# marsermd/DeepestScatter

Measured on AMD Instinct MI355X. Metric: Msamples/s (rays x spp) at 512^3 vol, 1024^2 frame; HBM GB/s vs roofline, higher is better.
Workload: dtype f32

## Files before the change

deepestscatter_amd/csrc/ct_api.cpp:

```cpp
#include <algorithm>
#include <array>
#include <atomic>
#include <chrono>
#include <climits>
#include <cmath>
#include <cstdarg>
#include <cstdio>
#include <cstdlib>
#include <cstring>
#include <new>
#include <string>
#include <utility>
#include <map>
#include <vector>

#include "../../include/cloudtrace.h"
#include "ct_handle.hpp"

static thread_local std::string g_create_error;

int ct::fail(CtHandle h, int code, const char *fmt, ...)
{
    char buf[512];
    va_list ap;
// ... 10 lines not shown

struct TracePhase {
    const char *name;
    std::chrono::steady_clock::time_point t0;
    bool on;
    TracePhase(CtHandle h, const char *n);
    ~TracePhase()
    {
        if (on) {
            fprintf(stderr, "[cloudtrace] %s %.2f ms\n", name,
                    std::chrono::duration<double, std::milli>(std::chrono::steady_clock::now() - t0).count());
        }
    }
};

inline TracePhase::TracePhase(CtHandle h, const char *n) : name(n), t0(std::chrono::steady_clock::now()), on(h && h->tune.TRACE) {}

static int check_invariants(CtHandle h);

static void v3_normalize_twice(const float in[3], float out[3])
{
    float v[3] = { in[0], in[1], in[2] };
    for (int pass = 0; pass < 2; pass++) {
        const float inv = 1.0f / sqrtf(v[0] * v[0] + v[1] * v[1] + v[2] * v[2]);
        v[0] *= inv;
        v[1] *= inv;
        v[2] *= inv;
    }
    out[0] = v[0];
    out[1] = v[1];
    out[2] = v[2];
}

static void mie_phase_texture(const float *raw, uint32_t n, std::vector<float> &out)
{
    out.resize(n);
    float average = 0;
    for (uint32_t i = 0; i < n; i++) {
        average += raw[i];
    }
    average /= (float)n;
    for (uint32_t i = 0; i < n; i++) {
        out[i] = raw[i] / average;
    }
}

static void mie_integral_texture(const float *raw, uint32_t n, std::vector<float> &out)
{
    out.resize(n);
    float sum = 0;
    for (uint32_t i = 0; i < n; i++) {
        sum += raw[i];
    }
    float integral = 0;
    for (uint32_t i = 0; i < n; i++) {
        integral += raw[i] / sum;
        out[i] = integral;
    }
}

static void build_guide(const std::vector<float> &cdf, std::vector<uint16_t> &guide)
{
    guide.assign(kGuideN + 2, 0);
    uint32_t t = 0;
    for (uint32_t b = 0; b <= (uint32_t)kGuideN; b++) {
        const float edge = (float)b / (float)kGuideN;
        while (t < cdf.size() && cdf[t] < edge) {
            t++;
        }
        guide[b] = (uint16_t)t;
    }
    guide[kGuideN + 1] = guide[kGuideN];
}

constexpr int kNeeSkipMaxR = 8;

static float nee_skip_reach(const DevScene &d)
{
    return d.sample_step * (1.0f - 1.0f / 256.0f);
}

static int nee_skip_radius(const DevScene &d, bool mie_finite)
{
    if (!mie_finite || !std::isfinite(d.lr) || !std::isfinite(d.lg) || !std::isfinite(d.lb) || !std::isfinite(d.sun_ratio) ||
        !(d.sample_step > 0.0f) || !std::isfinite(d.sample_step)) {
        return 0;
    }
    const double reach = (double)nee_skip_reach(d);
    int r = 0;
    for (const float s : { d.sx, d.sy, d.sz }) {
        const double D = reach * s * (1.0 + std::ldexp(1.0, -20)) + std::ldexp(1.0, -22) * (s + 1.0);
        if (!(D < kNeeSkipMaxR)) {
            return 0;
        }
        r = std::max(r, (int)std::ceil(D));
    }
    return std::max(r, 1);
}

static uint32_t morton2(uint32_t x, uint32_t y)
{
    auto spread = [](uint32_t v) {
        v &= 0xffffu;
        v = (v | (v << 8)) & 0x00ff00ffu;
        v = (v | (v << 4)) & 0x0f0f0f0fu;
        v = (v | (v << 2)) & 0x33333333u;
        v = (v | (v << 1)) & 0x55555555u;
        return v;
    };
    return spread(x) | (spread(y) << 1);
}

static uint32_t hilbert2(uint32_t x, uint32_t y)
{
    const uint32_t n = 1u << 15;
    uint32_t d = 0;
    for (uint32_t s = n / 2; s > 0; s /= 2) {
        const uint32_t rx = (x & s) ? 1u : 0u, ry = (y & s) ? 1u : 0u;
        d += s * s * ((3u * rx) ^ ry);
        if (ry == 0) {
            if (rx == 1) {
                x = n - 1u - x;
                y = n - 1u - y;
            }
            const uint32_t t = x;
            x = y;
            y = t;
        }
    }
    return d;
}

static void release(CtHandle h)
{
    if (!h) {
        return;
    }
    hipSetDevice(h->device);
    if (h->stream) {
        hipStreamSynchronize(h->stream);
    }
#ifdef CT_EXPERIMENTS
    if (h->vmm.va) {
        hipMemUnmap(h->vmm.va, h->vmm.size);
        for (auto &hd : h->vmm.handles) {
            hipMemRelease(hd);
        }
        hipMemAddressFree(h->vmm.va, h->vmm.size);
        h->vmm.va = nullptr;
        h->d_mbricks = nullptr;
    }
#endif
    void *ptrs[] = { h->d_density, h->d_inscatter, h->d_dbricks, h->d_ibricks, h->d_mbricks, h->d_tbricks, h->d_touched[0], h->d_touched[1], h->d_mrows, h->d_mcoarse, h->d_pyramid, h->d_mie, h->d_chopped, h->d_cdf,
                     h->d_guide, h->d_dist, h->d_dist_tmp, h->d_majorant, h->d_maj_cells, h->d_maj_codes, h->d_frame, h->d_mean, h->d_m2, h->d_screen, h->d_frames_all, h->cont[0], h->cont[1], h->left[0], h->left[1], h->d_cont_count, h->d_cont_total, h->d_primary, h->d_advance, h->d_pixels, h->d_cost, h->d_group_rank, h->d_group_order, h->d_job_group, h->d_job_sub, h->d_queue,
                     h->d_counters, h->d_colsum, h->d_avg, h->d_freeze, h->d_hit, h->d_cost_plane, h->d_timeline, h->pt.tasks, h->pt.primary, h->pt.frames, h->pt.pixels, h->pt.jg, h->pt.js,
                     h->net.found, h->net.waves, h->net.pos, h->net.dir, h->net.aux, h->net.out, h->net.desc, h->net.direct, h->net.tiles };
    for (void *p : ptrs) {
        if (p) {
            hipFree(p);
        }
    }
    for (auto &e : h->ev) {
        if (e) {
            hipEventDestroy(e);
        }
    }
    for (auto &sl : h->slots) {
        if (sl.queue) {
            hipFree(sl.queue);
        }
        for (hipEvent_t e : { sl.ev_in, sl.ev_start, sl.ev_done, sl.ev_acc0, sl.ev_acc1 }) {
            if (e) {
                hipEventDestroy(e);
            }
        }
    }
    for (hipEvent_t e : { h->ev_flush0, h->ev_flush1 }) {
        if (e) {
            hipEventDestroy(e);
        }
    }
    if (h->freeze_host) {
        hipHostFree(h->freeze_host);
    }
    if (h->hit_host) {
        hipHostFree(h->hit_host);
    }
    for (uint32_t *p : { h->jobs_host_g, h->jobs_host_s }) {
        if (p) {
            hipHostFree(p);
        }
    }
    if (h->own_stream) {
        hipStreamDestroy(h->own_stream);
    }
    delete h;
}

#ifdef CT_EXPERIMENTS
static int vmm_back_mbricks(CtHandle h)
{
    const size_t dense_bytes = h->mbricks_dense_bytes;
    hipMemAllocationProp prop{};
    prop.type = hipMemAllocationTypePinned;
    prop.location.type = hipMemLocationTypeDevice;
    prop.location.id = h->device;
    size_t gran = 0;
    HIPCHK(h, hipMemGetAllocationGranularity(&gran, &prop, hipMemAllocationGranularityRecommended));
    const size_t chunk = std::max<size_t>(gran, (size_t)2 << 20);
    if (chunk % 128 != 0 || (chunk & (chunk - 1)) != 0) {
        return fail(h, CT_E_HIP, "virtual-memory granularity %zu is not a power of two", chunk);
    }
    const size_t n_chunks = (dense_bytes + chunk - 1) / chunk;
    const size_t va_size = n_chunks * chunk;
    DevTemp<uint4> d_class;
    HIPCHK(h, dmalloc(&d_class, n_chunks));
    std::vector<uint4> cls(n_chunks);
    uint8_t *dense = h->d_mbricks;
    void *va = nullptr;
    std::vector<hipMemGenericAllocationHandle_t> handles;
    auto undo = [&]() {
        if (va) {
            hipMemUnmap(va, va_size);
            for (auto &hd : handles) {
                hipMemRelease(hd);
            }
            hipMemAddressFree(va, va_size);
        }
    };
#define VMMCHK(expr)                                                                                       \
    do {                                                                                                   \
        const hipError_t e_ = (expr);                                                                      \
        if (e_ != hipSuccess) {                                                                            \
            undo();                                                                                        \
            return fail(h, CT_E_HIP, "virtual-memory bricks: %s failed: %s", #expr, hipGetErrorString(e_)); \
        }                                                                                                  \
    } while (0)
    VMMCHK(launch_mbrick_chunk_class(dense, (int64_t)dense_bytes, (int64_t)chunk, d_class, h->stream));
    VMMCHK(hipMemcpyAsync(cls.data(), d_class, n_chunks * sizeof(uint4), hipMemcpyDeviceToHost, h->stream));
    VMMCHK(hipStreamSynchronize(h->stream));
    VMMCHK(hipMemAddressReserve(&va, va_size, chunk, nullptr, 0));
    std::vector<size_t> owner(n_chunks);
    std::vector<hipMemGenericAllocationHandle_t> of_chunk(n_chunks);
    std::map<uint64_t, size_t> first_with;
    size_t own = 0, with_data = 0;
    for (size_t c = 0; c < n_chunks; c++) {
        const bool whole = (c + 1) * chunk <= dense_bytes;
        owner[c] = c;
        if (whole && cls[c].x == 0u) {
            const uint64_t key = (uint64_t)cls[c].z | (uint64_t)cls[c].w << 32;
            const auto it = first_with.find(key);
            if (it != first_with.end()) {
                owner[c] = it->second;
            } else {
                first_with[key] = c;
            }
        } else {
            with_data += 1;
        }
        void *at = (uint8_t *)va + c * chunk;
        if (owner[c] == c) {
            hipMemGenericAllocationHandle_t hd;
            VMMCHK(hipMemCreate(&hd, chunk, &prop, 0));
            handles.push_back(hd);
            of_chunk[c] = hd;
            own += 1;
        } else {
            of_chunk[c] = of_chunk[owner[c]];
        }
        VMMCHK(hipMemMap(at, chunk, 0, of_chunk[c], 0));
    }
    hipMemAccessDesc acc{};
    acc.location = prop.location;
    acc.flags = hipMemAccessFlagsProtReadWrite;
    VMMCHK(hipMemSetAccess(va, va_size, &acc, 1));
    for (size_t c = 0; c < n_chunks; c++) {
        if (owner[c] != c) {
            continue;
        }
        uint8_t *at = (uint8_t *)va + c * chunk;
        const size_t n = std::min(chunk, dense_bytes - c * chunk);
        VMMCHK(hipMemcpyAsync(at, dense + c * chunk, n, hipMemcpyDeviceToDevice, h->stream));
        if (n < chunk) {
            VMMCHK(hipMemsetAsync(at + n, 0, chunk - n, h->stream));
        } else if (cls[c].x == 0u) {
            VMMCHK(launch_mbrick_chunk_quantize(at, (int64_t)chunk, h->stream));
        }
    }
    VMMCHK(hipStreamSynchronize(h->stream));
#undef VMMCHK
    HIPCHK(h, hipFree(dense));
    h->d_mbricks = (uint8_t *)va;
    h->dev.mbricks = h->d_mbricks;
    h->vmm.va = va;
    h->vmm.size = va_size;
    h->vmm.chunk = chunk;
    h->vmm.handles = std::move(handles);
    h->vmm.real_chunks = with_data;
    h->vmm.shared_chunks = own - with_data;
    h->vmm.mapped_chunks = n_chunks - own;
    h->mbricks_bytes = own * chunk;
    if (h->tune.STATS) {
        fprintf(stderr, "[cloudtrace] march bricks, dense addressing with sparse backing: %zu chunks of %zu KiB, %zu with texels, %zu distinct "
                        "empty ones, %zu mapped onto those: %.3f GB behind %.3f GB of addresses\n", n_chunks, chunk >> 10, with_data, own - with_data,
                n_chunks - own, (double)(own * chunk) / 1e9, (double)va_size / 1e9);
    }
    return CT_OK;
// ... 374 lines not shown
    HIPCHK(h, dmalloc(&h->d_majorant, nb));
    HIPCHK(h, launch_build_dist(h->d_density, nx, ny, nz, bbias, (int)bgx, (int)bgy, (int)bgz, h->d_dist,
                                h->d_dist_tmp, h->d_majorant, h->stream));
    HIPCHK(h, launch_brick_meta(h->d_dist, h->d_majorant, nx, ny, nz, bbias, (int)bgx, (int)bgy, (int)bgz,
                                h->d_dbricks, h->stream));
    return CT_OK;
}

static int build_majorant_grid(const CtScene *s, CtHandle h)
{
    DevScene &d = h->dev;
    const uint32_t nx = s->dims[0], ny = s->dims[1], nz = s->dims[2];
    const int32_t n[3] = { (int32_t)nx, (int32_t)ny, (int32_t)nz };
    const int bbias = d.brick_bias;
    int32_t lo[3], hi[3];
    density_bbox(s->density_host, n, lo, hi);
    const MajorantCells m = majorant_cells(n, bbias, lo, hi);
    if (!majorant_div_exact(m)) {
        return fail(h, CT_E_INVAL, "volume too large for the majorant grid's index arithmetic");
    }
    const auto &[C, div, origin, stored, virt] = m;
    const size_t cells = (size_t)stored[0] * stored[1] * stored[2];
    HIPCHK(h, dmalloc(&h->d_maj_cells, (cells + 3) & ~(size_t)3));
    HIPCHK(h, hipMemsetAsync(h->d_maj_cells, 0, (cells + 3) & ~(size_t)3, h->stream));
    HIPCHK(h, dmalloc(&h->d_maj_codes, (cells + 3) & ~(size_t)3));
    HIPCHK(h, hipMemsetAsync(h->d_maj_codes, 0, (cells + 3) & ~(size_t)3, h->stream));
    HIPCHK(h, launch_majorant_cells(h->d_density, nx, ny, nz, bbias, C, origin, stored[0], stored[1], stored[2], h->d_maj_cells,
                                    h->d_maj_codes, h->stream));
    d.maj_cells = h->d_maj_cells;
    d.maj_codes = h->d_maj_codes;
    d.mc_cell = C;
    d.mc_div = div;
    d.mc_gx = stored[0];
    d.mc_gy = stored[1];
    d.mc_gz = stored[2];
    d.mc_x0 = origin[0];
    d.mc_y0 = origin[1];
    d.mc_z0 = origin[2];
    d.mc_vx = virt[0];
    d.mc_vy = virt[1];
    d.mc_vz = virt[2];
    const int32_t bg[3] = { d.brick_gx, d.brick_gy, d.brick_gz };
    d.delta_interior = (cells_inside_apron(lo, hi, n, m, bg) && knob_flag(h->tune.DELTA_INTERIOR, true)) ? 1u : 0u;
    return CT_OK;
}

static int twin_grid(CtHandle h)
{
    DevScene &d = h->dev;
    const int bbias = d.brick_bias, tbias = ((bbias + 2) / 3) * 3;
    const int64_t tgx = ((int64_t)d.nx + bbias + tbias + 2) / 3 + 1, tgy = ((int64_t)d.ny + bbias + tbias + 2) / 3 + 1,
                  tgz = ((int64_t)d.nz + bbias + tbias + 2) / 3 + 1;
    if (!brick_indices_fit(tgx, tgy, tgz) || (int64_t)std::max({ d.nx, d.ny, d.nz }) + 2 * tbias >= (1 << 15)) {
        return fail(h, CT_E_INVAL, "volume too large for 32-bit brick indices");
    }
    if (hipMalloc(&h->d_tbricks, (size_t)(tgx * tgy * tgz) * 128) != hipSuccess) {
        return fail(h, CT_E_NOMEM, "out of device memory (twin bricks)");
    }
    d.tbricks = h->d_tbricks;
    d.t_bias = tbias;
    d.t_gx = (int32_t)tgx;
    d.t_gy = (int32_t)tgy;
    d.t_gz = (int32_t)tgz;
    if (!cells_inside_twin(d)) {
        d.delta_interior = 0u;
    }
    return CT_OK;
}

static int compact_march_bricks(CtHandle h, const uint8_t *tmp_b)
{
    DevScene &d = h->dev;
    const uint32_t nx = (uint32_t)d.nx, ny = (uint32_t)d.ny, nz = (uint32_t)d.nz;
    const int bbias = d.brick_bias;
    const int64_t bgx = d.brick_gx, bgy = d.brick_gy, bgz = d.brick_gz, mgx = d.m_gx;
    const size_t rows = (size_t)(bgy * bgz);
    DevTemp<uint32_t> d_x0, d_x1;
    DevTemp<uint8_t> compact;
    auto run = [&]() -> int {
        HIPCHK(h, dmalloc(&d_x0, rows));
        HIPCHK(h, dmalloc(&d_x1, rows));
        HIPCHK(h, hipMemsetAsync(d_x0, 0xff, rows * sizeof(uint32_t), h->stream));
        HIPCHK(h, hipMemsetAsync(d_x1, 0, rows * sizeof(uint32_t), h->stream));
        HIPCHK(h, launch_mbrick_extent(h->d_mbricks, (int)mgx, (int)bgy, (int)bgz, d_x0, d_x1, h->stream));
        std::vector<uint32_t> x0(rows), x1(rows);
        HIPCHK(h, hipMemcpyAsync(x0.data(), d_x0, rows * sizeof(uint32_t), hipMemcpyDeviceToHost, h->stream));
        HIPCHK(h, hipMemcpyAsync(x1.data(), d_x1, rows * sizeof(uint32_t), hipMemcpyDeviceToHost, h->stream));
        HIPCHK(h, hipStreamSynchronize(h->stream));
        std::vector<uint2> ri(rows);
        uint64_t lines = 0;
        for (size_t r = 0; r < rows; r++) {
            const uint32_t cnt = x1[r] > x0[r] ? x1[r] - x0[r] : 0u;
            ri[r] = make_uint2((uint32_t)lines, cnt ? (x0[r] | (cnt << 16)) : 0u);
            lines += cnt;
        }
        if (lines >= (1ull << 32)) {
            return fail(h, CT_E_INVAL, "volume too large for 32-bit brick indices");
        }
        HIPCHK(h, dmalloc(&h->d_mrows, rows));
        HIPCHK(h, hipMemcpyAsync(h->d_mrows, ri.data(), rows * sizeof(uint2), hipMemcpyHostToDevice, h->stream));
        HIPCHK(h, dmalloc(&compact, std::max<size_t>((size_t)lines, 1) * 128));
        HIPCHK(h, launch_mbrick_compact(h->d_mbricks, (int)mgx, (int)bgy, (int)bgz, h->d_mrows, compact, h->stream));
        const int cshift = 3;
        const int64_t cgx = (4 * bgx + 7) >> cshift, cgy = (4 * bgy + 7) >> cshift, cgz = (4 * bgz + 7) >> cshift;
        HIPCHK(h, dmalloc(&h->d_mcoarse, (size_t)(cgx * cgy * cgz)));
        HIPCHK(h, launch_coarse_clearance(tmp_b, nx, ny, nz, bbias, cshift, (int)cgx, (int)cgy, (int)cgz, h->d_mcoarse,
                                          h->stream));
        HIPCHK(h, hipStreamSynchronize(h->stream));
        HIPCHK(h, hipFree(h->d_mbricks));
        h->d_mbricks = compact.release();
        d.mbricks = h->d_mbricks;
        h->mbricks_bytes = (size_t)lines * 128;
        d.m_rows = h->d_mrows;
        d.m_coarse = h->d_mcoarse;
        d.m_cshift = cshift;
        d.m_cgx = (int32_t)cgx;
        d.m_cgxy = (int32_t)(cgx * cgy);
        return CT_OK;
    };
    const int rc = run();
    if (rc != CT_OK) {
        hipStreamSynchronize(h->stream);
    }
    return rc;
}

static int build_march_layouts(const CtScene *s, CtHandle h, int apron, const MarchStorage &ms, uint32_t zero_faces, bool mie_finite)
{
    DevScene &d = h->dev;
    const uint32_t nx = s->dims[0], ny = s->dims[1], nz = s->dims[2];
    const size_t texels = h->volume_bytes;
    const int bbias = d.brick_bias;
    const int64_t bgx = d.brick_gx, bgy = d.brick_gy, bgz = d.brick_gz;
#ifndef CT_EXPERIMENTS
    if (ms.experimental) {
        return fail(h, CT_E_INVAL, "march bricks behind virtual memory (CT_FLAG_VMM_BRICKS, CT_SPARSE=2..4) were measured and rejected "
                                   "(DESIGN.md 4.3 item 7b): they exist in the experiments build only (build --variant exp; CT_LIBRARY=libcloudtrace_exp.so)");
    }
#endif
    const int mbias = ((apron + 2) / 3) * 3;
    int64_t mgx = ((int64_t)nx + 2 * mbias + 2) / 3 + 1;
    if (ms.pad_rows) {
        int64_t p2 = 1;
        while (p2 < mgx) {
            p2 <<= 1;
        }
        mgx = p2;
    }
    if (!brick_indices_fit(mgx, bgy, bgz) || (int64_t)nx + 2 * mbias >= (1 << 17)) {
        return fail(h, CT_E_INVAL, "volume too large for 32-bit brick indices");
    }
    const size_t dense_bytes = (size_t)(mgx * bgy * bgz) * 128;
    h->mbricks_dense_bytes = h->mbricks_bytes = dense_bytes;
    HIPCHK(h, dmalloc(&h->d_mbricks, dense_bytes));
    d.mbricks = h->d_mbricks;
    d.m_bias_x = mbias;
    d.m_gx = (int32_t)mgx;
    d.m_gxy = (int32_t)(mgx * bgy);
    DevTemp<uint8_t> tmp_a, tmp_b, tmp_c;
    HIPCHK(h, dmalloc(&tmp_a, texels));
    if (dmalloc(&tmp_b, texels) != hipSuccess) {
        return fail(h, CT_E_NOMEM, "out of device memory (distance transform scratch)");
    }
    hipError_t e = launch_build_mbricks(h->d_density, nx, ny, nz, mbias, bbias, (int)mgx, (int)bgy, (int)bgz,
                                        tmp_a, tmp_b, h->d_mbricks, h->stream);
    if (e == hipSuccess) {
        e = launch_inscatter(d, h->d_inscatter, zero_faces, h->stream);
    }
    if (e == hipSuccess) {
        e = launch_build_bricks(h->d_inscatter, nx, ny, nz, bbias, (int)bgx, (int)bgy, (int)bgz, h->d_ibricks, h->stream);
    }
    const int nee_r = s->estimator == CT_EST_MARCH ? nee_skip_radius(d, mie_finite) : 0;
    if (e == hipSuccess && nee_r > 0) {
        e = dmalloc(&tmp_c, texels);
        if (e == hipSuccess) {
            e = launch_nee_skip_flags(h->d_inscatter, nx, ny, nz, nee_r, mbias, bbias, (int)mgx, (int)bgy, (int)bgz, tmp_a, tmp_c,
                                      h->d_mbricks, h->stream);
            d.nee_reach = nee_skip_reach(d);
            h->nee_skip_r = nee_r;
        }
    }
    if (e == hipSuccess && s->estimator == CT_EST_DELTA && d.delta_nee == 2u) {
        CT_TRY(twin_grid(h));
        e = launch_build_twin_bricks(h->d_density, h->d_inscatter, nx, ny, nz, d.t_bias, d.t_gx, d.t_gy, d.t_gz, h->d_tbricks, h->stream);
    }
    const hipError_t e2 = hipStreamSynchronize(h->stream);
    HIPCHK(h, e);
    HIPCHK(h, e2);
    return ms.sparse ? compact_march_bricks(h, tmp_b) : CT_OK;
}

static int frame_buffers(const CtScene *s, CtHandle h)
{
    const size_t pixels = (size_t)s->width * s->height;
    HIPCHK(h, dmalloc(&h->d_frame, pixels));
    HIPCHK(h, dmalloc(&h->d_mean, pixels));
    HIPCHK(h, dmalloc(&h->d_m2, pixels));
    HIPCHK(h, dmalloc(&h->d_screen, pixels));
    HIPCHK(h, dmalloc(&h->d_colsum, s->width));
    HIPCHK(h, dmalloc(&h->d_avg, 2));
    HIPCHK(h, dmalloc(&h->d_queue, kQueueWords));
    HIPCHK(h, dmalloc(&h->d_cont_count, 6));
    HIPCHK(h, hipMemsetAsync(h->d_cont_count, 0, 6 * sizeof(uint32_t), h->stream));
    h->cont_capacity = (size_t)h->shape.blocks * h->shape.threads;
    HIPCHK(h, hipEventCreate(&h->ev_flush0));
    HIPCHK(h, hipEventCreate(&h->ev_flush1));
    if (h->tune.TIMELINE.get()) {
        const size_t waves = (size_t)h->shape.blocks * h->shape.threads / 64u;
        HIPCHK(h, dmalloc(&h->d_timeline, 4 * waves));
        HIPCHK(h, hipMemsetAsync(h->d_timeline, 0, 4 * waves * sizeof(unsigned long long), h->stream));
    }
    HIPCHK(h, dmalloc(&h->d_cont_total, 1));
    HIPCHK(h, hipMemsetAsync(h->d_cont_total, 0, sizeof(unsigned long long), h->stream));
    for (auto &c : h->cont) {
        HIPCHK(h, dmalloc(&c, h->cont_capacity * (s->estimator == CT_EST_DELTA ? kContWordsDelta : kContWords)));
    }
    h->left_capacity = h->cont_capacity / 64;
    for (auto &c : h->left) {
        HIPCHK(h, dmalloc(&c, h->left_capacity * kLeftWords));
    }
    for (auto &sl : h->slots) {
        HIPCHK(h, dmalloc(&sl.queue, kQueueWords));
        for (hipEvent_t *e : { &sl.ev_in, &sl.ev_start, &sl.ev_done, &sl.ev_acc0, &sl.ev_acc1 }) {
            HIPCHK(h, hipEventCreate(e));
        }
    }
    HIPCHK(h, dmalloc(&h->d_counters, kCounterCount + 1 + kStatCount));
    HIPCHK(h, dmalloc(&h->d_freeze, 8));
    HIPCHK(h, hipMemsetAsync(h->d_freeze, 0, 8 * sizeof(uint32_t), h->stream));
    HIPCHK(h, hipHostMalloc((void **)&h->freeze_host, 4 * sizeof(uint32_t), hipHostMallocDefault));
    memset(h->freeze_host, 0, 4 * sizeof(uint32_t));
    HIPCHK(h, hipMemsetAsync(h->d_frame, 0, pixels * sizeof(float4), h->stream));
    HIPCHK(h, hipMemsetAsync(h->d_mean, 0, pixels * sizeof(float4), h->stream));
    HIPCHK(h, hipMemsetAsync(h->d_m2, 0, pixels * sizeof(float4), h->stream));
    HIPCHK(h, hipMemsetAsync(h->d_screen, 0, pixels * sizeof(uchar4), h->stream));
    HIPCHK(h, hipMemsetAsync(h->d_counters, 0, (kCounterCount + 1 + kStatCount) * sizeof(unsigned long long), h->stream));

    HIPCHK(h, dmalloc(&h->d_primary, 2 * pixels));
    HIPCHK(h, dmalloc(&h->d_advance, (s->estimator == CT_EST_DELTA ? 4 : 1) * pixels));
    HIPCHK(h, hipStreamSynchronize(h->stream));
    return CT_OK;
}

static int create_impl(const CtScene *s, CtHandle h)
{
    h->scene = *s;
    h->device = s->device;
    h->volume_bytes = (size_t)s->dims[0] * s->dims[1] * s->dims[2];
    h->tune = CtTuning::from_env();
    CT_TRY(open_device(s, h));
    CT_TRY(choose_schedule(s, h));
    scene_uniforms(s, h->dev);
    int apron = 0;
    CT_TRY(apron_grid(s, h, apron));
    CT_TRY(upload_mie(s, h, h->mie_finite));
    CT_TRY(build_apron_bricks(s, h));
    if (s->estimator == CT_EST_DELTA) {
        CT_TRY(build_majorant_grid(s, h));
    }
    const MarchStorage ms = march_storage(s, h->tune.SPARSE);
    h->zero_faces = zero_faces(s->density_host, s->dims[0], s->dims[1], s->dims[2]);
    CT_TRY(build_march_layouts(s, h, apron, ms, h->zero_faces, h->mie_finite));
#ifdef CT_EXPERIMENTS
    if (ms.vmm) {
        CT_TRY(vmm_back_mbricks(h));
    }
#endif
    CT_TRY(frame_buffers(s, h));

    const float eye[3] = { 2.5f, -0.4f, 0.f }, lookat[3] = { 0, 0, 0 }, up[3] = { 0, 1, 0 };
    float U[3], V[3], W[3];
    ct_calculate_camera_variables(eye, lookat, up, 30.0f, (float)s->width / (float)s->height, U, V, W);
    return ct_set_camera(h, eye, U, V, W);
}

extern "C" int ct_create(const CtScene *s, CtHandle *out)
{
    if (!out) {
        return fail(nullptr, CT_E_INVAL, "out is NULL");
    }
    *out = nullptr;
    if (!s) {
        return fail(nullptr, CT_E_INVAL, "scene is NULL");
    }
    if (s->abi_version != CT_ABI_VERSION) {
        return fail(nullptr, CT_E_INVAL, "abi_version %u, library is %u", s->abi_version, CT_ABI_VERSION);
    }
    if (!s->density_host || s->dims[0] < 2 || s->dims[1] < 2 || s->dims[2] < 2 || s->dims[0] > 2048 ||
        s->dims[1] > 2048 || s->dims[2] > 2048) {
        return fail(nullptr, CT_E_INVAL, "density volume missing or dims out of range [2,2048]");
    }
    if (s->mode < 0 || s->mode > 2) {
        return fail(nullptr, CT_E_INVAL, "Invalid Render Mode %d", s->mode);
    }
    if (s->estimator != CT_EST_MARCH && s->estimator != CT_EST_DELTA) {
        return fail(nullptr, CT_E_INVAL, "unknown estimator %d", s->estimator);
    }
    if (s->estimator == CT_EST_DELTA && (s->flags & CT_FLAG_SIMPLE_KERNEL)) {
        return fail(nullptr, CT_E_INVAL, "the one-thread-per-pixel cross-check kernel only implements MARCH");
    }
    if (!s->mie_host || !s->chopped_mie_host || s->mie_count != (uint32_t)kMieN) {
        return fail(nullptr, CT_E_INVAL, "Mie tables must be %d floats each", kMieN);
    }
    if (s->width == 0 || s->height == 0 || s->width > 12288 || s->height > 4096) {
        return fail(nullptr, CT_E_INVAL, "frame %ux%u out of range (seed packing x*4096+y needs H <= 4096)", s->width,
                    s->height);
    }
    if (!(s->sample_step > 0.f) || !(s->sample_step <= 0.03125f) || !(s->cloud_size_m > 0.f) ||
        !(s->mean_free_path_m > 0.f) || s->max_depth < 2 || s->max_depth > 65535) {
        return fail(nullptr, CT_E_INVAL, "sample_step/cloud_size_m/mean_free_path_m/max_depth out of range (max_depth 2..65535)");
    }
    if (!(s->cloud_size_m / s->mean_free_path_m * s->sample_step < 80.f)) {
        return fail(nullptr, CT_E_INVAL, "optical depth per step %g too large (must be < 80)",
                    (double)(s->cloud_size_m / s->mean_free_path_m * s->sample_step));
    }
    const float ll = s->light_direction[0] * s->light_direction[0] + s->light_direction[1] * s->light_direction[1] +
                     s->light_direction[2] * s->light_direction[2];
    if (!(ll > 0.f)) {
        return fail(nullptr, CT_E_INVAL, "light_direction is zero");
    }
    if (s->shard_count == 0 || s->shard_index >= s->shard_count) {
        return fail(nullptr, CT_E_INVAL, "shard %u of %u", s->shard_index, s->shard_count);
    }
    CtHandle h = new (std::nothrow) CtHandle_();
    if (!h) {
        return fail(nullptr, CT_E_NOMEM, "out of host memory");
    }
    const int rc = create_impl(s, h);
    if (rc != CT_OK) {
        g_create_error = h->error;
        release(h);
        return rc;
    }
    h->scene.density_host = nullptr;
    h->scene.mie_host = nullptr;
    h->scene.chopped_mie_host = nullptr;
    *out = h;
    return CT_OK;
}

extern "C" int ct_destroy(CtHandle h)
{
    release(h);
    return CT_OK;
}

extern "C" const char *ct_last_error(CtHandle h)
{
    return h ? h->error.c_str() : g_create_error.c_str();
}

extern "C" int ct_set_stream(CtHandle h, void *hip_stream)
{
    NEED(h);
    HIPCHK(h, hipStreamSynchronize(h->stream));
    h->stream = hip_stream ? (hipStream_t)hip_stream : h->own_stream;
    return CT_OK;
}

extern "C" int ct_set_camera(CtHandle h, const float eye[3], const float U[3], const float V[3], const float W[3])
{
    NEED(h);
    if (!eye || !U || !V || !W) {
        return fail(h, CT_E_INVAL, "camera vectors must not be NULL");
    }
    DevScene &d = h->dev;
    d.ex = eye[0]; d.ey = eye[1]; d.ez = eye[2];
    d.ux = U[0]; d.uy = U[1]; d.uz = U[2];
    d.vx = V[0]; d.vy = V[1]; d.vz = V[2];
    d.wx = W[0]; d.wy = W[1]; d.wz = W[2];
    h->camera_set = true;
    h->queue_dirty = true;
    discard_ahead(h);
    return CT_OK;
}

static int relight(CtHandle h, const CtScene &s)
{
    DevScene d = h->dev;
    light_uniforms(&s, d);
    const bool march = s.estimator == CT_EST_MARCH;
    const int nee_r = march ? nee_skip_radius(d, h->mie_finite) : 0;
    DevTemp<uint8_t> tmp_a, tmp_c;
    if (nee_r > 0 && (dmalloc(&tmp_a, h->volume_bytes) != hipSuccess || dmalloc(&tmp_c, h->volume_bytes) != hipSuccess)) {
        (void)hipGetLastError();
        return fail(h, CT_E_NOMEM, "out of device memory (shadow-zero flags scratch); the light is unchanged");
    }
    d.nee_reach = nee_r > 0 ? nee_skip_reach(d) : 0.0f;
    h->scene = s;
    h->dev = d;
    h->nee_skip_r = nee_r;
    discard_ahead(h);
    h->queue_dirty = true;
    h->tile_deepest.clear();
    const int nx = d.nx, ny = d.ny, nz = d.nz, bbias = d.brick_bias;
    hipError_t e = launch_inscatter(d, h->d_inscatter, h->zero_faces, h->stream);
    if (e == hipSuccess) {
        e = launch_build_bricks(h->d_inscatter, nx, ny, nz, bbias, d.brick_gx, d.brick_gy, d.brick_gz, h->d_ibricks, h->stream);
    }
    if (e == hipSuccess && march) {
        e = launch_shadow_zero_rows(h->d_inscatter, nx, ny, nz, nee_r, d.m_bias_x, bbias, d.m_gx, d.brick_gy, d.brick_gz, tmp_a, tmp_c,
                                    h->d_mbricks, h->d_mrows, h->stream);
    }
    if (e == hipSuccess && h->d_tbricks) {
        e = launch_twin_shadow_half(h->d_inscatter, nx, ny, nz, d.t_bias, d.t_gx, d.t_gy, d.t_gz, h->d_tbricks, h->stream);
    }
    const hipError_t e2 = hipStreamSynchronize(h->stream);
    HIPCHK(h, e);
    HIPCHK(h, e2);
    return CT_OK;
}

extern "C" int ct_set_light(CtHandle h, const float direction[3], const float color[3], float intensity)
{
    NEED_NOFLUSH(h);
    if (!direction) {
        return fail(h, CT_E_INVAL, "light direction must not be NULL");
    }
    if (!std::isfinite(direction[0]) || !std::isfinite(direction[1]) || !std::isfinite(direction[2])) {
        return fail(h, CT_E_INVAL, "light direction is not finite");
    }
    if (!(direction[0] * direction[0] + direction[1] * direction[1] + direction[2] * direction[2] > 0.f)) {
        return fail(h, CT_E_INVAL, "light_direction is zero");
    }
    if (h->vmm.va) {
        return fail(h, CT_E_INVAL, "ct_set_light: march bricks behind virtual memory cannot be re-lit");
    }
    const int rc = flush(h);
    if (rc != CT_OK) {
        return rc;
    }
    CtScene s = h->scene;
    for (int a = 0; a < 3; a++) {
        s.light_direction[a] = direction[a];
        if (color) {
            s.light_color[a] = color[a];
        }
    }
    s.light_intensity = intensity;
    return relight(h, s);
}

static int rebuild_queue(CtHandle h)
{
    TracePhase trace(h, "rebuild_queue");
    const uint32_t W = h->scene.width, H = h->scene.height;
    const size_t pixels = (size_t)W * H;
    HIPCHK(h, launch_primary_rays(h->dev, h->d_primary, h->stream));
    if (h->scene.estimator == CT_EST_DELTA) {
        HIPCHK(h, launch_primary_advance_delta(h->dev, h->d_primary, h->d_advance, h->stream));
    } else {
        HIPCHK(h, launch_primary_advance(h->dev, h->d_primary, h->d_advance, h->stream));
    }
    if (!h->d_hit) {
        HIPCHK(h, dmalloc(&h->d_hit, pixels));
        HIPCHK(h, hipHostMalloc((void **)&h->hit_host, pixels, hipHostMallocDefault));
    }
    HIPCHK(h, launch_hit_flags(h->d_primary, h->d_hit, (uint32_t)pixels, h->stream));
    HIPCHK(h, hipMemcpyAsync(h->hit_host, h->d_hit, pixels, hipMemcpyDeviceToHost, h->stream));
    HIPCHK(h, hipStreamSynchronize(h->stream));
    const uint8_t *hit = h->hit_host;
    const uint32_t tiles_x = h->dev.tiles_x, tiles_y = h->dev.tiles_y;
    std::vector<std::pair<uint32_t, uint32_t>> tiles;
    for (uint32_t ty = 0; ty < tiles_y; ty++) {
        for (uint32_t tx = 0; tx < tiles_x; tx++) {
            if (tile_owner(tx, ty, h->scene.shard_count) == h->scene.shard_index) {
                tiles.emplace_back(h->tile_hilbert ? hilbert2(tx, ty) : morton2(tx, ty), ty * tiles_x + tx);
            }
        }
    }
    std::sort(tiles.begin(), tiles.end());
    std::vector<uint32_t> list;
    list.reserve(pixels / std::max(1u, h->scene.shard_count) + 64);
    uint64_t own = 0;
    for (const auto &t : tiles) {
        const uint32_t ty = t.second / tiles_x, tx = t.second - ty * tiles_x;
        for (uint32_t l = 0; l < 64; l++) {
            const uint32_t x = tx * kTile + (l & 7u), y = ty * kTile + (l >> 3);
            if (x < W && y < H) {
                own++;
                const uint32_t p = y * W + x;
                if (hit[p]) {
                    list.push_back(p);
                }
            }
        }
    }
    h->own_pixels = own;
    h->hit_pixels = list.size();
    while (list.size() % 64 != 0) {
        list.push_back(0xffffffffu);
    }
    h->n_groups = (uint32_t)(list.size() / 64);
    if (h->n_groups > h->groups_capacity) {
        for (void *p : { (void *)h->d_pixels, (void *)h->d_cost }) {
            if (p) {
                HIPCHK(h, hipFree(p));
            }
        }
        h->d_pixels = h->d_cost = nullptr;
        for (void *p : { (void *)h->d_group_rank, (void *)h->d_group_order }) {
            if (p) {
                HIPCHK(h, hipFree(p));
            }
        }
        h->d_group_rank = h->d_group_order = nullptr;
        HIPCHK(h, dmalloc(&h->d_pixels, (size_t)h->n_groups * 64));
        HIPCHK(h, dmalloc(&h->d_cost, 2 * (size_t)h->n_groups));
        HIPCHK(h, dmalloc(&h->d_group_rank, (size_t)h->n_groups));
        HIPCHK(h, dmalloc(&h->d_group_order, (size_t)h->n_groups));
        h->groups_capacity = h->n_groups;
    }
    h->group_order.resize(h->n_groups);
    h->group_tile.resize(h->n_groups);
    for (uint32_t i = 0; i < h->n_groups; i++) {
        h->group_order[i] = i;
        const uint32_t p = list[(size_t)i * 64];
        h->group_tile[i] = (p / W / kTile) * tiles_x + (p % W) / kTile;
    }
    if (h->tile_deepest.size() == (size_t)tiles_x * tiles_y) {
        auto log2_class = [](uint32_t c) {
            uint32_t k = 0;
            while (c) {
                k++;
                c >>= 1;
            }
            return k;
        };
        std::stable_sort(h->group_order.begin(), h->group_order.end(), [&](uint32_t a, uint32_t b) {
            return log2_class(h->tile_deepest[h->group_tile[a]]) > log2_class(h->tile_deepest[h->group_tile[b]]);
        });
    }
    h->group_depth.assign(h->n_groups, 0.f);
    if (h->n_groups) {
        HIPCHK(h, hipMemcpyAsync(h->d_pixels, list.data(), list.size() * sizeof(uint32_t), hipMemcpyHostToDevice,
                                 h->stream));
        HIPCHK(h, hipMemsetAsync(h->d_cost, 0, 2 * (size_t)h->n_groups * sizeof(uint32_t), h->stream));
        HIPCHK(h, hipStreamSynchronize(h->stream));
    }
    h->queue_dirty = false;
    h->order_tuned = false;
    h->jobs_S = 0;
    return CT_OK;
}

static bool short_batch(CtHandle h, uint32_t S)
{
    return h->scene.estimator != CT_EST_DELTA && (double)S * (double)std::max<uint64_t>(h->hit_pixels, 1) < 4.0e7;
}

static int build_jobs(CtHandle h, uint32_t S, uint32_t chunk_groups)
{
    chunk_groups = std::max(1u, std::min(chunk_groups, std::max(h->n_groups, 1u)));
    if (h->jobs_S >= S && h->jobs_brief == short_batch(h, S) && h->chunk_groups == chunk_groups) {
        return CT_OK;
    }
    TracePhase trace(h, "build_jobs");
    if (h->order_tuned) {
        S = std::max(S, h->jobs_hint);
    }
    const float unit = (h->scene.estimator == CT_EST_DELTA) ? 1.f : 16.f;
    const bool brief = short_batch(h, S);
    const bool queues = (h->queues_enabled || (brief && !h->tune.XCD_QUEUES.get())) && !(h->scene.flags & CT_FLAG_SIMPLE_KERNEL) &&
                        (h->order_tuned || h->tune.XCD_QUEUES_UNTUNED.get());
    const uint32_t nq = (queues && h->n_groups >= (uint32_t)kQueues) ? (uint32_t)kQueues : 1u;
    const uint32_t regions_wanted = (brief && !h->queues_enabled && !h->tune.XCD_REGIONS.get()) ? 16u : h->regions;
    const float job_work = (brief && !h->tune.JOB_WORK.get()) ? 4.f : h->job_work;
    const float shared_cost = h->shared_depth * unit;
    std::vector<uint8_t> queue_of(h->n_groups, 0);
    {
        double total = 0;
        for (uint32_t g = 0; g < h->n_groups; g++) {
            if (nq > 1u && h->group_depth[g] >= shared_cost) {
                queue_of[g] = (uint8_t)kQueues;
            } else {
                total += (double)h->group_depth[g] + unit;
            }
        }
        double run = 0;
        for (uint32_t g = 0; g < h->n_groups; g++) {
            if (queue_of[g] == (uint8_t)kQueues) {
                continue;
            }
            const double w = (double)h->group_depth[g] + unit;
            const uint32_t regions = std::max(nq, regions_wanted);
            const uint32_t r = (uint32_t)std::min<double>(regions - 1, std::floor((run + 0.5 * w) / total * regions));
            queue_of[g] = (uint8_t)(r % nq);
            run += w;
        }
    }
    auto job_length = [&](uint32_t g) {
        const float d = h->group_depth[g];
        if (!h->order_tuned) {
            return 1u;
        }
        uint32_t len = h->job_max;
        if (d > 0.f) {
            len = (uint32_t)std::min((float)h->job_max, std::max(1.f, job_work * unit / d));
        }
        return len;
    };
    size_t total_jobs = 0;
    for (uint32_t g = 0; g < h->n_groups; g++) {
        const uint32_t len = job_length(g);
        total_jobs += (S + len - 1) / len;
    }
    if (total_jobs > h->jobs_host_capacity) {
        for (uint32_t **pp : { &h->jobs_host_g, &h->jobs_host_s }) {
            if (*pp) {
                HIPCHK(h, hipHostFree(*pp));
                *pp = nullptr;
            }
        }
        h->jobs_host_capacity = total_jobs + total_jobs / 4 + 1024;
        HIPCHK(h, hipHostMalloc((void **)&h->jobs_host_g, h->jobs_host_capacity * sizeof(uint32_t), hipHostMallocDefault));
        HIPCHK(h, hipHostMalloc((void **)&h->jobs_host_s, h->jobs_host_capacity * sizeof(uint32_t), hipHostMallocDefault));
    }
    uint32_t *const jg = h->jobs_host_g, *const js = h->jobs_host_s;
    size_t nj = 0;
    std::vector<double> q_weight(kQueues + 1, 0.0);
    const uint32_t n_chunks = h->n_groups ? (h->n_groups + chunk_groups - 1) / chunk_groups : 1u;
    if (n_chunks > 1 && h->chunk_interleave) {
        std::vector<uint32_t> mixed;
        mixed.reserve(h->n_groups);
        for (uint32_t c = 0; c < n_chunks; c++) {
            for (uint32_t r = c; r < h->n_groups; r += n_chunks) {
                mixed.push_back(h->group_order[r]);
            }
        }
        h->job_order = mixed;
    } else if (n_chunks > 1 && h->chunk_morton) {
        h->job_order.resize(h->n_groups);
        for (uint32_t g = 0; g < h->n_groups; g++) {
            h->job_order[g] = g;
        }
    } else {
        h->job_order = h->group_order;
    }
    h->chunk_q_begin.assign(n_chunks, std::array<uint32_t, kQueues + 2>{});
    for (uint32_t c = 0; c < n_chunks; c++) {
        const uint32_t r0 = c * chunk_groups, r1 = std::min(h->n_groups, r0 + chunk_groups);
        for (uint32_t x = 0; x <= (uint32_t)kQueues; x++) {
            h->chunk_q_begin[c][x] = (uint32_t)nj;
            if (x != 0u && nq == 1u && x != (uint32_t)kQueues) {
                continue;
            }
            for (uint32_t r = r0; r < r1; r++) {
                const uint32_t g = h->job_order[r];
                if (queue_of[g] != x) {
                    continue;
                }
                q_weight[x] += (double)h->group_depth[g] + unit;
                const uint32_t len = job_length(g);
                for (uint32_t s0 = 0; s0 < S; s0 += len) {
                    jg[nj] = g;
                    js[nj] = s0 | (std::min(len, S - s0) << 16);
                    nj += 1;
                }
            }
        }
        h->chunk_q_begin[c][kQueues + 1] = (uint32_t)nj;
    }
    for (int x = 0; x <= kQueues + 1; x++) {
        h->q_begin[x] = h->chunk_q_begin[0][x];
    }
    if (h->tune.STATS.get()) {
        fprintf(stderr, "[cloudtrace] job queues (S=%u, %u chunk(s) of %u groups):", S, n_chunks, chunk_groups);
        for (int x = 0; x <= kQueues; x++) {
            fprintf(stderr, " q%d weight %.0f;", x, q_weight[x]);
        }
        fprintf(stderr, "\n");
    }
    {
        std::vector<uint32_t> rank(h->n_groups);
        for (uint32_t r = 0; r < h->n_groups; r++) {
            rank[h->job_order[r]] = r;
        }
        if (h->n_groups) {
            HIPCHK(h, hipMemcpyAsync(h->d_group_rank, rank.data(), rank.size() * sizeof(uint32_t), hipMemcpyHostToDevice, h->stream));
            HIPCHK(h, hipMemcpyAsync(h->d_group_order, h->job_order.data(), h->job_order.size() * sizeof(uint32_t),
                                     hipMemcpyHostToDevice, h->stream));
            HIPCHK(h, hipStreamSynchronize(h->stream));
        }
    }
    h->chunk_groups = chunk_groups;
    h->n_chunks = n_chunks;
    h->n_jobs = (uint32_t)nj;
    if (h->n_jobs > h->jobs_capacity) {
        for (void *p : { (void *)h->d_job_group, (void *)h->d_job_sub }) {
            if (p) {
// ... 181 lines not shown
    }
    sl.pending = false;
    HIPCHK(h, hipEventSynchronize(sl.accumulated ? sl.ev_acc1 : sl.ev_done));
    float ms = 0;
    HIPCHK(h, hipEventElapsedTime(&ms, sl.ev_start, sl.ev_done));
    h->render_ms += ms;
    if (h->tune.TRACE.get()) {
        uint32_t cnt[3] = { 0, 0, 0 };
        hipMemcpy(cnt, h->d_cont_count, sizeof cnt, hipMemcpyDeviceToHost);
        fprintf(stderr, "[cloudtrace] estimator launch %.2f ms (suspended paths per buffer now: %u %u, cursor %u)\n", ms,
                cnt[0], cnt[1], cnt[2]);
    }
    if (sl.accumulated) {
        HIPCHK(h, hipEventElapsedTime(&ms, sl.ev_acc0, sl.ev_acc1));
        h->accum_ms += ms;
    }
    h->launches += 1;
    return CT_OK;
}

int ct::enqueue_convergence_test(CtHandle h, uint32_t subframes)
{
    HIPCHK(h, launch_converged_freeze(h->d_mean, h->d_m2, subframes, (uint64_t)h->scene.width * h->scene.height, 500u ,
                                      h->d_freeze, h->stream));
    HIPCHK(h, hipMemcpyAsync(h->freeze_host, h->d_freeze, 4 * sizeof(uint32_t), hipMemcpyDeviceToHost, h->stream));
    return CT_OK;
}

static int enqueue_accumulate(CtHandle h, CtHandle_::Slot &sl, const float4 *frames, bool dense, uint32_t n)
{
    const bool simple = (h->scene.flags & CT_FLAG_SIMPLE_KERNEL) != 0;
    const bool chunked = !(simple || dense) && h->n_chunks > 1;
    const uint32_t cadence = h->stop_cadence;
    const uint32_t *frozen = cadence ? h->d_freeze : nullptr;
    HIPCHK(h, hipEventRecord(sl.ev_acc0, h->stream));
    while (n != 0u) {
        const uint32_t off = sl.acc_done, next = sl.first + off;
        uint32_t piece = n;
        if (cadence && !chunked) {
            piece = std::min(n, cadence - (next - 1u) % cadence);
        }
        if (simple || dense) {
            HIPCHK(h, launch_accumulate_batch(frames + (size_t)off * h->scene.width * h->scene.height, h->d_mean, h->d_m2, next, piece,
                                              h->scene.width, h->scene.height, h->scene.shard_index, h->scene.shard_count,
                                              h->d_counters + 8, frozen, h->stream));
        } else {
            HIPCHK(h, launch_accumulate_list(frames + (size_t)off * frame_stride(h), (uint32_t)frame_stride(h), h->d_pixels, sl.groups * 64u,
                                             h->n_chunks <= 1 ? nullptr : h->d_group_order, sl.rank_base,
                                             sl.with_misses, h->d_primary, h->d_mean, h->d_m2, next, piece, h->scene.width,
                                             h->scene.height, h->scene.shard_index, h->scene.shard_count, h->d_counters + 8, frozen,
                                             h->stream));
        }
        sl.acc_done += piece;
        n -= piece;
        const uint32_t upto = sl.first + sl.acc_done - 1u;
        const bool whole_image = !chunked || (sl.last_chunk && sl.acc_done == sl.S);
        if (cadence && whole_image && upto % cadence == 0u && upto >= h->stop_min) {
            const int rc = enqueue_convergence_test(h, upto);
            if (rc != CT_OK) {
                return rc;
            }
        }
    }
    HIPCHK(h, hipEventRecord(sl.ev_acc1, h->stream));
    sl.accumulated = true;
    return CT_OK;
}

static uint32_t accumulate_target(CtHandle h)
{
    if (h->ahead == 0) {
        return 0xffffffffu;
    }
    const uint64_t lag = (uint64_t)std::max(h->n_regions - 1, 1) * h->ahead;
    return h->subframes > lag ? (uint32_t)(h->subframes - lag) : 0u;
}

static int advance_accumulate(CtHandle h, uint32_t target)
{
    while (!h->waiting.empty()) {
        const int w = h->waiting.front();
        CtHandle_::Slot &sl = h->slots[w];
        if (!sl.complete) {
            break;
        }
        const uint32_t next = sl.first + sl.acc_done, last = sl.first + sl.S - 1u;
        const uint32_t upto = std::min(last, target);
        if (upto >= next && sl.acc_done < sl.S) {
            const int rc = enqueue_accumulate(h, sl, slot_frames(h, w), false, upto - next + 1u);
            if (rc != CT_OK) {
                return rc;
            }
        }
        if (sl.acc_done < sl.S) {
            break;
        }
        sl.awaits_accumulate = false;
        h->waiting.erase(h->waiting.begin());
    }
    return CT_OK;
}

void ct::discard_ahead(CtHandle h)
{
    for (int w : h->waiting) {
        h->slots[w].awaits_accumulate = false;
    }
    h->waiting.clear();
    h->rendered = h->subframes;
}

static int launch_estimator(CtHandle h, const BatchArgs &ba)
{
    DevScene sc = h->dev;
    if (ba.S != 0 && short_batch(h, ba.S) && !h->tune.REGEN_MIN.get()) {
        sc.regen_min = 16;
    }
    bool launched = false;
#ifdef CT_EXPERIMENTS
    if (h->exchange && !ba.cost && !ba.cont_in && !ba.cont_out && h->scene.estimator == CT_EST_DELTA) {
        if (h->exchange == 2) {
            HIPCHK(h, launch_render_delta_w(sc, ba, h->xshape, h->stream));
        } else {
            HIPCHK(h, launch_render_delta_x(sc, ba, h->xshape, h->stream));
        }
        launched = true;
    }
#endif
    if (launched) {
    } else if (h->scene.estimator == CT_EST_DELTA) {
        HIPCHK(h, launch_render_delta(sc, ba, h->shape, h->stream));
    } else {
        HIPCHK(h, launch_render_persistent(sc, ba, h->shape, h->stream));
    }
    return CT_OK;
}

static int submit_batch(CtHandle h, int slot, float4 *dense_frames, uint32_t first, uint32_t S, bool accumulate,
                        bool suspend, uint32_t chunk)
{
    CtHandle_::Slot &sl = h->slots[slot];
    const bool simple = (h->scene.flags & CT_FLAG_SIMPLE_KERNEL) != 0;
    const bool dense = dense_frames != nullptr;
    const uint32_t max_age = (uint32_t)(h->n_regions - 1);
    const uint32_t rank_base = chunk * h->chunk_groups;
    const uint32_t chunk_n = h->n_groups > rank_base ? std::min(h->chunk_groups, h->n_groups - rank_base) : 0u;
    BatchArgs ba{};
    ba.frames = dense ? dense_frames : (simple ? slot_frames(h, slot) : h->d_frames_all);
    ba.frame_stride = (simple || dense) ? 0u : (uint32_t)frame_stride(h);
    ba.out_offset = (simple || dense) ? 0u : (uint32_t)((size_t)slot * h->slot_capacity);
    ba.primary = h->d_primary;
    ba.advance = h->no_advance ? nullptr : h->d_advance;
    ba.pixels = h->d_pixels;
    ba.group_rank = (simple || dense || h->n_chunks <= 1) ? nullptr : h->d_group_rank;
    ba.rank_base = rank_base;
    ba.job_group = h->d_job_group;
    ba.job_sub = h->d_job_sub;
    const bool measure = !h->order_tuned && !simple && !dense && chunk_n != 0u;
    if (measure) {
        const size_t entries = (size_t)S * frame_stride(h);
        if (entries > h->cost_plane_capacity) {
            if (h->d_cost_plane) {
                HIPCHK(h, hipFree(h->d_cost_plane));
                h->d_cost_plane = nullptr;
            }
            h->cost_plane_capacity = entries + entries / 4;
            HIPCHK(h, dmalloc(&h->d_cost_plane, h->cost_plane_capacity));
        }
        HIPCHK(h, hipMemsetAsync(h->d_cost_plane, 0, entries * sizeof(uint2), h->stream));
        ba.cost = h->d_cost_plane;
    }
    static const std::array<uint32_t, kQueues + 2> no_jobs{};
    const auto &qb = chunk < h->chunk_q_begin.size() ? h->chunk_q_begin[chunk] : no_jobs;
    ba.n_jobs = qb[kQueues + 1];
    for (int x = 0; x <= kQueues + 1; x++) {
        ba.q_begin[x] = qb[x];
    }
    const uint32_t chunk_jobs = qb[kQueues + 1] - qb[0];
    ba.first_subframe = first;
    ba.S = S;
    ba.queue = sl.queue;
    ba.counters = h->d_counters;
    ba.stats = h->d_counters + kCounterCount + 1;
    ba.timeline = h->d_timeline;
    ba.touched_density = h->d_touched[0];
    ba.touched_shadow = h->d_touched[1];
    if (suspend && short_batch(h, S) && h->serpentine) {
        ba.reverse = (uint32_t)(h->launch_no & 1u);
    }
    const int buf_out = (int)(h->launch_no & 1u), buf_in = buf_out ^ 1;
    ZeroList zero;
    if (h->cont_live) {
        ba.cont_in = h->cont[buf_in];
        ba.cont_in_count = h->d_cont_count + buf_in;
        ba.cont_cursor = h->d_cont_count + 2;
        ba.left_in = h->left[buf_in];
        ba.left_in_count = h->d_cont_count + 3 + buf_in;
        ba.left_cursor = h->d_cont_count + 5;
        zero.add(h->d_cont_count + 2, 1);
        zero.add(h->d_cont_count + 5, 1);
    }
    if (suspend) {
        ba.cont_out = h->cont[buf_out];
        ba.cont_out_count = h->d_cont_count + buf_out;
        ba.cont_capacity = (uint32_t)h->cont_capacity;
        ba.max_age = std::max(1u, max_age);
        ba.cont_total = h->d_cont_total;
        if (h->hand_on_jobs) {
            ba.left_out = h->left[buf_out];
            ba.left_out_count = h->d_cont_count + 3 + buf_out;
            ba.left_capacity = (uint32_t)h->left_capacity;
        }
        zero.add(h->d_cont_count + buf_out, 1);
        zero.add(h->d_cont_count + 3 + buf_out, 1);
    }
    zero.add(sl.queue, kQueueWords);
    HIPCHK(h, launch_zero_words(zero, h->stream));
    if (h->debug_invariants && !simple && !dense && h->n_groups != 0) {
        HIPCHK(h, hipMemsetD32Async((hipDeviceptr_t)slot_frames(h, slot), 0x7fc0deadu, (size_t)S * frame_stride(h) * 4u,
                                    h->stream));
    }
    HIPCHK(h, hipEventRecord(sl.ev_start, h->stream));
    if (simple) {
        h->host_paths += h->own_pixels * S;
        h->host_hits += h->hit_pixels * S;
        for (uint32_t s = 0; s < S; s++) {
            BatchArgs one = ba;
            one.frames = ba.frames + (size_t)s * h->scene.width * h->scene.height;
            one.first_subframe = first + s;
            one.S = 1;
            HIPCHK(h, launch_render_simple(h->dev, one, h->scene.shard_index, h->scene.shard_count, h->stream));
        }
    } else {
        if (chunk_jobs != 0 || ba.cont_in) {
            const int rc = launch_estimator(h, ba);
            if (rc != CT_OK) {
                return rc;
            }
            if (measure) {
                HIPCHK(h, launch_cost_reduce(h->d_cost_plane, (uint32_t)frame_stride(h), S, chunk_n,
                                             h->n_chunks <= 1 ? nullptr : h->d_group_order, rank_base, h->d_cost,
                                             h->d_cost + h->n_groups, h->stream));
            }
        }
        uint64_t chunk_hits = 0;
        for (uint32_t r = rank_base; r < rank_base + chunk_n; r++) {
            chunk_hits += (h->job_order[r] + 1u == h->n_groups) ? 64u - (uint64_t)((uint64_t)h->n_groups * 64u - h->hit_pixels) : 64u;
        }
        if (chunk == 0) {
            h->host_paths += h->own_pixels * S;
        }
        h->host_hits += chunk_hits * S;
        h->iv_expected_dealt += chunk_hits * S;
    }
    HIPCHK(h, hipEventRecord(sl.ev_done, h->stream));
    h->launch_no += 1;
    h->cont_live = suspend && !simple;
    sl.first = first;
    sl.S = S;
    sl.rank_base = rank_base;
    sl.groups = chunk_n;
    sl.with_misses = chunk == 0;
    sl.last_chunk = simple || dense || chunk + 1u >= std::max(h->n_chunks, 1u);
    sl.pending = true;
    sl.accumulated = false;
    sl.awaits_accumulate = false;
    sl.complete = false;
    sl.acc_done = 0;
    if (accumulate) {
        if (suspend) {
            sl.awaits_accumulate = true;
            h->waiting.push_back(slot);
            uint32_t younger = 0;
            for (size_t i = h->waiting.size(); i-- > 0;) {
                CtHandle_::Slot &w = h->slots[h->waiting[i]];
                if (!w.complete && ++younger > max_age) {
                    w.complete = true;
                }
            }
            return advance_accumulate(h, accumulate_target(h));
        } else {
            sl.complete = true;
            const int rc = enqueue_accumulate(h, sl, dense ? dense_frames : slot_frames(h, slot), dense, S);
            if (rc != CT_OK) {
                return rc;
            }
        }
    }
    return CT_OK;
}

static int check_invariants(CtHandle h)
{
    unsigned long long iv[4] = { 0, 0, 0, 0 }, bad = 0;
    HIPCHK(h, hipStreamSynchronize(h->stream));
    HIPCHK(h, hipMemcpy(iv, h->d_counters + kCounterCount + 1 + 64, sizeof iv, hipMemcpyDeviceToHost));
    HIPCHK(h, hipMemcpy(&bad, h->d_counters + 8, sizeof bad, hipMemcpyDeviceToHost));
    h->iv_checks += 1;
    const unsigned long long dealt = iv[0], resumed = iv[1], written = iv[2], suspended = iv[3];
    const bool simple = (h->scene.flags & CT_FLAG_SIMPLE_KERNEL) != 0;
    const bool ok = simple || (dealt + resumed == written + suspended && resumed == suspended && dealt == h->iv_expected_dealt &&
                               bad == 0);
    if (!ok) {
        h->iv_violations += 1;
        fprintf(stderr, "[cloudtrace] INVARIANT VIOLATED: dealt %llu (host expects %llu) resumed %llu written %llu suspended %llu, "
                        "samples without alpha 1 seen by accumulate: %llu\n",
                dealt, (unsigned long long)h->iv_expected_dealt, resumed, written, suspended, bad);
        return fail(h, CT_E_STATE, "invariant violated: dealt %llu (expected %llu) resumed %llu written %llu suspended %llu bad samples %llu",
                    dealt, (unsigned long long)h->iv_expected_dealt, resumed, written, suspended, bad);
    }
    return CT_OK;
}

int ct::flush(CtHandle h)
{
    if (h->cont_live) {
        BatchArgs ba{};
        ba.frames = h->d_frames_all;
        ba.frame_stride = (uint32_t)frame_stride(h);
        ba.primary = h->d_primary;
        ba.advance = h->no_advance ? nullptr : h->d_advance;
        ba.pixels = h->d_pixels;
        ba.job_group = h->d_job_group;
        ba.job_sub = h->d_job_sub;
        ba.n_jobs = 0;
        ba.first_subframe = 1;
        ba.S = 0;
        ba.queue = h->d_queue;
        ba.counters = h->d_counters;
        ba.stats = h->d_counters + kCounterCount + 1;
        const int buf_in = (int)((h->launch_no & 1u) ^ 1u);
        ba.cont_in = h->cont[buf_in];
        ba.cont_in_count = h->d_cont_count + buf_in;
        ba.cont_cursor = h->d_cont_count + 2;
        ba.left_in = h->left[buf_in];
        ba.left_in_count = h->d_cont_count + 3 + buf_in;
        ba.left_cursor = h->d_cont_count + 5;
        HIPCHK(h, hipMemsetAsync(h->d_cont_count + 2, 0, sizeof(uint32_t), h->stream));
        HIPCHK(h, hipMemsetAsync(h->d_cont_count + 5, 0, sizeof(uint32_t), h->stream));
        HIPCHK(h, hipMemsetAsync(h->d_queue, 0, kQueueWords * sizeof(uint32_t), h->stream));
        HIPCHK(h, hipEventRecord(h->ev_flush0, h->stream));
        const int rc = launch_estimator(h, ba);
        if (rc != CT_OK) {
            return rc;
        }
        HIPCHK(h, hipEventRecord(h->ev_flush1, h->stream));
        h->launch_no += 1;
        h->cont_live = false;
        HIPCHK(h, hipEventSynchronize(h->ev_flush1));
        float ms = 0;
        HIPCHK(h, hipEventElapsedTime(&ms, h->ev_flush0, h->ev_flush1));
        h->render_ms += ms;
        if (h->tune.TRACE.get()) {
            fprintf(stderr, "[cloudtrace] resume-only launch %.2f ms\n", ms);
        }
    }
    for (int w : h->waiting) {
        h->slots[w].complete = true;
    }
    {
        const int rc = advance_accumulate(h, h->ahead ? h->subframes : 0xffffffffu);
        if (rc != CT_OK) {
            return rc;
        }
    }
    for (int k = 0; k < CtHandle_::kMaxRegions; k++) {
        const int rc = collect(h, h->slots[k]);
        if (rc != CT_OK) {
            return rc;
        }
    }
    return h->debug_invariants ? check_invariants(h) : CT_OK;
}

static int prepare_batches(CtHandle h, uint32_t S)
{
    const bool simple = (h->scene.flags & CT_FLAG_SIMPLE_KERNEL) != 0;
    if (simple) {
        h->chunk_groups = std::max(h->n_groups, 1u);
        h->n_chunks = 1;
        return CT_OK;
    }
    if (h->queue_dirty) {
        int rc = flush(h);
        discard_ahead(h);
        if (rc == CT_OK) {
            rc = rebuild_queue(h);
        }
        if (rc != CT_OK) {
            return rc;
        }
    }
    const uint32_t want = groups_per_chunk(h, S);
    if (h->jobs_S < S || h->jobs_brief != short_batch(h, S) || h->chunk_groups != want || h->chunk_q_begin.empty()) {
        const int rc = flush(h);
        discard_ahead(h);
        return rc == CT_OK ? build_jobs(h, S, want) : rc;
    }
    return CT_OK;
}

static int run_batch(CtHandle h, float4 *dense_frames, uint32_t first, uint32_t S, bool accumulate)
{
    int rc = flush(h);
    discard_ahead(h);
    if (rc == CT_OK) {
        rc = prepare_batches(h, S);
    }
    if (rc == CT_OK && !dense_frames) {
        rc = ensure_frames(h, S, false);
    }
    if (rc != CT_OK) {
        return rc;
    }
    for (uint32_t c = 0; c < std::max(h->n_chunks, 1u) && rc == CT_OK; c++) {
        rc = submit_batch(h, 0, dense_frames, first, S, accumulate, false, c);
        if (rc == CT_OK) {
            rc = collect(h, h->slots[0]);
        }
    }
    if (rc != CT_OK) {
        return rc;
    }
    const bool simple = (h->scene.flags & CT_FLAG_SIMPLE_KERNEL) != 0;
    if (!simple && !h->order_tuned && !dense_frames) {
        return tune_order(h, S);
    }
    return CT_OK;
}

extern "C" int ct_render_subframe(CtHandle h, uint32_t subframe_id, float *frame_rgba_dev)
{
    NEED(h);
    if (!h->camera_set) {
        return fail(h, CT_E_STATE, "ct_set_camera has not been called");
    }
    const size_t bytes = (size_t)h->scene.width * h->scene.height * sizeof(float4);
    HIPCHK(h, launch_fill_frame(h->d_frame, h->scene.width, h->scene.height, h->scene.shard_index,
                                h->scene.shard_count, h->stream));
    const int rc = run_batch(h, h->d_frame, subframe_id, 1, false);
    if (rc != CT_OK) {
        return rc;
    }
    if (frame_rgba_dev) {
        HIPCHK(h, hipMemcpyAsync(frame_rgba_dev, h->d_frame, bytes, hipMemcpyDeviceToDevice, h->stream));
        HIPCHK(h, hipStreamSynchronize(h->stream));
    }
    return CT_OK;
}

extern "C" int ct_accumulate(CtHandle h, uint32_t subframe_id, const float *frame_rgba_dev)
{
    NEED(h);
    if (subframe_id == 0) {
        return fail(h, CT_E_INVAL, "subframe ids are 1-based (Camera.cpp:191)");
    }
    const float4 *src = frame_rgba_dev ? (const float4 *)frame_rgba_dev : h->d_frame;
    HIPCHK(h, hipEventRecord(h->ev[1], h->stream));
    HIPCHK(h, launch_accumulate_batch(src, h->d_mean, h->d_m2, subframe_id, 1, h->scene.width, h->scene.height,
                                      h->scene.shard_index, h->scene.shard_count, nullptr, h->stop_cadence ? h->d_freeze : nullptr,
                                      h->stream));
    if (h->stop_cadence && subframe_id % h->stop_cadence == 0u && subframe_id >= h->stop_min) {
        const int rc = enqueue_convergence_test(h, subframe_id);
        if (rc != CT_OK) {
            return rc;
        }
    }
    HIPCHK(h, hipEventRecord(h->ev[2], h->stream));
    HIPCHK(h, hipEventSynchronize(h->ev[2]));
    float ms = 0;
    HIPCHK(h, hipEventElapsedTime(&ms, h->ev[1], h->ev[2]));
    h->accum_ms += ms;
    h->subframes = subframe_id;
    discard_ahead(h);
    return CT_OK;
// ... 1144 lines not shown
```

deepestscatter_amd/csrc/ct_device.hpp:

```cpp
#pragma once

#include <hip/hip_runtime.h>
#include <stdint.h>

#include "../../include/ct_fmath.h"

namespace ct {

#define CT_DEV __device__ __forceinline__

struct f3 {
    float x, y, z;
};

CT_DEV f3 mk3(float x, float y, float z) { return f3{ x, y, z }; }
CT_DEV f3 add3(f3 a, f3 b) { return mk3(a.x + b.x, a.y + b.y, a.z + b.z); }
CT_DEV f3 sub3(f3 a, f3 b) { return mk3(a.x - b.x, a.y - b.y, a.z - b.z); }
CT_DEV f3 scale3(f3 a, float s) { return mk3(a.x * s, a.y * s, a.z * s); }
CT_DEV float dot3(f3 a, f3 b) { return a.x * b.x + a.y * b.y + a.z * b.z; }
CT_DEV f3 cross3(f3 a, f3 b)
{
    return mk3(a.y * b.z - a.z * b.y, a.z * b.x - a.x * b.z, a.x * b.y - a.y * b.x);
}
CT_DEV float rcp_(float x) { return 1.0f / x; }
// ... 35 lines not shown
struct DevScene {
    const uint8_t *dbricks;
    const uint8_t *ibricks;
    int32_t brick_bias;
    int32_t brick_gx;
    int32_t brick_gxy;
    int32_t brick_gy, brick_gz;
    uint32_t tex_fixed8;
    const uint8_t *mbricks;
    const uint2 *m_rows;
    const uint8_t *m_coarse;
    int32_t m_cshift, m_cgx, m_cgxy;
    const uint8_t *tbricks;
    int32_t t_bias;
    int32_t t_gx, t_gy, t_gz;
    uint32_t delta_nee;
    uint32_t delta_interior;
    const uint8_t *maj_cells;
    const uint8_t *maj_codes;
    int32_t mc_cell, mc_div, mc_gx, mc_gy, mc_gz, mc_x0, mc_y0, mc_z0, mc_vx, mc_vy, mc_vz;
    int32_t m_bias_x;
    int32_t m_gx, m_gxy;
    int32_t nx, ny, nz;
    float sx, sy, sz;
    float tsx, tsy, tsz;
    float bx, by, bz;
    float hx, hy, hz;
    float density_multiplier;
    float sample_step;
    float nlx, nly, nlz;
    float lr, lg, lb;
    float sun_ratio;
    const float *mie;
    const float *chopped;
    const float *cdf;
    const uint16_t *guide;
    float ex, ey, ez, ux, uy, uz, vx, vy, vz, wx, wy, wz;
    uint32_t width, height;
    uint32_t max_depth;
    int32_t mode;
    uint32_t tiles_x, tiles_y;
    uint32_t regen_min;
    uint32_t march_burst;
    uint32_t burst_scatter;
    uint32_t burst_idle;
    uint32_t tail_burst;
    uint32_t nee_cache;
    float nee_reach;
    uint32_t hint_period;
    uint32_t burst_march_min;
    uint32_t scatter_num, scatter_den;
    uint32_t scatter_min;
};

CT_DEV uint32_t tea4(uint32_t v0, uint32_t v1)
{
    uint32_t s0 = 0;
#pragma unroll
    for (int n = 0; n < 4; n++) {
        s0 += 0x9e3779b9u;
        v0 += ((v1 << 4) + 0xa341316cu) ^ (v1 + s0) ^ ((v1 >> 5) + 0xc8013ea4u);
        v1 += ((v0 << 4) + 0xad90777du) ^ (v0 + s0) ^ ((v0 >> 5) + 0x7e95761eu);
    }
    return v0;
}

CT_DEV uint32_t lcg24(uint32_t &prev)
{
    prev = 1664525u * prev + 1013904223u;
    return prev & 0x00FFFFFFu;
}

CT_DEV float u24_to_float(uint32_t u) { return (float)u / (float)0x01000000; }

CT_DEV bool in_box(const DevScene &sc, f3 p)
{
    return p.x >= -0.01f && p.y >= -0.01f && p.z >= -0.01f && p.x <= sc.hx && p.y <= sc.hy && p.z <= sc.hz;
}
CT_DEV bool in_box_flat(const DevScene &sc, f3 p)
{
    return (p.x >= -0.01f) & (p.y >= -0.01f) & (p.z >= -0.01f) & (p.x <= sc.hx) & (p.y <= sc.hy) & (p.z <= sc.hz);
}

CT_DEV float fract_(float x) { return __builtin_amdgcn_fractf(x); }

template <bool FIXED8>
CT_DEV float tex_weight(float x)
{
    if constexpr (FIXED8) {
        return __builtin_rintf(fract_(x) * 256.0f) * (1.0f / 256.0f);
    } else {
        return fract_(x);
    }
}

CT_DEV float filter_cell(uint2 c, float wx, float wy, float wz)
{
    const float t000 = (float)(c.x & 0xffu), t100 = (float)((c.x >> 8) & 0xffu);
    const float t010 = (float)((c.x >> 16) & 0xffu), t110 = (float)(c.x >> 24);
    const float t001 = (float)(c.y & 0xffu), t101 = (float)((c.y >> 8) & 0xffu);
    const float t011 = (float)((c.y >> 16) & 0xffu), t111 = (float)(c.y >> 24);
    const float c00 = fmaf(wx, t100 - t000, t000), c10 = fmaf(wx, t110 - t010, t010);
    const float c01 = fmaf(wx, t101 - t001, t001), c11 = fmaf(wx, t111 - t011, t011);
    const float c0 = fmaf(wy, c10 - c00, c00), c1 = fmaf(wy, c11 - c01, c01);
    return fmaf(wz, c1 - c0, c0) * (1.0f / 255.0f);
}

CT_DEV uint2 load_footprint(const DevScene &sc, const uint8_t *bricks, int32_t ix, int32_t iy, int32_t iz)
{
    const uint32_t x = (uint32_t)(ix + sc.brick_bias), y = (uint32_t)(iy + sc.brick_bias), z = (uint32_t)(iz + sc.brick_bias);
    const uint32_t brick = __umul24(z >> 2, (uint32_t)sc.brick_gxy) + __umul24(y >> 2, (uint32_t)sc.brick_gx) + (x >> 2);
    const uint32_t local = __umul24(z & 3u, 25u) + __umul24(y & 3u, 5u) + (x & 3u);
#ifdef CT_DEBUG_BOUNDS
    if ((x >> 2) >= (uint32_t)sc.brick_gx || (y >> 2) >= (uint32_t)sc.brick_gy || (z >> 2) >= (uint32_t)sc.brick_gz) {
        printf("CT_DEBUG_BOUNDS footprint texel (%d,%d,%d) outside the brick grid\n", ix, iy, iz);
        return make_uint2(0u, 0u);
    }
#endif
    const uint8_t *p = bricks + (((size_t)brick << 7) | local);
    uint2 a, c;
    __builtin_memcpy(&a, p, 8);
    __builtin_memcpy(&c, p + 25, 8);
    uint2 r;
    r.x = __builtin_amdgcn_perm(a.y, a.x, 0x06050100u);
    r.y = __builtin_amdgcn_perm(c.y, c.x, 0x06050100u);
    return r;
}

CT_DEV uint2 load_footprint_meta(const DevScene &sc, const uint8_t *bricks, int32_t ix, int32_t iy, int32_t iz,
                                 uint32_t &meta)
{
    const uint32_t x = (uint32_t)(ix + sc.brick_bias), y = (uint32_t)(iy + sc.brick_bias), z = (uint32_t)(iz + sc.brick_bias);
    const uint32_t brick = __umul24(z >> 2, (uint32_t)sc.brick_gxy) + __umul24(y >> 2, (uint32_t)sc.brick_gx) + (x >> 2);
    const uint32_t local = __umul24(z & 3u, 25u) + __umul24(y & 3u, 5u) + (x & 3u);
#ifdef CT_DEBUG_BOUNDS
    if ((x >> 2) >= (uint32_t)sc.brick_gx || (y >> 2) >= (uint32_t)sc.brick_gy || (z >> 2) >= (uint32_t)sc.brick_gz) {
        printf("CT_DEBUG_BOUNDS footprint texel (%d,%d,%d) outside the brick grid\n", ix, iy, iz);
        meta = 0u;
        return make_uint2(0u, 0u);
    }
#endif
    const uint8_t *base = bricks + ((size_t)brick << 7);
    const uint8_t *p = base + local;
    uint2 a, c;
    __builtin_memcpy(&a, p, 8);
    __builtin_memcpy(&c, p + 25, 8);
    meta = base[125];
    uint2 r;
    r.x = __builtin_amdgcn_perm(a.y, a.x, 0x06050100u);
    r.y = __builtin_amdgcn_perm(c.y, c.x, 0x06050100u);
    return r;
}

template <bool SPARSE>
CT_DEV uint2 load_footprint_m(const DevScene &sc, int32_t ix, int32_t iy, int32_t iz, uint32_t &meta)
{
    const uint32_t x = (uint32_t)(ix + sc.m_bias_x), y = (uint32_t)(iy + sc.brick_bias), z = (uint32_t)(iz + sc.brick_bias);
    const uint32_t bx = __umul24(x, 43691u) >> 17;
    const uint32_t lx = x - __umul24(bx, 3u);
    const uint32_t brick = __umul24(z >> 2, (uint32_t)sc.m_gxy) + __umul24(y >> 2, (uint32_t)sc.m_gx) + bx;
    const uint32_t local = __umul24(z & 3u, 25u) + __umul24(y & 3u, 5u) + lx;
#ifdef CT_DEBUG_BOUNDS
    if (bx >= (uint32_t)sc.m_gx || (y >> 2) >= (uint32_t)sc.brick_gy || (z >> 2) >= (uint32_t)sc.brick_gz) {
        printf("CT_DEBUG_BOUNDS march-brick texel (%d,%d,%d) outside the grid\n", ix, iy, iz);
        meta = 0u;
        return make_uint2(0u, 0u);
    }
#endif
    const uint8_t *p = sc.mbricks + (((size_t)brick << 7) | local);
    if (SPARSE) {
        const uint32_t row = __umul24(z >> 2, (uint32_t)sc.brick_gy) + (y >> 2);
        const uint2 ri = sc.m_rows[row];
        const uint32_t rel = bx - (ri.y & 0xffffu);
        if (rel >= (ri.y >> 16)) {
            const uint32_t cx = (uint32_t)(ix + sc.brick_bias) >> sc.m_cshift;
            meta = sc.m_coarse[__umul24(z >> sc.m_cshift, (uint32_t)sc.m_cgxy) + __umul24(y >> sc.m_cshift, (uint32_t)sc.m_cgx) + cx];
            return make_uint2(0u, 0u);
        }
        p = sc.mbricks + (((size_t)(ri.x + rel) << 7) | local);
    }
    uint2 a, c;
    __builtin_memcpy(&a, p, 8);
    __builtin_memcpy(&c, p + 25, 8);
    meta = __builtin_amdgcn_perm(a.y, a.x, 0x0c0c0c04u - lx);
    uint2 r;
    r.x = __builtin_amdgcn_perm(a.y, a.x, 0x06050100u);
    r.y = __builtin_amdgcn_perm(c.y, c.x, 0x06050100u);
    return r;
}

CT_DEV int32_t floor_to_int(float x)
{
    int32_t r;
    asm("v_cvt_flr_i32_f32 %0, %1" : "=v"(r) : "v"(x));
    return r;
}

template <bool FIXED8>
CT_DEV float tex3_apron(const DevScene &sc, const uint8_t *bricks, f3 p)
{
    const float x = fmaf(p.x, sc.sx, -0.5f), y = fmaf(p.y, sc.sy, -0.5f), z = fmaf(p.z, sc.sz, -0.5f);
    const int32_t ix = floor_to_int(x), iy = floor_to_int(y), iz = floor_to_int(z);
    const uint2 c = load_footprint(sc, bricks, ix, iy, iz);
    return filter_cell(c, tex_weight<FIXED8>(x), tex_weight<FIXED8>(y), tex_weight<FIXED8>(z));
}

CT_DEV uint2 fetch_cell(const DevScene &sc, const uint8_t *bricks, f3 p, uint32_t &meta)
{
    const float x = fmaf(p.x, sc.sx, -0.5f), y = fmaf(p.y, sc.sy, -0.5f), z = fmaf(p.z, sc.sz, -0.5f);
    return load_footprint_meta(sc, bricks, floor_to_int(x), floor_to_int(y), floor_to_int(z), meta);
}

CT_DEV uint2 fetch_cell_in_grid(const DevScene &sc, const uint8_t *bricks, f3 p, uint32_t &meta)
{
    const float x = fmaf(p.x, sc.sx, -0.5f), y = fmaf(p.y, sc.sy, -0.5f), z = fmaf(p.z, sc.sz, -0.5f);
    const int32_t lo = -sc.brick_bias;
    const int32_t ix = min(max(floor_to_int(x), lo), 4 * sc.brick_gx - 1 + lo);
    const int32_t iy = min(max(floor_to_int(y), lo), 4 * sc.brick_gy - 1 + lo);
    const int32_t iz = min(max(floor_to_int(z), lo), 4 * sc.brick_gz - 1 + lo);
    return load_footprint_meta(sc, bricks, ix, iy, iz, meta);
}

CT_DEV size_t apron_offset_in_grid(const DevScene &sc, f3 p)
{
    const float x = fmaf(p.x, sc.sx, -0.5f), y = fmaf(p.y, sc.sy, -0.5f), z = fmaf(p.z, sc.sz, -0.5f);
    const int32_t lo = -sc.brick_bias;
    const uint32_t ux = (uint32_t)(min(max(floor_to_int(x), lo), 4 * sc.brick_gx - 1 + lo) + sc.brick_bias);
    const uint32_t uy = (uint32_t)(min(max(floor_to_int(y), lo), 4 * sc.brick_gy - 1 + lo) + sc.brick_bias);
    const uint32_t uz = (uint32_t)(min(max(floor_to_int(z), lo), 4 * sc.brick_gz - 1 + lo) + sc.brick_bias);
    const uint32_t brick = __umul24(uz >> 2, (uint32_t)sc.brick_gxy) + __umul24(uy >> 2, (uint32_t)sc.brick_gx) + (ux >> 2);
    const uint32_t local = __umul24(uz & 3u, 25u) + __umul24(uy & 3u, 5u) + (ux & 3u);
    return ((size_t)brick << 7) | local;
}
CT_DEV size_t apron_offset_unclamped(const DevScene &sc, f3 p)
{
    const float x = fmaf(p.x, sc.sx, -0.5f), y = fmaf(p.y, sc.sy, -0.5f), z = fmaf(p.z, sc.sz, -0.5f);
    const uint32_t ux = (uint32_t)(floor_to_int(x) + sc.brick_bias);
    const uint32_t uy = (uint32_t)(floor_to_int(y) + sc.brick_bias);
    const uint32_t uz = (uint32_t)(floor_to_int(z) + sc.brick_bias);
    const uint32_t brick = __umul24(uz >> 2, (uint32_t)sc.brick_gxy) + __umul24(uy >> 2, (uint32_t)sc.brick_gx) + (ux >> 2);
    const uint32_t local = __umul24(uz & 3u, 25u) + __umul24(uy & 3u, 5u) + (ux & 3u);
#ifdef CT_DEBUG_BOUNDS
    if ((ux >> 2) >= (uint32_t)sc.brick_gx || (uy >> 2) >= (uint32_t)sc.brick_gy || (uz >> 2) >= (uint32_t)sc.brick_gz) {
        printf("CT_DEBUG_BOUNDS unclamped footprint texel (%u,%u,%u) outside the brick grid\n", ux, uy, uz);
        return 0;
    }
#endif
    return ((size_t)brick << 7) | local;
}
struct RawCell {
    uint2 a, c;
};
CT_DEV RawCell load_raw_apron(const uint8_t *q)
{
    RawCell r;
    __builtin_memcpy(&r.a, q, 8);
    __builtin_memcpy(&r.c, q + 25, 8);
    return r;
}
CT_DEV uint2 combine_apron(const RawCell &r)
{
    return make_uint2(__builtin_amdgcn_perm(r.a.y, r.a.x, 0x06050100u), __builtin_amdgcn_perm(r.c.y, r.c.x, 0x06050100u));
}
CT_DEV size_t twin_offset_in_grid(const DevScene &sc, f3 p)
{
    const float x = fmaf(p.x, sc.sx, -0.5f), y = fmaf(p.y, sc.sy, -0.5f), z = fmaf(p.z, sc.sz, -0.5f);
    const int32_t lo = -sc.t_bias;
    const uint32_t ux = (uint32_t)(min(max(floor_to_int(x), lo), 3 * sc.t_gx - 1 + lo) + sc.t_bias);
    const uint32_t uy = (uint32_t)(min(max(floor_to_int(y), lo), 3 * sc.t_gy - 1 + lo) + sc.t_bias);
    const uint32_t uz = (uint32_t)(min(max(floor_to_int(z), lo), 3 * sc.t_gz - 1 + lo) + sc.t_bias);
    const uint32_t bx = __umul24(ux, 43691u) >> 17, by = __umul24(uy, 43691u) >> 17, bz = __umul24(uz, 43691u) >> 17;
    const uint32_t lx = ux - __umul24(bx, 3u), ly = uy - __umul24(by, 3u), lz = uz - __umul24(bz, 3u);
    const uint32_t brick = __umul24(__umul24(bz, (uint32_t)sc.t_gy) + by, (uint32_t)sc.t_gx) + bx;
    const uint32_t local = (lz << 4) + (ly << 2) + lx;
#ifdef CT_DEBUG_BOUNDS
    if (bx >= (uint32_t)sc.t_gx || by >= (uint32_t)sc.t_gy || bz >= (uint32_t)sc.t_gz) {
        printf("CT_DEBUG_BOUNDS twin-brick texel (%u,%u,%u) outside the grid\n", ux, uy, uz);
        return 0;
    }
#endif
    return ((size_t)brick << 7) | local;
}
CT_DEV size_t twin_offset_unclamped(const DevScene &sc, f3 p)
{
    const float x = fmaf(p.x, sc.sx, -0.5f), y = fmaf(p.y, sc.sy, -0.5f), z = fmaf(p.z, sc.sz, -0.5f);
    const uint32_t ux = (uint32_t)(floor_to_int(x) + sc.t_bias);
    const uint32_t uy = (uint32_t)(floor_to_int(y) + sc.t_bias);
    const uint32_t uz = (uint32_t)(floor_to_int(z) + sc.t_bias);
    const uint32_t bx = __umul24(ux, 43691u) >> 17, by = __umul24(uy, 43691u) >> 17, bz = __umul24(uz, 43691u) >> 17;
    const uint32_t lx = ux - __umul24(bx, 3u), ly = uy - __umul24(by, 3u), lz = uz - __umul24(bz, 3u);
    const uint32_t brick = __umul24(__umul24(bz, (uint32_t)sc.t_gy) + by, (uint32_t)sc.t_gx) + bx;
    const uint32_t local = (lz << 4) + (ly << 2) + lx;
#ifdef CT_DEBUG_BOUNDS
    if (bx >= (uint32_t)sc.t_gx || by >= (uint32_t)sc.t_gy || bz >= (uint32_t)sc.t_gz) {
        printf("CT_DEBUG_BOUNDS unclamped twin-brick texel (%u,%u,%u) outside the grid\n", ux, uy, uz);
        return 0;
    }
#endif
    return ((size_t)brick << 7) | local;
}
CT_DEV RawCell load_raw_twin(const uint8_t *q)
{
    RawCell r;
    __builtin_memcpy(&r.a, q, 8);
    __builtin_memcpy(&r.c, q + 14, 8);
    return r;
}
CT_DEV uint2 combine_twin(const RawCell &r)
{
    return make_uint2(__builtin_amdgcn_perm(r.a.y, r.a.x, 0x05040100u), __builtin_amdgcn_perm(r.c.y, r.c.x, 0x07060302u));
}

CT_DEV uint2 fetch_cell_cached(const DevScene &sc, const uint8_t *bricks, f3 p, uint32_t &key, uint2 &cached, bool &reused,
                               bool zero = false)
{
    const float fx = fmaf(p.x, sc.sx, -0.5f), fy = fmaf(p.y, sc.sy, -0.5f), fz = fmaf(p.z, sc.sz, -0.5f);
    const uint32_t x = (uint32_t)(floor_to_int(fx) + sc.brick_bias), y = (uint32_t)(floor_to_int(fy) + sc.brick_bias),
                   z = (uint32_t)(floor_to_int(fz) + sc.brick_bias);
    const uint32_t brick = __umul24(z >> 2, (uint32_t)sc.brick_gxy) + __umul24(y >> 2, (uint32_t)sc.brick_gx) + (x >> 2);
    const uint32_t local = __umul24(z & 3u, 25u) + __umul24(y & 3u, 5u) + (x & 3u);
    const uint32_t off = (brick << 7) | local;
    reused = sc.nee_cache != 0u && off == key;
    if (!reused && !zero) {
        const uint8_t *q = bricks + (((size_t)brick << 7) | local);
        uint2 a, c;
        __builtin_memcpy(&a, q, 8);
        __builtin_memcpy(&c, q + 25, 8);
        cached.x = __builtin_amdgcn_perm(a.y, a.x, 0x06050100u);
        cached.y = __builtin_amdgcn_perm(c.y, c.x, 0x06050100u);
        key = off;
    }
    return zero ? make_uint2(0u, 0u) : cached;
}

template <bool SPARSE>
CT_DEV uint2 fetch_cell_m(const DevScene &sc, f3 p, uint32_t &meta)
{
    const float x = fmaf(p.x, sc.sx, -0.5f), y = fmaf(p.y, sc.sy, -0.5f), z = fmaf(p.z, sc.sz, -0.5f);
    return load_footprint_m<SPARSE>(sc, floor_to_int(x), floor_to_int(y), floor_to_int(z), meta);
}

template <bool FIXED8>
CT_DEV float filter_at(const DevScene &sc, uint2 cell, f3 p)
{
    const float x = fmaf(p.x, sc.sx, -0.5f), y = fmaf(p.y, sc.sy, -0.5f), z = fmaf(p.z, sc.sz, -0.5f);
    return filter_cell(cell, tex_weight<FIXED8>(x), tex_weight<FIXED8>(y), tex_weight<FIXED8>(z));
}

template <bool FIXED8>
CT_DEV float tex3_clamped(const DevScene &sc, const uint8_t *bricks, f3 p)
{
    const float x = fmaf(p.x, sc.sx, -0.5f), y = fmaf(p.y, sc.sy, -0.5f), z = fmaf(p.z, sc.sz, -0.5f);
    const float flx = floorf(x), fly = floorf(y), flz = floorf(z);
    const int32_t ix = (int32_t)fminf(fmaxf(flx, -1.0f), (float)(sc.nx - 1));
    const int32_t iy = (int32_t)fminf(fmaxf(fly, -1.0f), (float)(sc.ny - 1));
    const int32_t iz = (int32_t)fminf(fmaxf(flz, -1.0f), (float)(sc.nz - 1));
    const uint2 c = load_footprint(sc, bricks, ix, iy, iz);
    return filter_cell(c, tex_weight<FIXED8>(x), tex_weight<FIXED8>(y), tex_weight<FIXED8>(z));
}

template <bool FIXED8, typename Ptr>
CT_DEV float tex1(Ptr t, float u)
{
    const float x = fmaf(u, (float)kMieN, -0.5f);
    const float fl = floorf(x);
    const int32_t i = (int32_t)fl;
    const int32_t i0 = min(max(i, 0), kMieN - 1);
    const int32_t i1 = min(max(i + 1, 0), kMieN - 1);
    const float a = t[i0], b = t[i1];
    return fmaf(tex_weight<FIXED8>(x), b - a, a);
}

template <typename CdfPtr, typename GuidePtr>
CT_DEV float sample_cos_theta(CdfPtr cdf, GuidePtr guide, uint32_t u24)
{
    const float val = u24_to_float(u24);
    const uint32_t bucket = u24 >> 12;
    uint32_t lo = guide[bucket], hi = guide[bucket + 1];
    while (lo < hi) {
        const uint32_t mid = (lo + hi) >> 1;
        if (cdf[mid] < val) {
            lo = mid + 1;
        } else {
            hi = mid;
        }
    }
    const uint32_t t = lo;
    uint32_t k = 0;
    if (t != 0) {
        const float a = cdf[t - 1];
        const float b = cdf[min(t, (uint32_t)kMieN - 1)];
        const float d = b - a;
        uint32_t s = 0;
#pragma unroll
        for (uint32_t bit = 8; bit != 0; bit >>= 1) {
            const uint32_t cand = s | bit;
            const float f = fmaf((float)cand * 0.0625f, d, a);
            s = (f < val) ? cand : s;
        }
        k = min(16u * (t - 1) + 8u + s, 65535u);
    }
    return (float)(2u * k + 1u) * (1.0f / 65536.0f) - 1.0f;
}

template <typename CdfPtr, typename GuidePtr>
CT_DEV f3 new_direction(CdfPtr cdf, GuidePtr guide, uint32_t &seed, f3 prev)
{
    const float cos_theta = sample_cos_theta(cdf, guide, lcg24(seed));
    const float phi = u24_to_float(lcg24(seed)) * kPi * 2;
    const float sin_theta = sqrt_moderate(1 - cos_theta * cos_theta);
    float sn, cs;
    ct_sincosf(phi, &sn, &cs);
    const float px = sin_theta * cs, py = sin_theta * sn, pz = cos_theta;
    f3 b;
    if (fabsf(prev.x) > fabsf(prev.z)) {
        b = mk3(-prev.y, prev.x, 0.0f);
    } else {
        b = mk3(0.0f, -prev.z, prev.y);
    }
    b = normalize3_unitish(b);
    const f3 tg = cross3(b, prev);
    const f3 r = add3(add3(scale3(tg, px), scale3(b, py)), scale3(prev, pz));
    return normalize3_unitish(r);
}

CT_DEV bool intersect_box(const DevScene &sc, f3 o, f3 d, float &t_hit)
{
    const float nxh = -sc.bx / 2, nyh = -sc.by / 2, nzh = -sc.bz / 2;
    const float pxh = sc.bx / 2, pyh = sc.by / 2, pzh = sc.bz / 2;
    const float t0x = (nxh - o.x) / d.x, t0y = (nyh - o.y) / d.y, t0z = (nzh - o.z) / d.z;
    const float t1x = (pxh - o.x) / d.x, t1y = (pyh - o.y) / d.y, t1z = (pzh - o.z) / d.z;
    const float tmin = fmaxf(fmaxf(fminf(t0x, t1x), fminf(t0y, t1y)), fminf(t0z, t1z));
    const float tmax = fminf(fminf(fmaxf(t0x, t1x), fmaxf(t0y, t1y)), fmaxf(t0z, t1z));
    if (tmin <= tmax) {
        if (tmin > 0.0f && tmin < 1e27f) {
            t_hit = tmin;
            return true;
        }
        t_hit = 0.000001f;
        return true;
    }
    return false;
}

CT_DEV float logf_above_one(float x)
{
    const uint32_t u = ct_float_to_bits(x);
    int32_t e = (int32_t)(u >> 23) - 126;
    float m = ct_bits_to_float((u & 0x007fffffu) | 0x3f000000u);
    if (m < 0.707106781186547524f) {
        e -= 1;
        m = (m + m) - 1.0f;
    } else {
        m = m - 1.0f;
    }
    const float z = m * m;
    float p = 7.0376836292e-2f;
    p = fmaf(p, m, -1.1514610310e-1f);
    p = fmaf(p, m, 1.1676998740e-1f);
    p = fmaf(p, m, -1.2420140846e-1f);
    p = fmaf(p, m, 1.4249322787e-1f);
    p = fmaf(p, m, -1.6668057665e-1f);
    p = fmaf(p, m, 2.0000714765e-1f);
    p = fmaf(p, m, -2.4999993993e-1f);
    p = fmaf(p, m, 3.3333331174e-1f);
    const float fe = (float)e;
    float y = (p * m) * z;
    y = fmaf(fe, -2.12194440e-4f, y);
    y = fmaf(-0.5f, z, y);
    return fmaf(fe, 0.693359375f, m + y);
}

CT_DEV float expf_inrange(float x)
{
    const float n = rintf(x * 1.44269504088896341f);
    float r = fmaf(n, -0.693359375f, x);
    r = fmaf(n, 2.12194440e-4f, r);
    float p = 1.9875691500e-4f;
    p = fmaf(p, r, 1.3981999507e-3f);
    p = fmaf(p, r, 8.3334519073e-3f);
    p = fmaf(p, r, 4.1665795894e-2f);
    p = fmaf(p, r, 1.6666665459e-1f);
    p = fmaf(p, r, 5.0000001201e-1f);
    const float y = fmaf(p, r * r, r) + 1.0f;
    return y * ct_bits_to_float((uint32_t)((int32_t)n + 127) << 23);
}

}
```

deepestscatter_amd/csrc/ct_handle.hpp:

```cpp
#pragma once

#include <algorithm>
#include <array>
#include <cstdlib>
#include <string>
#include <utility>
#include <vector>

#include "../../include/cloudtrace.h"
#include "ct_internal.hpp"

using namespace ct;

struct Knob {
    bool is_set = false;
    std::string text;
    const char *get() const { return is_set ? text.c_str() : nullptr; }
    explicit operator bool() const { return is_set; }
};
#define CT_KNOBS(X) X(BURST_IDLE) X(BURST_MARCH_MIN) X(BURST_SCATTER) X(CHUNK_INTERLEAVE) X(CHUNK_MORTON) X(CONTINUATION) X(DEBUG_INVARIANTS) X(DELTA_INTERIOR) X(DELTA_NEE) X(EXCHANGE) X(HAND_ON_JOBS) X(HINT_PERIOD) X(JOB_MAX) X(JOB_WORK) X(MARCH_BURST) X(MAX_AGE) X(NEE_CACHE) X(NET_DESC_RECORDS) X(NO_ADVANCE) X(POINT_BLOCKS_PER_CU) X(POINT_ORDER) X(REGEN_MIN) X(RENDER_AHEAD) X(SCATTER_MIN) X(SCATTER_RATIO) X(SCRATCH_GIB) X(SCRATCH_MIB) X(SERPENTINE) X(SHARED_DEPTH) X(SPARSE) X(STATS) X(TAIL_BURST) X(TILE_ORDER) X(TIMELINE) X(TRACE) X(TUNE_SUBFRAMES) X(XCD_QUEUES) X(XCD_QUEUES_UNTUNED) X(XCD_REGIONS) X(BLOCKS_PER_CU)
struct CtTuning {
#define X(name) Knob name;
    CT_KNOBS(X)
#undef X
    static CtTuning from_env()
    {
        CtTuning t;
#define X(name)                                  \
    if (const char *e = getenv("CT_" #name)) {   \
        t.name.is_set = true;                    \
        t.name.text = e;                         \
    }
        CT_KNOBS(X)
#undef X
        return t;
    }
};

inline int knob_int(const Knob &k, int lo, int hi, int dflt)
{
    return k ? std::min(hi, std::max(lo, atoi(k.get()))) : dflt;
}

inline bool knob_flag(const Knob &k, bool dflt)
{
    return k ? atoi(k.get()) != 0 : dflt;
}

struct CtHandle_ {
    CtTuning tune;
    CtScene scene{};
    int device = 0;
    hipStream_t own_stream = nullptr;
    hipStream_t stream = nullptr;
    hipEvent_t ev[3] = { nullptr, nullptr, nullptr };

    DevScene dev{};
    bool camera_set = false;

    uint8_t *d_density = nullptr, *d_inscatter = nullptr, *d_dist = nullptr, *d_dist_tmp = nullptr, *d_majorant = nullptr, *d_maj_cells = nullptr, *d_maj_codes = nullptr;
    uint8_t *d_dbricks = nullptr, *d_ibricks = nullptr, *d_mbricks = nullptr, *d_tbricks = nullptr;
    uint2 *d_mrows = nullptr;
    uint8_t *d_mcoarse = nullptr;
    size_t mbricks_dense_bytes = 0, mbricks_bytes = 0;
    int nee_skip_r = 0;
    uint32_t zero_faces = 0;
    bool mie_finite = true;
    struct VmmBricks {
        void *va = nullptr;
        size_t size = 0, chunk = 0;
        std::vector<hipMemGenericAllocationHandle_t> handles;
        size_t real_chunks = 0, shared_chunks = 0, mapped_chunks = 0;
    } vmm;
    uint8_t *d_pyramid = nullptr;
    MipPyramid pyramid{};
    float *d_mie = nullptr, *d_chopped = nullptr, *d_cdf = nullptr;
    uint16_t *d_guide = nullptr;
    float4 *d_frame = nullptr, *d_mean = nullptr, *d_m2 = nullptr;
    uchar4 *d_screen = nullptr;
    static constexpr int kMaxRegions = 64;
    struct Slot {
        uint32_t *queue = nullptr;
        hipEvent_t ev_in = nullptr, ev_start = nullptr, ev_done = nullptr, ev_acc0 = nullptr, ev_acc1 = nullptr;
        bool pending = false;
        bool accumulated = false;
        bool awaits_accumulate = false;
        bool complete = false;
        uint32_t acc_done = 0;
        uint32_t first = 0, S = 0;
        uint32_t rank_base = 0, groups = 0;
        bool with_misses = false;
        bool last_chunk = true;
    };
    Slot slots[kMaxRegions];
    int n_regions = 2;
    int next_slot = 0;
    std::vector<int> waiting;
    uint32_t ahead = 0;
    uint32_t rendered = 0;
    uint32_t stop_cadence = 0, stop_min = 100;
    uint32_t *d_freeze = nullptr, *freeze_host = nullptr;
    uint32_t *cont[2] = { nullptr, nullptr };
    uint64_t launch_no = 0;
    bool cont_live = false;
    float4 *d_frames_all = nullptr;
    size_t frames_total = 0;
    size_t slot_capacity = 0;
    uint64_t scratch_cap_bytes = 0;
    uint32_t layout_S = 0;
    uint32_t *left[2] = { nullptr, nullptr };
    size_t left_capacity = 0;
    uint32_t *d_cont_count = nullptr;
    unsigned long long *d_cont_total = nullptr;
    size_t cont_capacity = 0;
    hipEvent_t ev_flush0 = nullptr, ev_flush1 = nullptr;
    bool continuation = true;
    int max_age_override = 0;
    bool hand_on_jobs = true;
    bool serpentine = false;
    float4 *d_primary = nullptr;
    float4 *d_advance = nullptr;
    uint32_t *d_pixels = nullptr;
    uint8_t *d_hit = nullptr, *hit_host = nullptr;
    uint32_t *d_cost = nullptr;
    uint32_t *d_touched[2] = { nullptr, nullptr };
    size_t touched_lines[2] = { 0, 0 };
    unsigned long long *d_timeline = nullptr;
    uint2 *d_cost_plane = nullptr;
    size_t cost_plane_capacity = 0;
    uint32_t *d_job_group = nullptr, *d_job_sub = nullptr;
    uint32_t n_groups = 0, groups_capacity = 0;
    uint32_t n_jobs = 0, jobs_capacity = 0, jobs_S = 0;
    uint32_t *jobs_host_g = nullptr, *jobs_host_s = nullptr;
    size_t jobs_host_capacity = 0;
    bool jobs_brief = false;
    uint32_t chunk_groups = 0, n_chunks = 0;
    std::vector<std::array<uint32_t, kQueues + 2>> chunk_q_begin;
    uint32_t *d_group_rank = nullptr, *d_group_order = nullptr;
    uint32_t jobs_hint = 0;
    uint32_t job_max = 16;
    float job_work = 16.f;
    uint32_t q_begin[kQueues + 2] = {};
    uint64_t own_pixels = 0, hit_pixels = 0;
    bool queue_dirty = true, order_tuned = false;
    bool no_advance = false;
    bool queues_enabled = false;
    float shared_depth = 1e30f;
    uint32_t regions = 128;
    std::vector<uint32_t> group_order;
    std::vector<uint32_t> group_tile;
    std::vector<uint32_t> tile_deepest;
    std::vector<uint32_t> job_order;
    bool chunk_interleave = false;
    bool chunk_morton = false;
    bool tile_hilbert = false;
    std::vector<float> group_depth;
    unsigned long long host_paths = 0, host_hits = 0;
    uint32_t *d_queue = nullptr;
    unsigned long long *d_counters = nullptr;
    float *d_colsum = nullptr, *d_avg = nullptr;
    uint32_t reinhard_generation = 0;

    bool debug_invariants = false;
    uint64_t iv_expected_dealt = 0, iv_checks = 0, iv_violations = 0;

    struct PointBuffers {
        CtPointRadianceTask *tasks = nullptr;
        float4 *primary = nullptr, *frames = nullptr;
        uint32_t *pixels = nullptr, *jg = nullptr, *js = nullptr;
        size_t cap_tasks = 0, cap_primary = 0, cap_pixels = 0, cap_frames = 0, cap_jg = 0, cap_js = 0;
    } pt;
    bool point_order = true;

    size_t volume_bytes = 0;
    LaunchShape shape{ 1024, 256, false };
    int exchange = 0;
    LaunchShape xshape{ 256, 1024, false };
    uint32_t subframes = 0;
    double render_ms = 0, accum_ms = 0;
    double dframe_scatter_ms = 0, dframe_gather_ms = 0;
    struct NetScratch {
        float4 *found = nullptr, *direct = nullptr;
        uint32_t *waves = nullptr;
        float *pos = nullptr, *dir = nullptr, *aux = nullptr, *out = nullptr;
        uint8_t *desc = nullptr;
        size_t band_cap = 0, desc_cap = 0, direct_cap = 0;
        double ms[4] = { 0, 0, 0, 0 };
        uint32_t *tiles = nullptr;
        uint32_t n_tiles = 0;
        bool tiles_built = false;
    } net;
    uint64_t launches = 0;
    std::string error;
};

namespace ct {

int fail(CtHandle h, int code, const char *fmt, ...);

int flush(CtHandle h);
void discard_ahead(CtHandle h);
int enqueue_convergence_test(CtHandle h, uint32_t subframes);

int ensure_pyramid(CtHandle h);

}

#define HIPCHK(h, expr)                                                                              \
    do {                                                                                             \
        hipError_t e_ = (expr);                                                                      \
        if (e_ != hipSuccess) {                                                                      \
            return fail((h), e_ == hipErrorOutOfMemory ? CT_E_NOMEM : CT_E_HIP, "%s failed: %s", #expr, \
                        hipGetErrorString(e_));                                                      \
        }                                                                                            \
    } while (0)

#define NEED_NOFLUSH(h)                                \
    do {                                               \
        if (!(h)) {                                    \
            return fail(nullptr, CT_E_INVAL, "null handle"); \
        }                                              \
        if (hipSetDevice((h)->device) != hipSuccess) { \
            return fail((h), CT_E_HIP, "hipSetDevice(%d) failed", (h)->device); \
        }                                              \
        (void)hipGetLastError();  \
    } while (0)

#define NEED(h)                                        \
    do {                                               \
        NEED_NOFLUSH(h);                               \
        const int rc_flush_ = flush(h);                \
        if (rc_flush_ != CT_OK) {                      \
            return rc_flush_;                          \
        }                                              \
    } while (0)

template <typename T>
hipError_t dmalloc(T **p, size_t count)
{
    return hipMalloc((void **)p, count * sizeof(T));
}

template <typename T>
struct DevTemp {
    T *p = nullptr;
    DevTemp() = default;
    DevTemp(DevTemp &&o) noexcept : p(std::exchange(o.p, nullptr)) {}
    ~DevTemp()
    {
        if (p) {
            hipFree(p);
        }
    }
    operator T *() const { return p; }
    T *release() { return std::exchange(p, nullptr); }
};

template <typename T>
hipError_t dmalloc(DevTemp<T> *t, size_t count)
{
    return dmalloc(&t->p, count);
}
```

deepestscatter_amd/csrc/ct_internal.hpp:

```cpp
#pragma once

#include <hip/hip_runtime.h>
#include <stdint.h>

#include "ct_device.hpp"

namespace ct {

constexpr int kTile = 8;
constexpr int kCounterCount = 9;
constexpr int kStatCount = 73;
constexpr int kContWords = 16;
constexpr int kContWordsDelta = 32;
constexpr int kLeftWords = 8;
constexpr int kQueueFlag = 32;
constexpr int kQueueDone = 16;
constexpr int kQueueWords = 64;
constexpr int kQueues = 8;

struct BatchArgs {
    float4 *frames;
    uint32_t frame_stride;
    const float4 *primary;
    const float4 *advance;
    const uint32_t *pixels;
    const uint32_t *group_rank;
    uint32_t rank_base;
    const uint32_t *job_group;
    const uint32_t *job_sub;
    uint2 *cost;
    uint32_t n_jobs;
    uint32_t q_begin[kQueues + 2];
    uint32_t reverse;
    uint32_t first_subframe;
    uint32_t S;
    uint32_t *queue;
    const uint32_t *cont_in;
    const uint32_t *cont_in_count;
    uint32_t *cont_cursor;
    uint32_t *cont_out;
    uint32_t *cont_out_count;
    uint32_t cont_capacity;
    uint32_t max_age;
    unsigned long long *cont_total;
    const uint32_t *left_in;
    const uint32_t *left_in_count;
    uint32_t *left_cursor;
    uint32_t *left_out;
    uint32_t *left_out_count;
    uint32_t left_capacity;
    uint32_t out_offset;
    unsigned long long *counters;
    unsigned long long *stats;
    unsigned long long *timeline;
    uint32_t *touched_density, *touched_shadow;
};

struct LaunchShape {
    int blocks;
    int threads;
    bool stats;
    uint32_t pool_slots = 0;
    uint32_t scatter_waves = 0;
};

inline void split_queues_evenly(BatchArgs &ba)
{
    for (int x = 0; x <= kQueues; x++) {
        ba.q_begin[x] = (uint32_t)(((uint64_t)ba.n_jobs * (uint32_t)x) / kQueues);
    }
    ba.q_begin[kQueues + 1] = ba.n_jobs;
}

#ifndef CT_SHARD_SHIFT
#define CT_SHARD_SHIFT 0
#endif
__host__ __device__ inline uint32_t tile_owner(uint32_t tx, uint32_t ty, uint32_t shard_count)
{
    return shard_count <= 1 ? 0u : ((tx >> CT_SHARD_SHIFT) + 3u * (ty >> CT_SHARD_SHIFT)) % shard_count;
}

hipError_t launch_build_bricks(const uint8_t *texels, int nx, int ny, int nz, int bias, int gx, int gy, int gz,
                               uint8_t *bricks, hipStream_t stream);
hipError_t launch_build_twin_bricks(const uint8_t *density, const uint8_t *shadow, int nx, int ny, int nz, int bias, int gx, int gy, int gz,
                                    uint8_t *bricks, hipStream_t stream);
hipError_t launch_build_dist(const uint8_t *texels, int nx, int ny, int nz, int bias, int gx, int gy, int gz,
                             uint8_t *dist, uint8_t *scratch, uint8_t *majorant, hipStream_t stream);
hipError_t launch_majorant_cells(const uint8_t *texels, int nx, int ny, int nz, int bias, int cell, const int origin[3], int gx, int gy, int gz,
                                 uint8_t *out, uint8_t *out_codes, hipStream_t stream);
hipError_t launch_brick_meta(const uint8_t *dist, const uint8_t *majorant, int nx, int ny, int nz, int bias, int gx,
                             int gy, int gz, uint8_t *bricks, hipStream_t stream);
hipError_t launch_build_mbricks(const uint8_t *texels, int nx, int ny, int nz, int bias_x, int bias, int gx, int gy,
                                int gz, uint8_t *tmp_a, uint8_t *tmp_b, uint8_t *bricks, hipStream_t stream);
#ifdef CT_EXPERIMENTS
hipError_t launch_mbrick_chunk_class(const uint8_t *bricks, int64_t total_bytes, int64_t chunk_bytes, uint4 *out, hipStream_t stream);
hipError_t launch_mbrick_chunk_quantize(uint8_t *chunk, int64_t chunk_bytes, hipStream_t stream);
#endif
hipError_t launch_mbrick_extent(const uint8_t *bricks, int gx, int gy, int gz, uint32_t *row_x0, uint32_t *row_x1, hipStream_t stream);
hipError_t launch_mbrick_compact(const uint8_t *dense, int gx, int gy, int gz, const uint2 *rows, uint8_t *compact, hipStream_t stream);
hipError_t launch_nee_skip_flags(const uint8_t *shadow, int nx, int ny, int nz, int r, int bias_x, int bias, int gx, int gy,
                                 int gz, uint8_t *tmp_a, uint8_t *tmp_c, uint8_t *bricks, hipStream_t stream);
hipError_t launch_shadow_zero_rows(const uint8_t *shadow, int nx, int ny, int nz, int r, int bias_x, int bias, int gx, int gy, int gz,
                                   uint8_t *tmp_a, uint8_t *tmp_c, uint8_t *bricks, const uint2 *rows, hipStream_t stream);
hipError_t launch_twin_shadow_half(const uint8_t *shadow, int nx, int ny, int nz, int bias, int gx, int gy, int gz, uint8_t *bricks,
                                   hipStream_t stream);
hipError_t launch_coarse_clearance(const uint8_t *dist, int nx, int ny, int nz, int bias, int cshift, int cgx, int cgy, int cgz,
                                   uint8_t *out, hipStream_t stream);
hipError_t launch_render_delta(const DevScene &sc, const BatchArgs &ba, LaunchShape shape, hipStream_t stream);
hipError_t launch_inscatter(const DevScene &sc, uint8_t *out, uint32_t zero_faces, hipStream_t stream);
hipError_t launch_primary_rays(const DevScene &sc, float4 *primary, hipStream_t stream);
hipError_t launch_cost_reduce(const uint2 *cost_plane, uint32_t frame_stride, uint32_t S, uint32_t n_groups_in_chunk,
                              const uint32_t *group_order, uint32_t rank_base, uint32_t *cost_sum, uint32_t *cost_deepest,
                              hipStream_t stream);
hipError_t launch_hit_flags(const float4 *primary, uint8_t *flags, uint32_t pixels, hipStream_t stream);
hipError_t launch_primary_advance(const DevScene &sc, const float4 *primary, float4 *advance, hipStream_t stream);
hipError_t launch_primary_advance_delta(const DevScene &sc, const float4 *primary, float4 *advance, hipStream_t stream);
struct ZeroList {
    uint32_t *ptr[6];
    uint32_t words[6];
    int n = 0;
    void add(uint32_t *p, uint32_t w) { ptr[n] = p; words[n] = w; n += 1; }
};
hipError_t launch_zero_words(const ZeroList &z, hipStream_t stream);
hipError_t launch_fill_frame(float4 *frame, uint32_t width, uint32_t height, uint32_t shard_index,
                             uint32_t shard_count, hipStream_t stream);
hipError_t launch_render_persistent(const DevScene &sc, const BatchArgs &ba, LaunchShape shape, hipStream_t stream);
hipError_t launch_render_simple(const DevScene &sc, const BatchArgs &ba, uint32_t shard_index,
                                uint32_t shard_count, hipStream_t stream);
hipError_t launch_accumulate_batch(const float4 *frames, float4 *mean, float4 *m2, uint32_t first_subframe,
                                   uint32_t S, uint32_t width, uint32_t height, uint32_t shard_index,
                                   uint32_t shard_count, unsigned long long *bad_samples, const uint32_t *frozen,
                                   hipStream_t stream);
hipError_t launch_accumulate_list(const float4 *frames, uint32_t frame_stride, const uint32_t *pixels,
                                  uint32_t n_entries, const uint32_t *group_order, uint32_t rank_base, bool with_misses,
                                  const float4 *primary, float4 *mean, float4 *m2,
                                  uint32_t first_subframe, uint32_t S, uint32_t width, uint32_t height,
                                  uint32_t shard_index, uint32_t shard_count, unsigned long long *bad_samples,
                                  const uint32_t *frozen, hipStream_t stream);
hipError_t launch_reinhard(const float4 *mean, uint32_t width, uint32_t height, float exposure,
                           float *column_sums, float *avg, uchar4 *screen, uint32_t *generation, int device, hipStream_t stream);
hipError_t launch_converged(const float4 *mean, const float4 *m2, uint32_t subframe_id, uint64_t pixels,
                            unsigned long long *unconverged, hipStream_t stream);
hipError_t launch_converged_freeze(const float4 *mean, const float4 *m2, uint32_t subframe_id, uint64_t pixels,
                                   uint32_t limit, uint32_t *state, hipStream_t stream);
hipError_t launch_cdf_selftest(const float *cdf, const uint16_t *guide, uint32_t first_u24, uint32_t count,
                               uint32_t *k_out, hipStream_t stream);
hipError_t launch_math_selftest(int which, uint32_t lo_bits, uint32_t hi_bits, unsigned long long *out, hipStream_t stream);
hipError_t launch_fetch_probe(const uint8_t *buf, uint32_t log2_lines, uint32_t second_offset,
                              unsigned long long *sum, hipStream_t stream);
hipError_t launch_fetch_probe_ws(const uint8_t *buf, uint32_t log2_threads, uint32_t ws_lines, uint32_t salt, unsigned long long *sum,
                                 hipStream_t stream);
hipError_t launch_point_rays(const DevScene &sc, const void *tasks, uint32_t n, uint32_t n_pad, float4 *primary,
                             uint32_t *pixels, hipStream_t stream);
hipError_t launch_point_accumulate(const float4 *frames, uint32_t stride, void *tasks, uint32_t n, uint32_t launches,
                                   hipStream_t stream);
hipError_t launch_scatter_samples(const DevScene &sc, uint32_t count, uint32_t batch_seed, float *positions,
                                  float *directions, hipStream_t stream);
struct PixelBand {
    uint32_t x0, y0, w;
    uint32_t n;
    const uint32_t *tiles;
    uint32_t tiles_x, width, height;
};
inline PixelBand rect_band(uint32_t x0, uint32_t y0, uint32_t w, uint32_t rows)
{
    return { x0, y0, w, w * rows, nullptr, 0u, 0u, 0u };
}
inline PixelBand tile_band(const DevScene &sc, const uint32_t *tiles, uint32_t count)
{
    return { 0u, 0u, 0u, 64u * count, tiles, sc.tiles_x, sc.width, sc.height };
}
struct FlightTemps {
    float4 *found;
    uint32_t *waves;
    float4 *direct;
};
hipError_t launch_first_scatter_frame(const DevScene &sc, const PixelBand &band, const FlightTemps &t, uint32_t subframe_id,
                                      uint32_t capacity, float *positions, float *directions, uint32_t *pixels, hipStream_t stream);
struct NetCompose {
    int32_t transform;
    float sr, sg, sb;
};
struct ComposeTarget {
    float4 *frame;
    float4 *mean, *m2;
    uint32_t subframe_id;
};
hipError_t launch_network_aux(const float *directions, uint32_t count, float lx, float ly, float lz, float *aux, hipStream_t stream);
hipError_t launch_network_compose(const PixelBand &band, const FlightTemps &t, const NetCompose &c, const float *out,
                                  const ComposeTarget &dst, const uint32_t *frozen, hipStream_t stream);
constexpr int kMaxMipLevels = 16;
struct MipPyramid {
    const uint8_t *base;
    uint32_t levels;
    uint32_t offset[kMaxMipLevels];
    int32_t nx[kMaxMipLevels], ny[kMaxMipLevels], nz[kMaxMipLevels];
};
hipError_t launch_mip_level(const uint8_t *prev, int px, int py, int pz, uint8_t *cur, int cx, int cy, int cz,
                            hipStream_t stream);
hipError_t launch_descriptors(const DevScene &sc, const MipPyramid &mp, const float *positions, const float *directions,
                              uint32_t count, float level0, float voxel_m, float cloud_size_m, uint8_t *out,
                              hipStream_t stream);
LaunchShape persistent_shape(int device, bool delta, int blocks_per_cu = 0);
#ifdef CT_EXPERIMENTS
LaunchShape exchange_shape(int device);
hipError_t launch_render_delta_x(const DevScene &sc, const BatchArgs &ba, LaunchShape shape, hipStream_t stream);
LaunchShape wave_exchange_shape(int device);
hipError_t launch_render_delta_w(const DevScene &sc, const BatchArgs &ba, LaunchShape shape, hipStream_t stream);
#endif

}
```

deepestscatter_amd/csrc/ct_kernels.hip:

```cpp
#include <algorithm>
#include <cstdlib>

#include "ct_internal.hpp"

namespace ct {

__global__ void build_bricks_kernel(const uint8_t *__restrict__ t, int nx, int ny, int nz, int bias,
                                    uint8_t *__restrict__ bricks, int gx, int gy, int gz)
{
    const int64_t total = (int64_t)gx * gy * gz * 128;
    for (int64_t i = (int64_t)blockIdx.x * blockDim.x + threadIdx.x; i < total; i += (int64_t)gridDim.x * blockDim.x) {
        const int64_t b = i >> 7;
        const int o = (int)(i & 127);
        uint8_t v = 0;
        if (o < 125) {
            const int lx = o % 5, ly = (o / 5) % 5, lz = o / 25;
            const int x = (int)(b % gx) * 4 + lx - bias;
            const int y = (int)((b / gx) % gy) * 4 + ly - bias;
            const int z = (int)(b / ((int64_t)gx * gy)) * 4 + lz - bias;
            const int xc = min(max(x, 0), nx - 1), yc = min(max(y, 0), ny - 1), zc = min(max(z, 0), nz - 1);
            v = t[((size_t)zc * ny + yc) * nx + xc];
        }
        bricks[i] = v;
    }
// ... 416 lines not shown
}

__global__ void coarse_clearance_kernel(const uint8_t *__restrict__ dist, int nx, int ny, int nz, int bias, int cshift, int cgx,
                                        int cgy, int cgz, uint8_t *__restrict__ out)
{
    const int64_t total = (int64_t)cgx * cgy * cgz;
    const int C = 1 << cshift;
    for (int64_t i = (int64_t)blockIdx.x * blockDim.x + threadIdx.x; i < total; i += (int64_t)gridDim.x * blockDim.x) {
        const int cx = (int)(i % cgx), cy = (int)((i / cgx) % cgy), cz = (int)(i / ((int64_t)cgx * cgy));
        const int x0 = cx * C - bias, y0 = cy * C - bias, z0 = cz * C - bias;
        int c = kClearMax;
        bool interior = true;
        for (int z = z0; z < z0 + C; z++) {
            for (int y = y0; y < y0 + C; y++) {
                for (int x = x0; x < x0 + C; x++) {
                    const bool in_grid = x >= 0 && y >= 0 && z >= 0 && x < nx && y < ny && z < nz;
                    const int d = in_grid ? (int)dist[((size_t)z * ny + y) * nx + x] : 0;
                    c = min(c, d - 1);
                    interior = interior && x >= 1 && y >= 1 && z >= 1 && x <= nx - 3 && y <= ny - 3 && z <= nz - 3;
                }
            }
        }
        out[i] = (uint8_t)(max(c, 0) | (interior ? 0x80 : 0));
    }
}

hipError_t launch_mbrick_extent(const uint8_t *bricks, int gx, int gy, int gz, uint32_t *row_x0, uint32_t *row_x1, hipStream_t stream)
{
    const int64_t total = (int64_t)gx * gy * gz;
    const int blocks = (int)std::min<int64_t>((total + 255) / 256, 65536 * 4);
    hipLaunchKernelGGL(mbrick_extent_kernel, dim3(blocks), dim3(256), 0, stream, bricks, gx, gy, gz, row_x0, row_x1);
    return hipGetLastError();
}

hipError_t launch_mbrick_compact(const uint8_t *dense, int gx, int gy, int gz, const uint2 *rows, uint8_t *compact, hipStream_t stream)
{
    const int64_t total = (int64_t)gx * gy * gz;
    const int blocks = (int)std::min<int64_t>((total * 8 + 255) / 256, 65536 * 8);
    hipLaunchKernelGGL(mbrick_compact_kernel, dim3(blocks), dim3(256), 0, stream, (const uint4 *)dense, gx, total, rows, (uint4 *)compact);
    return hipGetLastError();
}

hipError_t launch_coarse_clearance(const uint8_t *dist, int nx, int ny, int nz, int bias, int cshift, int cgx, int cgy, int cgz,
                                   uint8_t *out, hipStream_t stream)
{
    const int64_t total = (int64_t)cgx * cgy * cgz;
    const int blocks = (int)std::min<int64_t>((total + 255) / 256, 65536 * 4);
    hipLaunchKernelGGL(coarse_clearance_kernel, dim3(blocks), dim3(256), 0, stream, dist, nx, ny, nz, bias, cshift, cgx, cgy, cgz, out);
    return hipGetLastError();
}

constexpr int kDistMax = 64;

__global__ void brick_free_kernel(const uint8_t *__restrict__ t, int nx, int ny, int nz, int bias, int gx, int gy,
                                  int gz, uint8_t *__restrict__ dist, uint8_t *__restrict__ majorant)
{
    const int b = blockIdx.x * blockDim.x + threadIdx.x;
    if (b >= gx * gy * gz) {
        return;
    }
    const int bx = b % gx, by = (b / gx) % gy, bz = b / (gx * gy);
    const int x0 = bx * kBrick - bias, y0 = by * kBrick - bias, z0 = bz * kBrick - bias;
    const bool interior = x0 >= 1 && y0 >= 1 && z0 >= 1 && x0 + kBrick - 1 <= nx - 3 && y0 + kBrick - 1 <= ny - 3 &&
                          z0 + kBrick - 1 <= nz - 3;
    int m = 0;
    for (int z = z0 - 1; z <= z0 + kBrick + 1; z++) {
        const int zc = min(max(z, 0), nz - 1);
        for (int y = y0 - 1; y <= y0 + kBrick + 1; y++) {
            const uint8_t *row = t + ((size_t)zc * ny + min(max(y, 0), ny - 1)) * nx;
            for (int x = x0 - 1; x <= x0 + kBrick + 1; x++) {
                m = max(m, (int)row[min(max(x, 0), nx - 1)]);
            }
        }
    }
    majorant[b] = (uint8_t)m;
    dist[b] = (interior && m == 0) ? (uint8_t)kDistMax : (uint8_t)0;
}

__global__ void brick_meta_kernel(const uint8_t *__restrict__ dist, const uint8_t *__restrict__ majorant, int nx,
                                  int ny, int nz, int bias, int gx, int gy, int gz, uint8_t *__restrict__ bricks)
{
    const int b = blockIdx.x * blockDim.x + threadIdx.x;
    if (b >= gx * gy * gz) {
        return;
    }
    const int bx = b % gx, by = (b / gx) % gy, bz = b / (gx * gy);
    const int x0 = bx * kBrick - bias, y0 = by * kBrick - bias, z0 = bz * kBrick - bias;
    const bool interior = x0 >= 1 && y0 >= 1 && z0 >= 1 && x0 + kBrick - 1 <= nx - 3 && y0 + kBrick - 1 <= ny - 3 &&
                          z0 + kBrick - 1 <= nz - 3;
    bricks[((size_t)b << 7) + 125] = (uint8_t)(min((int)dist[b], 127) | (interior ? 0x80 : 0));
    bricks[((size_t)b << 7) + 126] = majorant[b];
}

__global__ void brick_dist_relax_kernel(const uint8_t *__restrict__ in, uint8_t *__restrict__ out, int gx, int gy,
                                        int gz)
{
    const int b = blockIdx.x * blockDim.x + threadIdx.x;
    if (b >= gx * gy * gz) {
        return;
    }
    const int bx = b % gx, by = (b / gx) % gy, bz = b / (gx * gy);
    int m = 255;
    for (int dz = -1; dz <= 1; dz++) {
        for (int dy = -1; dy <= 1; dy++) {
            for (int dx = -1; dx <= 1; dx++) {
                const int x = bx + dx, y = by + dy, z = bz + dz;
                const int v = (x < 0 || y < 0 || z < 0 || x >= gx || y >= gy || z >= gz)
                                  ? 0
                                  : (int)in[((size_t)z * gy + y) * gx + x];
                m = min(m, v);
            }
        }
    }
    out[b] = (uint8_t)min((int)in[b], m + 1);
}

hipError_t launch_build_dist(const uint8_t *texels, int nx, int ny, int nz, int bias, int gx, int gy, int gz,
                             uint8_t *dist, uint8_t *scratch, uint8_t *majorant, hipStream_t stream)
{
    const int total = gx * gy * gz;
    const int threads = 256, blocks = (total + threads - 1) / threads;
    hipLaunchKernelGGL(brick_free_kernel, dim3(blocks), dim3(threads), 0, stream, texels, nx, ny, nz, bias, gx, gy,
                       gz, dist, majorant);
    uint8_t *a = dist, *b = scratch;
    for (int i = 0; i < kDistMax; i++) {
        hipLaunchKernelGGL(brick_dist_relax_kernel, dim3(blocks), dim3(threads), 0, stream, a, b, gx, gy, gz);
        uint8_t *tmp = a;
        a = b;
        b = tmp;
    }
    if (a != dist) {
        hipError_t e = hipMemcpyAsync(dist, a, (size_t)total, hipMemcpyDeviceToDevice, stream);
        if (e != hipSuccess) {
            return e;
        }
    }
    return hipGetLastError();
}

hipError_t launch_brick_meta(const uint8_t *dist, const uint8_t *majorant, int nx, int ny, int nz, int bias, int gx,
                             int gy, int gz, uint8_t *bricks, hipStream_t stream)
{
    const int total = gx * gy * gz;
    hipLaunchKernelGGL(brick_meta_kernel, dim3((total + 255) / 256), dim3(256), 0, stream, dist, majorant, nx, ny, nz,
                       bias, gx, gy, gz, bricks);
    return hipGetLastError();
}

struct MieLds {
    float cdf[kMieN];
    uint16_t guide[kGuideN + 2];
};

struct MieLdsFull {
    float cdf[kMieN];
    float chopped[kMieN];
    uint16_t guide[kGuideN + 2];
};

CT_DEV void load_tables(const DevScene &sc, MieLdsFull &lds)
{
    for (int i = threadIdx.x; i < kMieN; i += blockDim.x) {
        lds.cdf[i] = sc.cdf[i];
        lds.chopped[i] = sc.chopped[i];
    }
    for (int i = threadIdx.x; i < kGuideN + 2; i += blockDim.x) {
        lds.guide[i] = sc.guide[i];
    }
    __syncthreads();
}

CT_DEV void load_tables(const DevScene &sc, MieLds &lds)
{
    for (int i = threadIdx.x; i < kMieN; i += blockDim.x) {
        lds.cdf[i] = sc.cdf[i];
    }
    for (int i = threadIdx.x; i < kGuideN + 2; i += blockDim.x) {
        lds.guide[i] = sc.guide[i];
    }
    __syncthreads();
}

CT_DEV f3 primary_direction(const DevScene &sc, uint32_t x, uint32_t y)
{
    const float dx = (float)x / (float)sc.width * 2.f - 1.f;
    const float dy = (float)y / (float)sc.height * 2.f - 1.f;
    const f3 U = mk3(sc.ux, sc.uy, sc.uz), V = mk3(sc.vx, sc.vy, sc.vz), W = mk3(sc.wx, sc.wy, sc.wz);
    return normalize3(add3(add3(scale3(U, dx), scale3(V, dy)), W));
}

__global__ __launch_bounds__(256) void primary_rays_kernel(DevScene sc, float4 *__restrict__ primary)
{
    const uint32_t x = blockIdx.x * 32u + (threadIdx.x & 31u);
    const uint32_t y = blockIdx.y * 8u + (threadIdx.x >> 5);
    if (x >= sc.width || y >= sc.height) {
        return;
    }
    const f3 eye = mk3(sc.ex, sc.ey, sc.ez);
    const f3 d = primary_direction(sc, x, y);
    float t_hit = 0;
    const bool hit = intersect_box(sc, eye, d, t_hit);
    f3 pos = add3(eye, scale3(d, t_hit));
    pos = add3(pos, scale3(mk3(sc.bx, sc.by, sc.bz), 0.5f));
    const f3 dir = normalize3(d);
    const size_t p = (size_t)y * sc.width + x;
    primary[2 * p] = make_float4(pos.x, pos.y, pos.z, hit ? 1.f : 0.f);
    primary[2 * p + 1] = make_float4(dir.x, dir.y, dir.z, __uint_as_float(x * 4096u + y));
}

hipError_t launch_primary_rays(const DevScene &sc, float4 *primary, hipStream_t stream)
{
    const dim3 grid((sc.width + 31) / 32, (sc.height + 7) / 8), block(256);
    hipLaunchKernelGGL(primary_rays_kernel, grid, block, 0, stream, sc, primary);
    return hipGetLastError();
}

__global__ __launch_bounds__(256) void hit_flags_kernel(const float4 *__restrict__ primary, uint8_t *__restrict__ flags, uint32_t pixels)
{
    const uint32_t p = blockIdx.x * blockDim.x + threadIdx.x;
    if (p < pixels) {
        flags[p] = primary[2 * (size_t)p].w != 0.f ? 1u : 0u;
    }
}

__global__ __launch_bounds__(64) void cost_reduce_kernel(const uint2 *__restrict__ plane, uint32_t frame_stride, uint32_t S,
                                                         const uint32_t *__restrict__ group_order, uint32_t rank_base,
                                                         uint32_t *__restrict__ cost_sum, uint32_t *__restrict__ cost_deepest)
{
    const uint32_t c = blockIdx.x, lane = threadIdx.x;
    uint32_t sum = 0, deepest = 0;
    for (uint32_t s = 0; s < S; s++) {
        const uint2 v = plane[(size_t)s * frame_stride + c * 64u + lane];
        sum += v.x;
        deepest = max(deepest, v.y);
    }
#pragma unroll
    for (int off = 32; off > 0; off >>= 1) {
        sum += __shfl_xor(sum, off);
        deepest = max(deepest, (uint32_t)__shfl_xor((int)deepest, off));
    }
    if (lane == 0) {
        const uint32_t g = group_order ? group_order[rank_base + c] : c;
        cost_sum[g] += sum;
        cost_deepest[g] = max(cost_deepest[g], deepest);
    }
}

hipError_t launch_cost_reduce(const uint2 *cost_plane, uint32_t frame_stride, uint32_t S, uint32_t n_groups_in_chunk,
                              const uint32_t *group_order, uint32_t rank_base, uint32_t *cost_sum, uint32_t *cost_deepest,
                              hipStream_t stream)
{
    if (n_groups_in_chunk != 0u && S != 0u) {
        hipLaunchKernelGGL(cost_reduce_kernel, dim3(n_groups_in_chunk), dim3(64), 0, stream, cost_plane, frame_stride, S, group_order,
                           rank_base, cost_sum, cost_deepest);
    }
    return hipGetLastError();
}

hipError_t launch_hit_flags(const float4 *primary, uint8_t *flags, uint32_t pixels, hipStream_t stream)
{
    hipLaunchKernelGGL(hit_flags_kernel, dim3((pixels + 255u) / 256u), dim3(256), 0, stream, primary, flags, pixels);
    return hipGetLastError();
}

struct PointTask {
    int32_t id;
    uint32_t experimentCount;
    float radiance, runningVariance;
    float px, py, pz, dx, dy, dz;
};

__global__ __launch_bounds__(256) void point_rays_kernel(DevScene sc, const PointTask *__restrict__ tasks, uint32_t n,
                                                         uint32_t n_pad, float4 *__restrict__ primary,
                                                         uint32_t *__restrict__ pixels)
{
    const uint32_t i = blockIdx.x * blockDim.x + threadIdx.x;
    if (i >= n_pad) {
        return;
    }
    if (i >= n) {
        pixels[i] = 0xffffffffu;
        return;
    }
    pixels[i] = i;
    const PointTask t = tasks[i];
    const f3 o = mk3(t.px, t.py, t.pz), d = mk3(t.dx, t.dy, t.dz);
    float t_hit = 0;
    const bool hit = intersect_box(sc, o, d, t_hit);
    f3 pos = add3(o, scale3(d, t_hit));
    pos = add3(pos, scale3(mk3(sc.bx, sc.by, sc.bz), 0.5f));
    const f3 dir = normalize3(d);
    primary[2 * (size_t)i] = make_float4(pos.x, pos.y, pos.z, hit ? 1.f : 0.f);
    primary[2 * (size_t)i + 1] = make_float4(dir.x, dir.y, dir.z, __uint_as_float(i * 4096u));
}

__global__ __launch_bounds__(256) void point_accumulate_kernel(const float4 *__restrict__ frames, uint32_t stride,
                                                               PointTask *__restrict__ tasks, uint32_t n,
                                                               uint32_t launches)
{
    const uint32_t i = blockIdx.x * blockDim.x + threadIdx.x;
    if (i >= n) {
        return;
    }
    PointTask t = tasks[i];
    for (uint32_t f = 0; f < launches; f++) {
        const float new_radiance = frames[(size_t)f * stride + i].x;
        t.experimentCount++;
        const float N = (float)t.experimentCount;
        const float new_weight = (float)(1.0 / (double)N);
        const float previous_mean = t.radiance;
        const float new_mean = t.radiance + (new_radiance - previous_mean) * new_weight;
        t.radiance = new_mean;
        t.runningVariance += (new_radiance - previous_mean) * (new_radiance - new_mean);
    }
    tasks[i] = t;
}

hipError_t launch_point_rays(const DevScene &sc, const void *tasks, uint32_t n, uint32_t n_pad, float4 *primary,
                             uint32_t *pixels, hipStream_t stream)
{
    hipLaunchKernelGGL(point_rays_kernel, dim3((n_pad + 255) / 256), dim3(256), 0, stream, sc,
                       (const PointTask *)tasks, n, n_pad, primary, pixels);
    return hipGetLastError();
}

hipError_t launch_point_accumulate(const float4 *frames, uint32_t stride, void *tasks, uint32_t n, uint32_t launches,
                                   hipStream_t stream)
{
    hipLaunchKernelGGL(point_accumulate_kernel, dim3((n + 255) / 256), dim3(256), 0, stream, frames, stride,
                       (PointTask *)tasks, n, launches);
    return hipGetLastError();
}

__global__ void fill_frame_kernel(float4 *__restrict__ frame, uint32_t width, uint32_t height, uint32_t shard_index,
                                  uint32_t shard_count)
{
    const uint32_t x = blockIdx.x * 32u + (threadIdx.x & 31u);
    const uint32_t y = blockIdx.y * 8u + (threadIdx.x >> 5);
    if (x >= width || y >= height) {
        return;
    }
    const bool own = tile_owner(x / kTile, y / kTile, shard_count) == shard_index;
    frame[(size_t)y * width + x] = make_float4(0.f, 0.f, 0.f, own ? 1.f : 0.f);
}

__global__ __launch_bounds__(64) void zero_words_kernel(ZeroList z)
{
    for (int k = 0; k < z.n; k++) {
        for (uint32_t i = threadIdx.x; i < z.words[k]; i += 64u) {
            z.ptr[k][i] = 0u;
        }
    }
}

hipError_t launch_zero_words(const ZeroList &z, hipStream_t stream)
{
    if (z.n > 0) {
        hipLaunchKernelGGL(zero_words_kernel, dim3(1), dim3(64), 0, stream, z);
    }
    return hipGetLastError();
}

hipError_t launch_fill_frame(float4 *frame, uint32_t width, uint32_t height, uint32_t shard_index,
                             uint32_t shard_count, hipStream_t stream)
{
    const dim3 grid((width + 31) / 32, (height + 7) / 8), block(256);
    hipLaunchKernelGGL(fill_frame_kernel, grid, block, 0, stream, frame, width, height, shard_index, shard_count);
    return hipGetLastError();
}

template <bool FIXED8>
CT_DEV f3 in_scattering(const DevScene &sc, f3 pos, f3 dir, bool chopped)
{
    const float cos_light = dot3(mk3(sc.nlx, sc.nly, sc.nlz), dir);
    const float u = (cos_light + 1) / 2;
    const float *table = chopped ? sc.chopped : sc.mie;
    const float phase = tex1<FIXED8>(table, u);
    const float ins = tex3_apron<FIXED8>(sc, sc.ibricks, pos);
    f3 l = scale3(mk3(sc.lr, sc.lg, sc.lb), ins);
    l = scale3(l, phase);
    return scale3(l, sc.sun_ratio);
}

struct NeeLoads {
    float a, b, w;
    uint2 cell;
};

template <bool FIXED8>
CT_DEV NeeLoads in_scattering_issue(const DevScene &sc, f3 pos, f3 dir, bool chopped)
{
    NeeLoads n;
    const float cos_light = dot3(mk3(sc.nlx, sc.nly, sc.nlz), dir);
    const float u = (cos_light + 1) / 2;
    const float *table = chopped ? sc.chopped : sc.mie;
    const float x = fmaf(u, (float)kMieN, -0.5f);
    const int32_t i = (int32_t)floorf(x);
    float2 pair;
    __builtin_memcpy(&pair, table + min(max(i, 0), kMieN - 2), sizeof pair);
    n.a = (i > kMieN - 2) ? pair.y : pair.x;
    n.b = (i < 0) ? pair.x : pair.y;
    n.w = tex_weight<FIXED8>(x);
    uint32_t meta_unused;
    n.cell = fetch_cell(sc, sc.ibricks, pos, meta_unused);
    return n;
}

template <bool FIXED8>
CT_DEV NeeLoads in_scattering_issue_phase(const DevScene &sc, f3 dir, bool chopped)
{
    NeeLoads n;
    const float cos_light = dot3(mk3(sc.nlx, sc.nly, sc.nlz), dir);
    const float u = (cos_light + 1) / 2;
    const float *table = chopped ? sc.chopped : sc.mie;
    const float x = fmaf(u, (float)kMieN, -0.5f);
    const int32_t i = (int32_t)floorf(x);
    float2 pair;
    __builtin_memcpy(&pair, table + min(max(i, 0), kMieN - 2), sizeof pair);
    n.a = (i > kMieN - 2) ? pair.y : pair.x;
    n.b = (i < 0) ? pair.x : pair.y;
    n.w = tex_weight<FIXED8>(x);
    n.cell = make_uint2(0u, 0u);
    return n;
}

template <bool FIXED8>
CT_DEV NeeLoads in_scattering_issue_lds(const DevScene &sc, const float *lds_chopped, f3 pos, f3 dir, bool chopped,
                                        uint32_t &nee_key, uint2 &nee_cell, bool &reused, bool zero = false)
{
    NeeLoads n;
    const float cos_light = dot3(mk3(sc.nlx, sc.nly, sc.nlz), dir);
    const float u = (cos_light + 1) / 2;
    const float x = fmaf(u, (float)kMieN, -0.5f);
    const int32_t i = (int32_t)floorf(x);
    const int32_t j = min(max(i, 0), kMieN - 2);
    float2 pair;
    if (chopped) {
        pair = make_float2(lds_chopped[j], lds_chopped[j + 1]);
    } else {
        __builtin_memcpy(&pair, sc.mie + j, sizeof pair);
    }
    n.a = (i > kMieN - 2) ? pair.y : pair.x;
    n.b = (i < 0) ? pair.x : pair.y;
    n.w = tex_weight<FIXED8>(x);
    n.cell = fetch_cell_cached(sc, sc.ibricks, pos, nee_key, nee_cell, reused, zero);
    return n;
}

template <bool FIXED8>
CT_DEV f3 in_scattering_finish(const DevScene &sc, const NeeLoads &n, f3 pos)
{
    const float phase = fmaf(n.w, n.b - n.a, n.a);
    const float ins = filter_at<FIXED8>(sc, n.cell, pos);
    f3 l = scale3(mk3(sc.lr, sc.lg, sc.lb), ins);
    l = scale3(l, phase);
    return scale3(l, sc.sun_ratio);
}

enum : int { ST_IDLE = 0, ST_MARCH = 1, ST_BOUNCE = 2 };

#ifndef CT_MARCH_FLAT_ZERO
#define CT_MARCH_FLAT_ZERO 1
#endif
#ifndef CT_MARCH_FLAT_EXIT
#define CT_MARCH_FLAT_EXIT 1
#endif
#ifndef CT_MARCH_FUSE
#define CT_MARCH_FUSE 1
#endif
constexpr bool MARCH_FUSE = CT_MARCH_FUSE != 0;
#ifndef CT_MARCH_NEE_SKIP
#define CT_MARCH_NEE_SKIP 1
#endif

CT_DEV float inv_max_advance(const DevScene &sc, f3 stepv)
{
    const float m = fmaxf(fmaxf(fabsf(stepv.x) * sc.sx, fabsf(stepv.y) * sc.sy), fabsf(stepv.z) * sc.sz);
    return __builtin_amdgcn_rcpf(fmaxf(m, 1e-20f));
}


CT_DEV int skip_steps(uint32_t c, float inv_maxd)
{
    return (int)(((float)c - 0.03125f) * inv_maxd);
}

CT_DEV void replay_steps(f3 &pos, f3 stepv, int n)
{
    int i = 0;
    for (; i + 8 <= n; i += 8) {
#pragma unroll
        for (int k = 0; k < 8; k++) {
            pos = add3(pos, stepv);
        }
    }
    for (; i < n; i++) {
        pos = add3(pos, stepv);
    }
}

template <bool FIXED8, bool SPARSE = false>
__global__ __launch_bounds__(256) void inscatter_kernel(DevScene sc, uint8_t *__restrict__ out, uint32_t zero_faces)
{
    const int64_t total = (int64_t)sc.nx * sc.ny * sc.nz;
    const int64_t i = (int64_t)blockIdx.x * blockDim.x + threadIdx.x;
    if (i >= total) {
        return;
    }
    const int x = (int)(i % sc.nx), y = (int)((i / sc.nx) % sc.ny), z = (int)(i / ((int64_t)sc.nx * sc.ny));
    const float max_size = (float)max(max(sc.nx, sc.ny), sc.nz);
    const float tsx = max_size / (float)sc.nx, tsy = max_size / (float)sc.ny, tsz = max_size / (float)sc.nz;
    const float min_scale = fminf(fminf(tsx, tsy), tsz);
    const float inv_min_scale = 1.0f / min_scale;
    f3 p = mk3((float)x / max_size, (float)y / max_size, (float)z / max_size);
    p = scale3(p, inv_min_scale);
    const f3 step_to_light = scale3(normalize3(mk3(sc.nlx, sc.nly, sc.nlz)), sc.sample_step);
    const int step_count = (int)(1 / sc.sample_step);
    float transmittance = 1;
    int s = 0;
    bool done = false;
    if (sc.mbricks != nullptr && (SPARSE || sc.m_rows == nullptr)) {
        const float inv_maxd = inv_max_advance(sc, step_to_light);
        while (s < step_count && in_box(sc, p)) {
            uint32_t meta;
            const uint2 cell = fetch_cell_m<SPARSE>(sc, p, meta);
            if ((cell.x | cell.y) != 0u) {
                const float density = filter_at<FIXED8>(sc, cell, p) * sc.density_multiplier;
                const float extinction = density * sc.sample_step;
                transmittance *= ct_expf(-extinction);
                if (transmittance * 255.f < 1.f) {
                    done = true;
                    break;
                }
            }
            p = add3(p, step_to_light);
            s += 1;
            const uint32_t clear = meta & 0x3fu;
            if (clear != 0u) {
                const int n = min(skip_steps(clear, inv_maxd), step_count - s);
                replay_steps(p, step_to_light, n);
                s += n;
            }
        }
    }
    for (; !done && s < step_count; s++) {
        const float tx = fmaf(p.x, sc.sx, -0.5f), ty = fmaf(p.y, sc.sy, -0.5f), tz = fmaf(p.z, sc.sz, -0.5f);
        const bool gone = ((zero_faces & 1u) && tx < 0.0f && step_to_light.x <= 0.0f) ||
                          ((zero_faces & 2u) && tx >= (float)(sc.nx - 1) && step_to_light.x >= 0.0f) ||
                          ((zero_faces & 4u) && ty < 0.0f && step_to_light.y <= 0.0f) ||
                          ((zero_faces & 8u) && ty >= (float)(sc.ny - 1) && step_to_light.y >= 0.0f) ||
                          ((zero_faces & 16u) && tz < 0.0f && step_to_light.z <= 0.0f) ||
                          ((zero_faces & 32u) && tz >= (float)(sc.nz - 1) && step_to_light.z >= 0.0f);
        if (gone) {
            break;
        }
        const float density = tex3_clamped<FIXED8>(sc, sc.dbricks, p) * sc.density_multiplier;
        const float extinction = density * sc.sample_step;
        transmittance *= ct_expf(-extinction);
        p = add3(p, step_to_light);
        if (transmittance * 255.f < 1.f) {
            break;
        }
    }
    out[i] = (uint8_t)(transmittance * 255.f);
}

hipError_t launch_inscatter(const DevScene &sc, uint8_t *out, uint32_t zero_faces, hipStream_t stream)
{
    const int64_t total = (int64_t)sc.nx * sc.ny * sc.nz;
    const int threads = 256;
    const int64_t blocks = (total + threads - 1) / threads;
    const dim3 grid((unsigned)blocks), block(threads);
    if (sc.mbricks != nullptr && sc.m_rows != nullptr) {
        if (sc.tex_fixed8) {
            hipLaunchKernelGGL((inscatter_kernel<true, true>), grid, block, 0, stream, sc, out, zero_faces);
        } else {
            hipLaunchKernelGGL((inscatter_kernel<false, true>), grid, block, 0, stream, sc, out, zero_faces);
        }
    } else if (sc.tex_fixed8) {
        hipLaunchKernelGGL(inscatter_kernel<true>, grid, block, 0, stream, sc, out, zero_faces);
    } else {
        hipLaunchKernelGGL(inscatter_kernel<false>, grid, block, 0, stream, sc, out, zero_faces);
    }
    return hipGetLastError();
}

#include "ct_sched.hpp"

template <bool SPARSE>
__global__ __launch_bounds__(256) void primary_advance_kernel(DevScene sc, const float4 *__restrict__ primary,
                                                              float4 *__restrict__ advance)
{
    const uint32_t x = blockIdx.x * 32u + (threadIdx.x & 31u);
    const uint32_t y = blockIdx.y * 8u + (threadIdx.x >> 5);
    if (x >= sc.width || y >= sc.height) {
        return;
    }
    const size_t p = (size_t)y * sc.width + x;
    const float4 p0 = primary[2 * p], p1 = primary[2 * p + 1];
    f3 pos = mk3(p0.x, p0.y, p0.z);
    const f3 dir = mk3(p1.x, p1.y, p1.z);
    f3 start = pos;
    uint32_t start_bits = 0;
    if (p0.w != 0.f && in_box(sc, pos)) {
        const f3 stepv = scale3(dir, sc.sample_step);
        const float inv_maxd = inv_max_advance(sc, stepv);
        uint32_t dfree = 0, steps = 0;
        for (int it = 0; it < 65536 && steps < 0x00f00000u; it++) {
            start = pos;
            start_bits = steps | (dfree << 24);
            if (dfree != 0u) {
                const int n = skip_steps(dfree, inv_maxd);
                replay_steps(pos, stepv, n);
                steps += (uint32_t)n;
            }
            pos = add3(pos, stepv);
            steps += 1u;
            uint32_t meta;
            const uint2 cell = fetch_cell_m<SPARSE>(sc, pos, meta);
            dfree = meta & 0x3fu;
            if ((cell.x | cell.y) != 0u || ((meta & 0x80u) == 0u && !in_box(sc, pos))) {
                break;
            }
        }
    }
    advance[p] = make_float4(start.x, start.y, start.z, __uint_as_float(start_bits));
}

hipError_t launch_primary_advance(const DevScene &sc, const float4 *primary, float4 *advance, hipStream_t stream)
{
    const dim3 grid((sc.width + 31) / 32, (sc.height + 7) / 8), block(256);
    if (sc.m_rows) {
        hipLaunchKernelGGL(primary_advance_kernel<true>, grid, block, 0, stream, sc, primary, advance);
    } else {
        hipLaunchKernelGGL(primary_advance_kernel<false>, grid, block, 0, stream, sc, primary, advance);
    }
    return hipGetLastError();
}

template <int MODE, bool STATS, bool SPARSE, bool COST = true, bool FIXED8 = false>
__global__ __launch_bounds__(512) __attribute__((amdgpu_waves_per_eu(6))) void render_persistent_kernel(DevScene sc, BatchArgs ba)
{
    __shared__ MieLdsFull lds;
    load_tables(sc, lds);

    const uint32_t lane = threadIdx.x & 63u;
#ifdef CT_DIAG_TIMELINE
    if (ba.timeline && lane == 0u) {
        ba.timeline[4u * (blockIdx.x * (blockDim.x >> 6) + (threadIdx.x >> 6))] = wall_clock64();
    }
#endif
    f3 pos = mk3(0, 0, 0), dir = mk3(0, 0, 1), stepv = mk3(0, 0, 0), rad = mk3(0, 0, 0);
    uint32_t seed = 0, depth = 0, out_idx = 0;
    uint32_t work = 0;
    float xi = 0, T = 1;
    uint32_t dfree = 0;
    float inv_maxd = 0;
    int state = ST_IDLE;

    JobState job{ 0, 0, 0, 0, 0, 0 };
    bool left_done = false;
    uint32_t q_cur = (uint32_t)kQueues, q_tried = 0;
    bool drained = false;
    uint32_t c_dl = 0, c_il = 0, c_cap = 0;
    uint32_t w_fetch = 0, w_nee = 0;
    uint32_t iv_dealt = 0, iv_written = 0, iv_resumed = 0, iv_suspended = 0;
    uint32_t nee_key = 0xffffffffu;
    uint2 nee_cell = make_uint2(0u, 0u);
    uint32_t st_regen = 0, st_regen_l = 0, st_march = 0, st_march_l = 0, st_scat = 0, st_scat_l = 0;
    uint32_t st_fetch = 0, st_zero = 0, st_skip = 0, st_zero_d0 = 0, st_zero_d1 = 0, st_skip_iters = 0, st_stolen = 0, st_iters = 0, st_first = 0;
    uint32_t st_hit2 = 0, st_hit3 = 0, st_h2 = 0xffffffffu, st_h3 = 0xffffffffu;
    uint32_t st_same_line = 0, st_dup_line = 0, st_prev_line = 0xffffffffu;
    uint32_t st_nee_zero = 0;

    uint32_t age = 0;
    if (ba.cont_in) {
        const uint32_t total = __builtin_amdgcn_readfirstlane(*ba.cont_in_count);
        uint32_t base = 0;
        if (lane == 0) {
            base = atomicAdd(ba.cont_cursor, 64u);
        }
        base = __builtin_amdgcn_readfirstlane(base);
        if (base + lane < total) {
            const uint4 *e = (const uint4 *)(ba.cont_in + (size_t)(base + lane) * kContWords);
            const uint4 w0 = e[0], w1 = e[1], w2 = e[2], w3 = e[3];
            pos = mk3(__uint_as_float(w0.x), __uint_as_float(w0.y), __uint_as_float(w0.z));
            dir = mk3(__uint_as_float(w0.w), __uint_as_float(w1.x), __uint_as_float(w1.y));
            rad = mk3(__uint_as_float(w1.z), __uint_as_float(w1.w), __uint_as_float(w2.x));
            seed = w2.y;
            out_idx = w2.z;
            xi = __uint_as_float(w2.w);
            T = __uint_as_float(w3.x);
            inv_maxd = __uint_as_float(w3.y);
            depth = w3.z & 0xffffu;
            dfree = (w3.z >> 16) & 0xffu;
            state = (int)(w3.z >> 24);
            stepv = scale3(dir, sc.sample_step);
            age = w3.w;
            if (STATS) {
                iv_resumed += 1;
            }
        }
    }
    const bool may_suspend = ba.cont_out != nullptr;
    const bool single_queue = ba.q_begin[1] == ba.n_jobs;

    const unsigned long long t_start = STATS ? wall_clock64() : 0ull;
    unsigned long long t_drained = 0;
#ifdef CT_DIAG_TIMELINE
    bool tl_marked = false;
#endif
    uint32_t visit = 0;
    for (;;) {
        visit += 1;
        if (may_suspend && single_queue && !drained && sc.hint_period != 0u && (visit & (sc.hint_period - 1u)) == 0u) {
            const uint32_t empty = __builtin_amdgcn_readfirstlane(__atomic_load_n(ba.queue + kQueueFlag, __ATOMIC_RELAXED));
            if (empty != 0u) {
                if (job.next != job.end && ba.left_out && job.age < ba.max_age && hand_on_job(ba, lane, job)) {
                    job.next = job.end;
                }
                if (job.next == job.end) {
                    drained = true;
                }
            }
        }
#ifdef CT_DIAG_TIMELINE
        if (ba.timeline && drained && !tl_marked) {
            tl_marked = true;
            const uint32_t live = (uint32_t)__builtin_popcountll(__builtin_amdgcn_ballot_w64(state != ST_IDLE));
            const uint32_t old = (uint32_t)__builtin_popcountll(__builtin_amdgcn_ballot_w64(state != ST_IDLE && age >= ba.max_age));
            if (lane == 0u) {
                unsigned long long *tl = ba.timeline + 4u * (blockIdx.x * (blockDim.x >> 6) + (threadIdx.x >> 6));
                tl[2] = wall_clock64();
                tl[3] = live | (old << 8) | ((job.next != job.end ? 1u : 0u) << 16);
            }
        }
#endif
        if (STATS) {
            st_iters += 1;
            if (drained && t_drained == 0) {
                t_drained = wall_clock64();
            }
        }
        const uint64_t idle = __builtin_amdgcn_ballot_w64(state == ST_IDLE);
        const uint32_t n_idle = (uint32_t)__builtin_popcountll(idle);
        if ((n_idle >= sc.regen_min || n_idle == 64u) && !(drained && job.next == job.end)) {
            if (job.next == job.end && !take_leftover(ba, lane, left_done, job)) {
                uint32_t j = 0;
                if (!take_job(ba, lane, q_cur, q_tried, j)) {
                    drained = true;
                } else {
                    if (STATS) {
                        st_stolen += (q_tried != 0u) ? 1u : 0u;
                    }
                    const uint32_t sub = __builtin_amdgcn_readfirstlane(ba.job_sub[j]);
                    const uint32_t s0 = sub & 0xffffu;
                    job.g = __builtin_amdgcn_readfirstlane(ba.job_group[j]);
                    job.next = 0;
                    job.end = (s0 < ba.S ? min(sub >> 16, ba.S - s0) : 0u) * 64u;
                    job.base = ba.out_offset + s0 * ba.frame_stride + group_column(ba, job.g);
                    job.first = ba.first_subframe + s0;
                    job.age = 0;
                }
            }
            if (job.next != job.end) {
                const uint32_t avail = job.end - job.next;
                if (STATS) {
                    st_regen += 1;
                    st_regen_l += min(n_idle, avail);
                }
                const uint32_t rank = lane_rank(idle);
                const bool take = (state == ST_IDLE) && rank < avail;
                const uint32_t q = job.next + rank;
                job.next += min(n_idle, avail);
                if (take) {
                    const uint32_t s = q >> 6, l = q & 63u;
                    const uint32_t g = job.g;
                    const uint32_t pixel = ba.pixels[g * 64u + l];
                    if (pixel != 0xffffffffu) {
                        if (STATS) {
                            iv_dealt += 1;
                        }
                        const float4 p0 = ba.primary[2 * (size_t)pixel];
                        const float4 p1 = ba.primary[2 * (size_t)pixel + 1];
                        out_idx = ba.frame_stride ? job.base + s * ba.frame_stride + l : pixel;
                        pos = mk3(p0.x, p0.y, p0.z);
                        const bool hit = p0.w != 0.f;
                        dir = mk3(p1.x, p1.y, p1.z);
                        seed = tea4(__float_as_uint(p1.w), job.first + s);
                        rad = mk3(0, 0, 0);
                        depth = 0;
                        work = 0;
                        age = job.age;
                        if (MODE == 1) {
                            dir = new_direction(lds.cdf, lds.guide, seed, dir);
                        }
                        bool go = hit && in_box(sc, pos);
                        if (MODE != 2 && go) {
                            depth = 1;
                            if (depth == sc.max_depth) {
                                c_cap += 1;
                                go = false;
                            }
                        }
                        if (go) {
                            xi = u24_to_float(lcg24(seed));
                            T = 1;
                            stepv = scale3(dir, sc.sample_step);
                            inv_maxd = inv_max_advance(sc, stepv);
                            dfree = 0;
                            if (MODE != 1 && ba.advance) {
                                const float4 a = ba.advance[pixel];
                                const uint32_t bits = __float_as_uint(a.w);
                                pos = mk3(a.x, a.y, a.z);
                                dfree = bits >> 24;
                                c_dl += bits & 0x00ffffffu;
                            }
                            state = ST_MARCH;
                        } else {
                            ba.frames[out_idx] = make_float4(0.f, 0.f, 0.f, 1.f);
                            if (STATS) {
                                iv_written += 1;
                            }
                        }
                    }
                }
            }
        }

        const uint64_t marching = __builtin_amdgcn_ballot_w64(state == ST_MARCH);
        const uint64_t bouncing = __builtin_amdgcn_ballot_w64(state == ST_BOUNCE);
        const uint32_t nm = (uint32_t)__builtin_popcountll(marching);
        const uint32_t nb = (uint32_t)__builtin_popcountll(bouncing);
        if ((marching | bouncing) == 0 && drained && job.next == job.end) {
            break;
        }

        bool finished = false;
        const bool do_scatter = nb * sc.scatter_den > nm * sc.scatter_num && (nb >= sc.scatter_min || nm == 0);
        if (do_scatter) {
            if (STATS) {
                st_scat += 1;
                st_scat_l += nb;
            }
            bool nee_fetched = false;
            if (state == ST_BOUNCE) {
                bool nee_zero = false;
                {
                    const float lg = logf_above_one(div_(xi, T));
                    const float inv = rcp_moderate(inv_maxd);
                    pos = sub3(pos, scale3(scale3(dir, lg), inv));
                    nee_zero = CT_MARCH_NEE_SKIP != 0 && (dfree & 0x40u) != 0u && lg * inv <= sc.nee_reach;
                }
                if ((dfree & 0x80u) != 0u || in_box(sc, pos)) {
                    const bool chopped = (MODE == 1) ? true : (MODE == 0 ? (depth != 1) : false);
                    bool nee_reused = false;
                    const uint32_t st_key_before = nee_key;
                    NeeLoads nee;
                    if (CT_MARCH_NEE_SKIP == 1) {
                        if (!nee_zero) {
                            nee = in_scattering_issue_lds<FIXED8>(sc, lds.chopped, pos, dir, chopped, nee_key, nee_cell, nee_reused);
                        }
                    } else {
                        nee = in_scattering_issue_lds<FIXED8>(sc, lds.chopped, pos, dir, chopped, nee_key, nee_cell, nee_reused, nee_zero);
                    }
                    if (STATS) {
                        st_nee_zero += nee_zero ? 1u : 0u;
                        nee_reused = nee_reused || nee_zero;
                    }
                    if (STATS && !nee_reused) {
                        st_hit2 += (nee_key == st_h2) ? 1u : 0u;
                        st_hit3 += (nee_key != st_h2 && nee_key == st_h3) ? 1u : 0u;
                        st_h3 = st_h2;
                        st_h2 = st_key_before;
                    }
                    nee_fetched = !nee_reused && !nee_zero;
                    if (STATS) {
                        st_first += nee_reused ? 1u : 0u;
                        if (ba.touched_shadow && !nee_reused) {
                            const uint32_t line = (uint32_t)(apron_offset_in_grid(sc, pos) >> 7);
                            atomicOr(&ba.touched_shadow[line >> 5], 1u << (line & 31u));
                        }
                    }
                    c_il += 1;
                    if (COST) {
                        work += 4u;
                    }
                    bool go = (MODE != 2);
                    if (go) {
                        dir = new_direction(lds.cdf, lds.guide, seed, dir);
                        depth++;
                        if (depth == sc.max_depth) {
                            c_cap += 1;
                            go = false;
                        }
                    }
                    if (CT_MARCH_NEE_SKIP != 1 || !nee_zero) {
                        rad = add3(rad, in_scattering_finish<FIXED8>(sc, nee, pos));
                    }
                    if (go) {
                        xi = u24_to_float(lcg24(seed));
                        T = 1;
                        stepv = scale3(dir, sc.sample_step);
                        inv_maxd = inv_max_advance(sc, stepv);
                        dfree = 0;
                        state = ST_MARCH;
                    } else {
                        finished = true;
                    }
                } else {
                    finished = true;
                }
            }
            w_nee += (uint32_t)__builtin_popcountll(__builtin_amdgcn_ballot_w64(nee_fetched));
        }
        bool track = !do_scatter;
        uint32_t nm_track = nm;
        if (do_scatter && MARCH_FUSE) {
            nm_track = (uint32_t)__builtin_popcountll(__builtin_amdgcn_ballot_w64(state == ST_MARCH));
            track = nm_track != 0u;
        }
        if (track) {
            if (STATS) {
                st_march += 1;
                st_march_l += nm_track;
            }
            w_fetch += nm_track;
            uint32_t burst = drained ? sc.tail_burst : sc.march_burst;
            for (;;) {
            if (state == ST_MARCH) {
                if (dfree != 0u) {
                    const int n = skip_steps(dfree, inv_maxd);
                    replay_steps(pos, stepv, n);
                    c_dl += (uint32_t)n;
                    if (STATS) {
                        st_skip += (uint32_t)n;
                        int wmax = n;
#pragma unroll
                        for (int off = 32; off > 0; off >>= 1) {
                            wmax = max(wmax, __shfl_xor(wmax, off));
                        }
                        st_skip_iters += (lane_rank(__builtin_amdgcn_ballot_w64(true)) == 0u) ? (uint32_t)wmax : 0u;
                    }
                }
                pos = add3(pos, stepv);
                uint32_t meta;
                const uint2 cell = fetch_cell_m<SPARSE>(sc, pos, meta);
                dfree = meta & 0x3fu;
                c_dl += 1;
                if (COST) {
                    work += 1u;
                }
                if (STATS) {
                    st_fetch += 1;
                    {
                        const float fx = fmaf(pos.x, sc.sx, -0.5f), fy = fmaf(pos.y, sc.sy, -0.5f), fz = fmaf(pos.z, sc.sz, -0.5f);
                        const uint32_t lx = (uint32_t)(floor_to_int(fx) + sc.m_bias_x), ly = (uint32_t)(floor_to_int(fy) + sc.brick_bias),
                                       lz = (uint32_t)(floor_to_int(fz) + sc.brick_bias);
                        const uint32_t line = __umul24(lz >> 2, (uint32_t)sc.m_gxy) + __umul24(ly >> 2, (uint32_t)sc.m_gx) + (__umul24(lx, 43691u) >> 17);
                        st_same_line += (line == st_prev_line) ? 1u : 0u;
                        st_prev_line = line;
                        if (ba.touched_density && !SPARSE) {
                            atomicOr(&ba.touched_density[line >> 5], 1u << (line & 31u));
                        }
                        const uint64_t act = __builtin_amdgcn_ballot_w64(true);
                        bool dup = false;
                        for (uint32_t i = 0; i < 64u; i++) {
                            const uint32_t other = (uint32_t)__builtin_amdgcn_readlane((int)line, (int)i);
                            dup = dup || (((act >> i) & 1ull) != 0ull && i < lane && other == line);
                        }
                        st_dup_line += dup ? 1u : 0u;
                    }
                    st_zero += ((cell.x | cell.y) == 0u) ? 1u : 0u;
                    st_zero_d0 += ((cell.x | cell.y) == 0u && dfree == 0u) ? 1u : 0u;
                    st_zero_d1 += ((cell.x | cell.y) == 0u && dfree == 1u) ? 1u : 0u;
                }
                bool collided = false;
                if (CT_MARCH_FLAT_ZERO || (cell.x | cell.y) != 0u) {
                    const float density = filter_at<FIXED8>(sc, cell, pos) * sc.density_multiplier;
                    const float extinction = density * sc.sample_step;
                    T *= expf_inrange(-extinction);
                    if (xi > T) {
                        collided = true;
                        inv_maxd = density;
                    }
                }
#if CT_MARCH_FLAT_EXIT
                state = collided ? ST_BOUNCE : state;
                dfree = collided ? (meta & 0xc0u) : dfree;
                if (!collided & ((meta & 0x80u) == 0u) & !in_box_flat(sc, pos)) {
#else
                if (collided) {
                    state = ST_BOUNCE;
                    dfree = meta & 0xc0u;
                } else if ((meta & 0x80u) == 0u && !in_box(sc, pos)) {
#endif
                    ba.frames[out_idx] = make_float4(rad.x, rad.y, rad.z, 1.f);
                    if (STATS) {
                        iv_written += 1;
                    }
                    if (COST && ba.cost) {
                        ba.cost[out_idx - ba.out_offset] = make_uint2(work, depth);
                    }
                    state = ST_IDLE;
                }
            }
            if (--burst == 0u) {
                break;
            }
            const uint32_t m_now = (uint32_t)__builtin_popcountll(__builtin_amdgcn_ballot_w64(state == ST_MARCH));
            const uint32_t b_now = (uint32_t)__builtin_popcountll(__builtin_amdgcn_ballot_w64(state == ST_BOUNCE));
            if (drained) {
                if (m_now == 0u || 2u * b_now >= m_now + b_now) {
                    break;
                }
            } else if (m_now < sc.burst_march_min || b_now >= sc.burst_scatter || 64u - m_now - b_now >= sc.burst_idle) {
                break;
            }
            w_fetch += m_now;
            if (STATS) {
                st_march += 1;
                st_march_l += m_now;
            }
            }
        }
        if (finished) {
            ba.frames[out_idx] = make_float4(rad.x, rad.y, rad.z, 1.f);
            if (STATS) {
                iv_written += 1;
            }
            if (COST && ba.cost) {
                ba.cost[out_idx - ba.out_offset] = make_uint2(work, depth);
            }
            state = ST_IDLE;
        }
        if (may_suspend && drained && job.next == job.end) {
            const bool mine = state != ST_IDLE && age < ba.max_age;
            const uint64_t live = __builtin_amdgcn_ballot_w64(mine);
            if (live != 0ull) {
                const uint32_t n = (uint32_t)__builtin_popcountll(live);
                uint32_t base = 0;
                if (lane == (uint32_t)__builtin_ctzll(live)) {
                    base = atomicAdd(ba.cont_out_count, n);
                    if (base + n > ba.cont_capacity) {
                        atomicSub(ba.cont_out_count, n);
                        base = 0xffffffffu;
                    } else if (ba.cont_total) {
                        atomicAdd(ba.cont_total, (unsigned long long)n);
                    }
                }
                base = __builtin_amdgcn_readlane(base, __builtin_ctzll(live));
                if (mine && base != 0xffffffffu) {
                    uint4 *e = (uint4 *)(ba.cont_out + (size_t)(base + lane_rank(live)) * kContWords);
                    e[0] = make_uint4(__float_as_uint(pos.x), __float_as_uint(pos.y), __float_as_uint(pos.z), __float_as_uint(dir.x));
                    e[1] = make_uint4(__float_as_uint(dir.y), __float_as_uint(dir.z), __float_as_uint(rad.x), __float_as_uint(rad.y));
                    e[2] = make_uint4(__float_as_uint(rad.z), seed, out_idx, __float_as_uint(xi));
                    e[3] = make_uint4(__float_as_uint(T), __float_as_uint(inv_maxd), depth | (dfree << 16) | ((uint32_t)state << 24), age + 1u);
                    state = ST_IDLE;
                    if (STATS) {
                        iv_suspended += 1;
                    }
                }
            }
        }
    }

#ifdef CT_DIAG_TIMELINE
    if (ba.timeline && lane == 0u) {
        ba.timeline[4u * (blockIdx.x * (blockDim.x >> 6) + (threadIdx.x >> 6)) + 1u] = wall_clock64();
    }
#endif
    const uint32_t vals[3] = { wave_sum(c_dl), wave_sum(c_il), wave_sum(c_cap) };
    if (STATS) {
        uint32_t sv[16] = { st_fetch, st_zero, st_skip, st_zero_d0, st_zero_d1, st_skip_iters, st_first,
                            iv_dealt, iv_resumed, iv_written, iv_suspended, st_same_line, st_dup_line, st_hit2, st_hit3, st_nee_zero };
#pragma unroll
        for (int i = 0; i < 16; i++) {
            sv[i] = wave_sum(sv[i]);
        }
        if (lane == 0) {
            atomicAdd(&ba.stats[0], (unsigned long long)st_regen);
            atomicAdd(&ba.stats[1], (unsigned long long)st_regen_l);
            atomicAdd(&ba.stats[2], (unsigned long long)st_march);
            atomicAdd(&ba.stats[3], (unsigned long long)st_march_l);
            atomicAdd(&ba.stats[4], (unsigned long long)st_scat);
            atomicAdd(&ba.stats[5], (unsigned long long)st_scat_l);
            atomicAdd(&ba.stats[6], (unsigned long long)sv[0]);
            atomicAdd(&ba.stats[7], (unsigned long long)sv[1]);
            atomicAdd(&ba.stats[8], (unsigned long long)sv[2]);
            atomicAdd(&ba.stats[9], (unsigned long long)sv[3]);
            atomicAdd(&ba.stats[10], (unsigned long long)sv[4]);
            atomicAdd(&ba.stats[11], (unsigned long long)sv[5]);
            atomicAdd(&ba.stats[12], (unsigned long long)sv[6]);
            atomicAdd(&ba.stats[13], 1ull);
            atomicAdd(&ba.stats[14], (unsigned long long)st_stolen);
            atomicMax(&ba.stats[15], (unsigned long long)st_iters);
            const unsigned long long t_end = wall_clock64();
#ifdef CT_STATS_FINE
            atomicAdd(&ba.stats[16 + min((unsigned long long)23, (t_end - t_start) / 25000ull)], 1ull);
            atomicAdd(&ba.stats[40 + min((unsigned long long)23, (t_end - (t_drained ? t_drained : t_end)) / 5000ull)], 1ull);
// ... 696 lines not shown
            const uint32_t b_now = (uint32_t)__builtin_popcountll(__builtin_amdgcn_ballot_w64(state == ST_BOUNCE));
            if ((DELTA_CHECK_EVERY == 1 || (burst % DELTA_CHECK_EVERY) == 0u) &&
                (m_now == 0u || b_now >= sc.burst_scatter || 64u - m_now - b_now >= sc.burst_idle)) {
                break;
            }
            if (STATS) {
                st_march += 1;
                st_march_l += m_now;
                if (m_now) {
                    st_hist_t[min((m_now - 1u) >> 3, 7u)] += 1;
                }
                st_drained_t += drained ? 1u : 0u;
            }
            }
        }
        if (finished) {
#ifdef CT_DEBUG_BOUNDS
            if (age == 0u && ba.frame_stride && out_idx - ba.out_offset >= ba.S * ba.frame_stride) {
                printf("CT_DEBUG_BOUNDS frames[%u] outside the batch (offset %u, S %u, stride %u)\n", out_idx, ba.out_offset, ba.S, ba.frame_stride);
                out_idx = ba.out_offset;
            }
#endif
            ba.frames[out_idx] = make_float4(rad.x, rad.y, rad.z, 1.f);
            if (STATS) {
                iv_written += 1;
            }
            if (!INTERIOR && ba.cost) {
                ba.cost[out_idx - ba.out_offset] = make_uint2(depth, depth);
            }
            state = ST_IDLE;
        }
        if (may_suspend && drained && job.next == job.end) {
            const bool mine = state != ST_IDLE && age < ba.max_age;
            const uint64_t live = __builtin_amdgcn_ballot_w64(mine);
            if (live != 0ull) {
                const uint32_t n = (uint32_t)__builtin_popcountll(live);
                uint32_t base = 0;
                if (lane == (uint32_t)__builtin_ctzll(live)) {
                    base = atomicAdd(ba.cont_out_count, n);
                    if (base + n > ba.cont_capacity) {
                        atomicSub(ba.cont_out_count, n);
                        base = 0xffffffffu;
                    } else if (ba.cont_total) {
                        atomicAdd(ba.cont_total, (unsigned long long)n);
                    }
                }
                base = __builtin_amdgcn_readlane(base, __builtin_ctzll(live));
                if (mine && base != 0xffffffffu) {
                    uint4 *e = (uint4 *)(ba.cont_out + (size_t)(base + lane_rank(live)) * kContWordsDelta);
                    e[0] = make_uint4(__float_as_uint(pos.x), __float_as_uint(pos.y), __float_as_uint(pos.z), __float_as_uint(dir.x));
                    e[1] = make_uint4(__float_as_uint(dir.y), __float_as_uint(dir.z), __float_as_uint(rad.x), __float_as_uint(rad.y));
                    e[2] = make_uint4(__float_as_uint(rad.z), seed, out_idx, depth | ((uint32_t)state << 24));
                    e[3] = make_uint4(__float_as_uint(dda.org.x), __float_as_uint(dda.org.y), __float_as_uint(dda.org.z), __float_as_uint(dda.t));
                    e[4] = make_uint4(__float_as_uint(dda.tmax.x), __float_as_uint(dda.tmax.y), __float_as_uint(dda.tmax.z), (uint32_t)dda.bx);
                    e[5] = make_uint4(__float_as_uint(dda.tdelta.x), __float_as_uint(dda.tdelta.y), __float_as_uint(dda.tdelta.z), (uint32_t)dda.by);
                    e[6] = make_uint4((uint32_t)dda.bz, age + 1u, 0u, 0u);
                    state = ST_IDLE;
                    if (STATS) {
                        iv_suspended += 1;
                    }
                }
            }
        }
    }

    const uint32_t vals[3] = { wave_sum(c_dl), wave_sum(c_il), wave_sum(c_cap) };
    if (STATS) {
        uint32_t sv[8] = { st_fetch, st_zero, st_skip, iv_dealt, iv_resumed, iv_written, iv_suspended, st_empty };
#pragma unroll
        for (int i = 0; i < 8; i++) {
            sv[i] = wave_sum(sv[i]);
        }
        if (lane == 0) {
            atomicAdd(&ba.stats[0], (unsigned long long)st_regen);
            atomicAdd(&ba.stats[1], (unsigned long long)st_regen_l);
            atomicAdd(&ba.stats[2], (unsigned long long)st_march);
            atomicAdd(&ba.stats[3], (unsigned long long)st_march_l);
            atomicAdd(&ba.stats[4], (unsigned long long)st_scat);
            atomicAdd(&ba.stats[5], (unsigned long long)st_scat_l);
            atomicAdd(&ba.stats[6], (unsigned long long)sv[0]);
            atomicAdd(&ba.stats[7], (unsigned long long)sv[1]);
            atomicAdd(&ba.stats[8], (unsigned long long)sv[2]);
            for (int i = 0; i < 8; i++) {
                atomicAdd(&ba.stats[16 + i], (unsigned long long)st_hist_t[i]);
                atomicAdd(&ba.stats[24 + i], (unsigned long long)st_hist_s[i]);
            }
            atomicAdd(&ba.stats[9], (unsigned long long)sv[7]);
            atomicAdd(&ba.stats[32], (unsigned long long)st_drained_t);
            atomicAdd(&ba.stats[64], (unsigned long long)sv[3]);
            atomicAdd(&ba.stats[65], (unsigned long long)sv[4]);
            atomicAdd(&ba.stats[66], (unsigned long long)sv[5]);
            atomicAdd(&ba.stats[67], (unsigned long long)sv[6]);
        }
    }
    flush_counters(ba, lane, vals[0], vals[1], vals[2], vals[0], vals[1]);
}

template <bool STATS, int NEE, bool FIXED8>
static void launch_render_delta_mode(const DevScene &sc, const BatchArgs &ba, dim3 grid, dim3 block, hipStream_t stream)
{
    if (NEE != 0 && !STATS && sc.delta_interior != 0u && ba.cost == nullptr) {
        constexpr int N = NEE != 0 ? NEE : 1;
        switch (sc.mode) {
        case 0: hipLaunchKernelGGL((render_delta_kernel<0, false, N, true, FIXED8>), grid, block, 0, stream, sc, ba); break;
        case 1: hipLaunchKernelGGL((render_delta_kernel<1, false, N, true, FIXED8>), grid, block, 0, stream, sc, ba); break;
        default: hipLaunchKernelGGL((render_delta_kernel<2, false, N, true, FIXED8>), grid, block, 0, stream, sc, ba); break;
        }
        return;
    }
    switch (sc.mode) {
    case 0: hipLaunchKernelGGL((render_delta_kernel<0, STATS, NEE, false, FIXED8>), grid, block, 0, stream, sc, ba); break;
    case 1: hipLaunchKernelGGL((render_delta_kernel<1, STATS, NEE, false, FIXED8>), grid, block, 0, stream, sc, ba); break;
    default: hipLaunchKernelGGL((render_delta_kernel<2, STATS, NEE, false, FIXED8>), grid, block, 0, stream, sc, ba); break;
    }
}

template <bool FIXED8>
static void launch_render_delta_nee(const DevScene &sc, const BatchArgs &ba, dim3 grid, dim3 block, hipStream_t stream, bool stats)
{
    const int nee = sc.delta_nee == 2u && sc.tbricks ? 2 : (sc.delta_nee == 1u ? 1 : 0);
    if (stats) {
        switch (nee) {
        case 0: launch_render_delta_mode<true, 0, FIXED8>(sc, ba, grid, block, stream); break;
        case 1: launch_render_delta_mode<true, 1, FIXED8>(sc, ba, grid, block, stream); break;
        default: launch_render_delta_mode<true, 2, FIXED8>(sc, ba, grid, block, stream); break;
        }
    } else {
        switch (nee) {
        case 0: launch_render_delta_mode<false, 0, FIXED8>(sc, ba, grid, block, stream); break;
        case 1: launch_render_delta_mode<false, 1, FIXED8>(sc, ba, grid, block, stream); break;
        default: launch_render_delta_mode<false, 2, FIXED8>(sc, ba, grid, block, stream); break;
        }
    }
}

hipError_t launch_render_delta(const DevScene &sc, const BatchArgs &ba, LaunchShape shape, hipStream_t stream)
{
    const dim3 grid(shape.blocks), block(shape.threads);
    if (sc.tex_fixed8) {
        launch_render_delta_nee<true>(sc, ba, grid, block, stream, shape.stats);
    } else {
        launch_render_delta_nee<false>(sc, ba, grid, block, stream, shape.stats);
    }
    return hipGetLastError();
}

#ifdef CT_EXPERIMENTS
#include "ct_exchange.hpp"
#endif

LaunchShape persistent_shape(int device, bool delta, int blocks_per_cu)
{
    hipDeviceProp_t prop;
    LaunchShape s{ 1024, delta ? kDeltaThreads : 512, false };
    if (hipGetDeviceProperties(&prop, device) == hipSuccess && prop.multiProcessorCount > 0) {
        int per_cu = 0;
        const hipError_t e = delta ? hipOccupancyMaxActiveBlocksPerMultiprocessor(&per_cu, render_delta_kernel<0, false, 0>, kDeltaThreads, 0)
                                   : hipOccupancyMaxActiveBlocksPerMultiprocessor(&per_cu, render_persistent_kernel<0, false, false>, 512, 0);
        if (e != hipSuccess || per_cu < 1) {
            per_cu = delta ? 2 : 3;
        }
        s.blocks = prop.multiProcessorCount * std::min(per_cu, 8);
        if (blocks_per_cu >= 1 && blocks_per_cu <= 8) {
            s.blocks = prop.multiProcessorCount * blocks_per_cu;
        }
    }
    return s;
}

template <bool STATS, bool SPARSE, bool FIXED8>
static void launch_render_persistent_mode(const DevScene &sc, const BatchArgs &ba, dim3 grid, dim3 block, hipStream_t stream)
{
    if (!STATS && !SPARSE && ba.cost == nullptr) {
        switch (sc.mode) {
        case 0: hipLaunchKernelGGL((render_persistent_kernel<0, false, false, false, FIXED8>), grid, block, 0, stream, sc, ba); break;
        case 1: hipLaunchKernelGGL((render_persistent_kernel<1, false, false, false, FIXED8>), grid, block, 0, stream, sc, ba); break;
        default: hipLaunchKernelGGL((render_persistent_kernel<2, false, false, false, FIXED8>), grid, block, 0, stream, sc, ba); break;
        }
        return;
    }
    switch (sc.mode) {
    case 0: hipLaunchKernelGGL((render_persistent_kernel<0, STATS, SPARSE, true, FIXED8>), grid, block, 0, stream, sc, ba); break;
    case 1: hipLaunchKernelGGL((render_persistent_kernel<1, STATS, SPARSE, true, FIXED8>), grid, block, 0, stream, sc, ba); break;
    default: hipLaunchKernelGGL((render_persistent_kernel<2, STATS, SPARSE, true, FIXED8>), grid, block, 0, stream, sc, ba); break;
    }
}

template <bool FIXED8>
static void launch_render_persistent_stats(const DevScene &sc, const BatchArgs &ba, dim3 grid, dim3 block, hipStream_t stream,
                                            bool stats)
{
    const bool sparse = sc.m_rows != nullptr;
    if (stats) {
        if (sparse) {
            launch_render_persistent_mode<true, true, FIXED8>(sc, ba, grid, block, stream);
        } else {
            launch_render_persistent_mode<true, false, FIXED8>(sc, ba, grid, block, stream);
        }
    } else if (sparse) {
        launch_render_persistent_mode<false, true, FIXED8>(sc, ba, grid, block, stream);
    } else {
        launch_render_persistent_mode<false, false, FIXED8>(sc, ba, grid, block, stream);
    }
}

hipError_t launch_render_persistent(const DevScene &sc, const BatchArgs &ba, LaunchShape shape, hipStream_t stream)
{
    const dim3 grid(shape.blocks), block(shape.threads);
    if (sc.tex_fixed8) {
        launch_render_persistent_stats<true>(sc, ba, grid, block, stream, shape.stats);
    } else {
        launch_render_persistent_stats<false>(sc, ba, grid, block, stream, shape.stats);
    }
    return hipGetLastError();
}

template <bool FIXED8>
__global__ __launch_bounds__(256) void render_simple_kernel(DevScene sc, BatchArgs ba, uint32_t shard_index,
                                                            uint32_t shard_count)
{
    __shared__ MieLds lds;
    load_tables(sc, lds);
    const uint32_t tile = blockIdx.x / 4u;
    const uint32_t wave = threadIdx.x >> 6, l = threadIdx.x & 63u;
    const uint32_t tile_id = blockIdx.x * 4u + wave;
    (void)tile;
    if (tile_id >= sc.tiles_x * sc.tiles_y) {
        return;
    }
    const uint32_t ty = tile_id / sc.tiles_x, tx = tile_id - ty * sc.tiles_x;
    if (tile_owner(tx, ty, shard_count) != shard_index) {
        return;
    }
    const uint32_t x = tx * kTile + (l & 7u), y = ty * kTile + (l >> 3);
    if (x >= sc.width || y >= sc.height) {
        return;
    }
    const uint32_t out_idx = y * sc.width + x;
    uint32_t c_hits = 0, c_dl = 0, c_il = 0, c_cap = 0;
    f3 rad = mk3(0, 0, 0);
    const f3 eye = mk3(sc.ex, sc.ey, sc.ez);
    const f3 d = primary_direction(sc, x, y);
    float t_hit;
    if (intersect_box(sc, eye, d, t_hit)) {
        c_hits = 1;
        f3 pos = add3(eye, scale3(d, t_hit));
        pos = add3(pos, scale3(mk3(sc.bx, sc.by, sc.bz), 0.5f));
        f3 dir = normalize3(d);
        uint32_t seed = tea4(x * 4096u + y, ba.first_subframe);
        if (sc.mode == 1) {
            dir = new_direction(lds.cdf, lds.guide, seed, dir);
        }
        uint32_t depth = 0;
        while (in_box(sc, pos)) {
            if (sc.mode != 2) {
                depth++;
                if (depth == sc.max_depth) {
                    c_cap = 1;
                    break;
                }
            }
            const float xi = u24_to_float(lcg24(seed));
            const f3 stepv = scale3(dir, sc.sample_step);
            float T = 1;
            bool scattered = false;
            while (in_box(sc, pos)) {
                pos = add3(pos, stepv);
                const float density = tex3_apron<FIXED8>(sc, sc.dbricks, pos) * sc.density_multiplier;
                c_dl++;
                const float extinction = density * sc.sample_step;
                T *= ct_expf(-extinction);
                if (xi > T) {
                    scattered = true;
                    const float lg = ct_logf(xi / T);
                    const float inv = 1.0f / density;
                    pos = sub3(pos, scale3(scale3(dir, lg), inv));
                    break;
                }
            }
            if (!scattered || !in_box(sc, pos)) {
                break;
            }
            const bool chopped = (sc.mode == 1) ? true : (sc.mode == 0 ? (depth != 1) : false);
            rad = add3(rad, in_scattering<FIXED8>(sc, pos, dir, chopped));
            c_il++;
            if (sc.mode == 2) {
                break;
            }
            dir = new_direction(lds.cdf, lds.guide, seed, dir);
        }
    }
    ba.frames[out_idx] = make_float4(rad.x, rad.y, rad.z, 1.f);
    atomicAdd(&ba.counters[0], 1ull);
    atomicAdd(&ba.counters[1], (unsigned long long)c_hits);
    atomicAdd(&ba.counters[2], (unsigned long long)c_dl);
    atomicAdd(&ba.counters[3], (unsigned long long)c_il);
    atomicAdd(&ba.counters[4], (unsigned long long)c_il);
    atomicAdd(&ba.counters[5], (unsigned long long)c_cap);
    atomicAdd(&ba.counters[6], (unsigned long long)c_dl);
    atomicAdd(&ba.counters[7], (unsigned long long)c_il);
}

hipError_t launch_render_simple(const DevScene &sc, const BatchArgs &ba, uint32_t shard_index,
                                uint32_t shard_count, hipStream_t stream)
{
    const uint32_t tiles = sc.tiles_x * sc.tiles_y;
    if (sc.tex_fixed8) {
        hipLaunchKernelGGL(render_simple_kernel<true>, dim3((tiles + 3) / 4), dim3(256), 0, stream, sc, ba, shard_index,
                           shard_count);
    } else {
        hipLaunchKernelGGL(render_simple_kernel<false>, dim3((tiles + 3) / 4), dim3(256), 0, stream, sc, ba, shard_index,
                           shard_count);
    }
    return hipGetLastError();
}

template <bool FIXED8>
CT_DEV bool plain_flight(const DevScene &sc, float xi, f3 &pos, f3 dir)
{
    const f3 stepv = scale3(dir, sc.sample_step);
    float T = 1;
    while (in_box(sc, pos)) {
        pos = add3(pos, stepv);
        const float density = tex3_apron<FIXED8>(sc, sc.dbricks, pos) * sc.density_multiplier;
        const float extinction = density * sc.sample_step;
        T *= ct_expf(-extinction);
        if (xi > T) {
            const float lg = ct_logf(xi / T);
            const float inv = 1.0f / density;
            pos = sub3(pos, scale3(scale3(dir, lg), inv));
            return true;
        }
    }
    return false;
}

template <bool FIXED8>
__global__ __launch_bounds__(64) void scatter_samples_kernel(DevScene sc, uint32_t count, uint32_t batch_seed,
                                                            float *__restrict__ positions,
                                                            float *__restrict__ directions)
{
    const uint32_t i = blockIdx.x * blockDim.x + threadIdx.x;
    if (i >= count) {
        return;
    }
    uint32_t seed = tea4(i, batch_seed);
    const float nanv = __uint_as_float(0x7fc00000u);
    f3 out_p = mk3(nanv, nanv, nanv), out_d = mk3(nanv, nanv, nanv);
    for (uint32_t attempt = 0; attempt < 4096u; attempt++) {
        const float u = u24_to_float(lcg24(seed));
        const float v = u24_to_float(lcg24(seed));
        const float phi = u * kPi * 2;
        const float cos_theta = 2 * v - 1;
        const float sin_theta = sqrtf(1 - cos_theta * cos_theta);
        float sn, cs;
        ct_sincosf(phi, &sn, &cs);
        const f3 normal = mk3(cs * sin_theta, sn * sin_theta, cos_theta);
        const float theta = u24_to_float(lcg24(seed)) * kPi * 2;
        const float sqrt_r = sqrtf(u24_to_float(lcg24(seed)));
        float st, ct;
        ct_sincosf(theta, &st, &ct);
        const float dx = sqrt_r * ct, dy = sqrt_r * st;
        f3 b;
        if (fabsf(normal.x) > fabsf(normal.z)) {
            b = mk3(-normal.y, normal.x, 0.0f);
// ... 752 lines not shown
```

Before: 3677.

## Precompute per-slot start records, use 32-bit brick offsets, move mie table to LDS

Adds a kernel that packs each queue slot's start position, direction, seed and advance prefix into a contiguous record, so the persistent march kernel reads one coalesced pair instead of chasing pixel indices into primary and advance. Brick address computation now uses 32-bit offsets unless the volume exceeds 4 GiB or a knob forces wide offsets. The mie phase table is copied into LDS next to the chopped table, and the march block grows to 768 threads with two blocks per CU by default. These add LDS use and an extra precompute pass per queue rebuild, and the occupancy change may help or hurt.

After: 3769, median of 6. 1.03x the previous value.

```diff
diff --git a/deepestscatter_amd/csrc/ct_api.cpp b/deepestscatter_amd/csrc/ct_api.cpp
--- a/deepestscatter_amd/csrc/ct_api.cpp
+++ b/deepestscatter_amd/csrc/ct_api.cpp
@@ -186,7 +186,7 @@
     }
 #endif
     void *ptrs[] = { h->d_density, h->d_inscatter, h->d_dbricks, h->d_ibricks, h->d_mbricks, h->d_tbricks, h->d_touched[0], h->d_touched[1], h->d_mrows, h->d_mcoarse, h->d_pyramid, h->d_mie, h->d_chopped, h->d_cdf,
-                     h->d_guide, h->d_dist, h->d_dist_tmp, h->d_majorant, h->d_maj_cells, h->d_maj_codes, h->d_frame, h->d_mean, h->d_m2, h->d_screen, h->d_frames_all, h->cont[0], h->cont[1], h->left[0], h->left[1], h->d_cont_count, h->d_cont_total, h->d_primary, h->d_advance, h->d_pixels, h->d_cost, h->d_group_rank, h->d_group_order, h->d_job_group, h->d_job_sub, h->d_queue,
+                     h->d_guide, h->d_dist, h->d_dist_tmp, h->d_majorant, h->d_maj_cells, h->d_maj_codes, h->d_frame, h->d_mean, h->d_m2, h->d_screen, h->d_frames_all, h->cont[0], h->cont[1], h->left[0], h->left[1], h->d_cont_count, h->d_cont_total, h->d_primary, h->d_advance, h->d_pixels, h->d_start, h->d_cost, h->d_group_rank, h->d_group_order, h->d_job_group, h->d_job_sub, h->d_queue,
                      h->d_counters, h->d_colsum, h->d_avg, h->d_freeze, h->d_hit, h->d_cost_plane, h->d_timeline, h->pt.tasks, h->pt.primary, h->pt.frames, h->pt.pixels, h->pt.jg, h->pt.js,
                      h->net.found, h->net.waves, h->net.pos, h->net.dir, h->net.aux, h->net.out, h->net.desc, h->net.direct, h->net.tiles };
     for (void *p : ptrs) {
@@ -867,6 +867,8 @@
     }
     const size_t dense_bytes = (size_t)(mgx * bgy * bgz) * 128;
     h->mbricks_dense_bytes = h->mbricks_bytes = dense_bytes;
+    const size_t ibricks_bytes = (size_t)(bgx * bgy * bgz) * 128;
+    h->shape.wide = std::max(dense_bytes, ibricks_bytes) > (1ull << 32) || knob_flag(h->tune.WIDE_OFFSETS, false);
     HIPCHK(h, dmalloc(&h->d_mbricks, dense_bytes));
     d.mbricks = h->d_mbricks;
     d.m_bias_x = mbias;
@@ -1156,6 +1158,11 @@
     return relight(h, s);
 }
 
+static bool start_records(CtHandle h)
+{
+    return h->scene.estimator == CT_EST_MARCH && !(h->scene.flags & CT_FLAG_SIMPLE_KERNEL) && knob_flag(h->tune.START_RECORDS, true);
+}
+
 static int rebuild_queue(CtHandle h)
 {
     TracePhase trace(h, "rebuild_queue");
@@ -1208,12 +1215,13 @@
     }
     h->n_groups = (uint32_t)(list.size() / 64);
     if (h->n_groups > h->groups_capacity) {
-        for (void *p : { (void *)h->d_pixels, (void *)h->d_cost }) {
+        for (void *p : { (void *)h->d_pixels, (void *)h->d_cost, (void *)h->d_start }) {
             if (p) {
                 HIPCHK(h, hipFree(p));
             }
         }
         h->d_pixels = h->d_cost = nullptr;
+        h->d_start = nullptr;
         for (void *p : { (void *)h->d_group_rank, (void *)h->d_group_order }) {
             if (p) {
                 HIPCHK(h, hipFree(p));
@@ -1224,6 +1232,9 @@
         HIPCHK(h, dmalloc(&h->d_cost, 2 * (size_t)h->n_groups));
         HIPCHK(h, dmalloc(&h->d_group_rank, (size_t)h->n_groups));
         HIPCHK(h, dmalloc(&h->d_group_order, (size_t)h->n_groups));
+        if (start_records(h)) {
+            HIPCHK(h, dmalloc(&h->d_start, 2 * (size_t)h->n_groups * 64));
+        }
         h->groups_capacity = h->n_groups;
     }
     h->group_order.resize(h->n_groups);
@@ -1251,6 +1262,11 @@
         HIPCHK(h, hipMemcpyAsync(h->d_pixels, list.data(), list.size() * sizeof(uint32_t), hipMemcpyHostToDevice,
                                  h->stream));
         HIPCHK(h, hipMemsetAsync(h->d_cost, 0, 2 * (size_t)h->n_groups * sizeof(uint32_t), h->stream));
+        if (h->d_start) {
+            const bool prefix = h->scene.mode != 1 && !h->no_advance;
+            HIPCHK(h, launch_start_records(h->dev, h->d_pixels, h->n_groups * 64u, h->d_primary, prefix ? h->d_advance : nullptr, h->d_start,
+                                           h->stream));
+        }
         HIPCHK(h, hipStreamSynchronize(h->stream));
     }
     h->queue_dirty = false;
@@ -1738,6 +1754,7 @@
     ba.primary = h->d_primary;
     ba.advance = h->no_advance ? nullptr : h->d_advance;
     ba.pixels = h->d_pixels;
+    ba.start = dense ? nullptr : h->d_start;
     ba.group_rank = (simple || dense || h->n_chunks <= 1) ? nullptr : h->d_group_rank;
     ba.rank_base = rank_base;
     ba.job_group = h->d_job_group;
@@ -1907,6 +1924,7 @@
         ba.primary = h->d_primary;
         ba.advance = h->no_advance ? nullptr : h->d_advance;
         ba.pixels = h->d_pixels;
+        ba.start = h->d_start;
         ba.job_group = h->d_job_group;
         ba.job_sub = h->d_job_sub;
         ba.n_jobs = 0;
diff --git a/deepestscatter_amd/csrc/ct_device.hpp b/deepestscatter_amd/csrc/ct_device.hpp
--- a/deepestscatter_amd/csrc/ct_device.hpp
+++ b/deepestscatter_amd/csrc/ct_device.hpp
@@ -211,13 +211,21 @@
     return r;
 }
 
-template <bool SPARSE>
+template <bool WIDE>
+CT_DEV void load_footprint_pair(const uint8_t *bricks, uint32_t brick, uint32_t local, uint2 &a, uint2 &c)
+{
+    const uint8_t *p = WIDE ? bricks + (((size_t)brick << 7) | local) : bricks + (uint32_t)((brick << 7) | local);
+    __builtin_memcpy(&a, p, 8);
+    __builtin_memcpy(&c, p + 25, 8);
+}
+
+template <bool SPARSE, bool WIDE = true>
 CT_DEV uint2 load_footprint_m(const DevScene &sc, int32_t ix, int32_t iy, int32_t iz, uint32_t &meta)
 {
     const uint32_t x = (uint32_t)(ix + sc.m_bias_x), y = (uint32_t)(iy + sc.brick_bias), z = (uint32_t)(iz + sc.brick_bias);
     const uint32_t bx = __umul24(x, 43691u) >> 17;
-    const uint32_t lx = x - __umul24(bx, 3u);
-    const uint32_t brick = __umul24(z >> 2, (uint32_t)sc.m_gxy) + __umul24(y >> 2, (uint32_t)sc.m_gx) + bx;
+    const uint32_t lx = x - ((bx << 1) + bx);
+    uint32_t brick = __umul24(z >> 2, (uint32_t)sc.m_gxy) + __umul24(y >> 2, (uint32_t)sc.m_gx) + bx;
     const uint32_t local = __umul24(z & 3u, 25u) + __umul24(y & 3u, 5u) + lx;
 #ifdef CT_DEBUG_BOUNDS
     if (bx >= (uint32_t)sc.m_gx || (y >> 2) >= (uint32_t)sc.brick_gy || (z >> 2) >= (uint32_t)sc.brick_gz) {
@@ -226,7 +234,6 @@
         return make_uint2(0u, 0u);
     }
 #endif
-    const uint8_t *p = sc.mbricks + (((size_t)brick << 7) | local);
     if (SPARSE) {
         const uint32_t row = __umul24(z >> 2, (uint32_t)sc.brick_gy) + (y >> 2);
         const uint2 ri = sc.m_rows[row];
@@ -236,11 +243,10 @@
             meta = sc.m_coarse[__umul24(z >> sc.m_cshift, (uint32_t)sc.m_cgxy) + __umul24(y >> sc.m_cshift, (uint32_t)sc.m_cgx) + cx];
             return make_uint2(0u, 0u);
         }
-        p = sc.mbricks + (((size_t)(ri.x + rel) << 7) | local);
+        brick = ri.x + rel;
     }
     uint2 a, c;
-    __builtin_memcpy(&a, p, 8);
-    __builtin_memcpy(&c, p + 25, 8);
+    load_footprint_pair<WIDE>(sc.mbricks, brick, local, a, c);
     meta = __builtin_amdgcn_perm(a.y, a.x, 0x0c0c0c04u - lx);
     uint2 r;
     r.x = __builtin_amdgcn_perm(a.y, a.x, 0x06050100u);
@@ -370,6 +376,7 @@
     return make_uint2(__builtin_amdgcn_perm(r.a.y, r.a.x, 0x05040100u), __builtin_amdgcn_perm(r.c.y, r.c.x, 0x07060302u));
 }
 
+template <bool WIDE>
 CT_DEV uint2 fetch_cell_cached(const DevScene &sc, const uint8_t *bricks, f3 p, uint32_t &key, uint2 &cached, bool &reused,
                                bool zero = false)
 {
@@ -381,10 +388,8 @@
     const uint32_t off = (brick << 7) | local;
     reused = sc.nee_cache != 0u && off == key;
     if (!reused && !zero) {
-        const uint8_t *q = bricks + (((size_t)brick << 7) | local);
         uint2 a, c;
-        __builtin_memcpy(&a, q, 8);
-        __builtin_memcpy(&c, q + 25, 8);
+        load_footprint_pair<WIDE>(bricks, brick, local, a, c);
         cached.x = __builtin_amdgcn_perm(a.y, a.x, 0x06050100u);
         cached.y = __builtin_amdgcn_perm(c.y, c.x, 0x06050100u);
         key = off;
@@ -392,11 +397,11 @@
     return zero ? make_uint2(0u, 0u) : cached;
 }
 
-template <bool SPARSE>
+template <bool SPARSE, bool WIDE = true>
 CT_DEV uint2 fetch_cell_m(const DevScene &sc, f3 p, uint32_t &meta)
 {
     const float x = fmaf(p.x, sc.sx, -0.5f), y = fmaf(p.y, sc.sy, -0.5f), z = fmaf(p.z, sc.sz, -0.5f);
-    return load_footprint_m<SPARSE>(sc, floor_to_int(x), floor_to_int(y), floor_to_int(z), meta);
+    return load_footprint_m<SPARSE, WIDE>(sc, floor_to_int(x), floor_to_int(y), floor_to_int(z), meta);
 }
 
 template <bool FIXED8>
diff --git a/deepestscatter_amd/csrc/ct_handle.hpp b/deepestscatter_amd/csrc/ct_handle.hpp
--- a/deepestscatter_amd/csrc/ct_handle.hpp
+++ b/deepestscatter_amd/csrc/ct_handle.hpp
@@ -18,7 +18,7 @@
     const char *get() const { return is_set ? text.c_str() : nullptr; }
     explicit operator bool() const { return is_set; }
 };
-#define CT_KNOBS(X) X(BURST_IDLE) X(BURST_MARCH_MIN) X(BURST_SCATTER) X(CHUNK_INTERLEAVE) X(CHUNK_MORTON) X(CONTINUATION) X(DEBUG_INVARIANTS) X(DELTA_INTERIOR) X(DELTA_NEE) X(EXCHANGE) X(HAND_ON_JOBS) X(HINT_PERIOD) X(JOB_MAX) X(JOB_WORK) X(MARCH_BURST) X(MAX_AGE) X(NEE_CACHE) X(NET_DESC_RECORDS) X(NO_ADVANCE) X(POINT_BLOCKS_PER_CU) X(POINT_ORDER) X(REGEN_MIN) X(RENDER_AHEAD) X(SCATTER_MIN) X(SCATTER_RATIO) X(SCRATCH_GIB) X(SCRATCH_MIB) X(SERPENTINE) X(SHARED_DEPTH) X(SPARSE) X(STATS) X(TAIL_BURST) X(TILE_ORDER) X(TIMELINE) X(TRACE) X(TUNE_SUBFRAMES) X(XCD_QUEUES) X(XCD_QUEUES_UNTUNED) X(XCD_REGIONS) X(BLOCKS_PER_CU)
+#define CT_KNOBS(X) X(BURST_IDLE) X(BURST_MARCH_MIN) X(BURST_SCATTER) X(CHUNK_INTERLEAVE) X(CHUNK_MORTON) X(CONTINUATION) X(DEBUG_INVARIANTS) X(DELTA_INTERIOR) X(DELTA_NEE) X(EXCHANGE) X(HAND_ON_JOBS) X(HINT_PERIOD) X(JOB_MAX) X(JOB_WORK) X(MARCH_BURST) X(MAX_AGE) X(NEE_CACHE) X(NET_DESC_RECORDS) X(NO_ADVANCE) X(POINT_BLOCKS_PER_CU) X(POINT_ORDER) X(REGEN_MIN) X(RENDER_AHEAD) X(SCATTER_MIN) X(SCATTER_RATIO) X(SCRATCH_GIB) X(SCRATCH_MIB) X(SERPENTINE) X(SHARED_DEPTH) X(SPARSE) X(STATS) X(TAIL_BURST) X(TILE_ORDER) X(TIMELINE) X(TRACE) X(TUNE_SUBFRAMES) X(XCD_QUEUES) X(XCD_QUEUES_UNTUNED) X(XCD_REGIONS) X(BLOCKS_PER_CU) X(WIDE_OFFSETS) X(START_RECORDS)
 struct CtTuning {
 #define X(name) Knob name;
     CT_KNOBS(X)
@@ -121,6 +121,7 @@
     float4 *d_primary = nullptr;
     float4 *d_advance = nullptr;
     uint32_t *d_pixels = nullptr;
+    float4 *d_start = nullptr;
     uint8_t *d_hit = nullptr, *hit_host = nullptr;
     uint32_t *d_cost = nullptr;
     uint32_t *d_touched[2] = { nullptr, nullptr };
diff --git a/deepestscatter_amd/csrc/ct_internal.hpp b/deepestscatter_amd/csrc/ct_internal.hpp
--- a/deepestscatter_amd/csrc/ct_internal.hpp
+++ b/deepestscatter_amd/csrc/ct_internal.hpp
@@ -24,6 +24,7 @@
     const float4 *primary;
     const float4 *advance;
     const uint32_t *pixels;
+    const float4 *start;
     const uint32_t *group_rank;
     uint32_t rank_base;
     const uint32_t *job_group;
@@ -62,6 +63,7 @@
     bool stats;
     uint32_t pool_slots = 0;
     uint32_t scatter_waves = 0;
+    bool wide = false;
 };
 
 inline void split_queues_evenly(BatchArgs &ba)
@@ -114,6 +116,8 @@
                               hipStream_t stream);
 hipError_t launch_hit_flags(const float4 *primary, uint8_t *flags, uint32_t pixels, hipStream_t stream);
 hipError_t launch_primary_advance(const DevScene &sc, const float4 *primary, float4 *advance, hipStream_t stream);
+hipError_t launch_start_records(const DevScene &sc, const uint32_t *pixels, uint32_t slots, const float4 *primary,
+                                const float4 *advance, float4 *start, hipStream_t stream);
 hipError_t launch_primary_advance_delta(const DevScene &sc, const float4 *primary, float4 *advance, hipStream_t stream);
 struct ZeroList {
     uint32_t *ptr[6];
diff --git a/deepestscatter_amd/csrc/ct_kernels.hip b/deepestscatter_amd/csrc/ct_kernels.hip
--- a/deepestscatter_amd/csrc/ct_kernels.hip
+++ b/deepestscatter_amd/csrc/ct_kernels.hip
@@ -592,9 +592,18 @@
     uint16_t guide[kGuideN + 2];
 };
 
+#ifndef CT_MARCH_PHASE_LDS
+#define CT_MARCH_PHASE_LDS 2
+#endif
+constexpr int kMarchThreads = CT_MARCH_PHASE_LDS == 2 ? 768 : 512;
+constexpr int kMarchBlocksPerCu = CT_MARCH_PHASE_LDS == 2 ? 2 : 3;
+
 struct MieLdsFull {
     float cdf[kMieN];
     float chopped[kMieN];
+#if CT_MARCH_PHASE_LDS == 2
+    float mie[kMieN];
+#endif
     uint16_t guide[kGuideN + 2];
 };
 
@@ -603,6 +612,9 @@
     for (int i = threadIdx.x; i < kMieN; i += blockDim.x) {
         lds.cdf[i] = sc.cdf[i];
         lds.chopped[i] = sc.chopped[i];
+#if CT_MARCH_PHASE_LDS == 2
+        lds.mie[i] = sc.mie[i];
+#endif
     }
     for (int i = threadIdx.x; i < kGuideN + 2; i += blockDim.x) {
         lds.guide[i] = sc.guide[i];
@@ -864,8 +876,11 @@
     return n;
 }
 
-template <bool FIXED8>
-CT_DEV NeeLoads in_scattering_issue_lds(const DevScene &sc, const float *lds_chopped, f3 pos, f3 dir, bool chopped,
+typedef const float __attribute__((address_space(3))) LdsFloat;
+typedef const float __attribute__((address_space(1))) GlobalFloat;
+
+template <bool FIXED8, bool WIDE>
+CT_DEV NeeLoads in_scattering_issue_lds(const DevScene &sc, const MieLdsFull &lds, f3 pos, f3 dir, bool chopped,
                                         uint32_t &nee_key, uint2 &nee_cell, bool &reused, bool zero = false)
 {
     NeeLoads n;
@@ -875,15 +890,27 @@
     const int32_t i = (int32_t)floorf(x);
     const int32_t j = min(max(i, 0), kMieN - 2);
     float2 pair;
+#if CT_MARCH_PHASE_LDS == 2
+    LdsFloat *table = chopped ? (LdsFloat *)lds.chopped : (LdsFloat *)lds.mie;
+    pair = make_float2(table[j], table[j + 1]);
+#elif CT_MARCH_PHASE_LDS == 1
+    LdsFloat *table = (LdsFloat *)lds.chopped;
+    pair = make_float2(table[j], table[j + 1]);
+    if (!chopped) {
+        GlobalFloat *first = (GlobalFloat *)(sc.mie + j);
+        pair = make_float2(first[0], first[1]);
+    }
+#else
     if (chopped) {
-        pair = make_float2(lds_chopped[j], lds_chopped[j + 1]);
+        pair = make_float2(lds.chopped[j], lds.chopped[j + 1]);
     } else {
         __builtin_memcpy(&pair, sc.mie + j, sizeof pair);
     }
+#endif
     n.a = (i > kMieN - 2) ? pair.y : pair.x;
     n.b = (i < 0) ? pair.x : pair.y;
     n.w = tex_weight<FIXED8>(x);
-    n.cell = fetch_cell_cached(sc, sc.ibricks, pos, nee_key, nee_cell, reused, zero);
+    n.cell = fetch_cell_cached<WIDE>(sc, sc.ibricks, pos, nee_key, nee_cell, reused, zero);
     return n;
 }
 
@@ -1078,8 +1105,41 @@
     return hipGetLastError();
 }
 
-template <int MODE, bool STATS, bool SPARSE, bool COST = true, bool FIXED8 = false>
-__global__ __launch_bounds__(512) __attribute__((amdgpu_waves_per_eu(6))) void render_persistent_kernel(DevScene sc, BatchArgs ba)
+__global__ __launch_bounds__(256) void start_records_kernel(DevScene sc, const uint32_t *__restrict__ pixels, uint32_t slots,
+                                                            const float4 *__restrict__ primary, const float4 *__restrict__ advance,
+                                                            float4 *__restrict__ start)
+{
+    const uint32_t i = blockIdx.x * 256u + threadIdx.x;
+    if (i >= slots) {
+        return;
+    }
+    const uint32_t pixel = pixels[i];
+    float4 r0 = make_float4(0.f, 0.f, 0.f, __uint_as_float(0xc0000000u)), r1 = make_float4(0.f, 0.f, 0.f, 0.f);
+    if (pixel != 0xffffffffu) {
+        const float4 p0 = primary[2 * (size_t)pixel];
+        r1 = primary[2 * (size_t)pixel + 1];
+        const bool go = p0.w != 0.f && in_box(sc, mk3(p0.x, p0.y, p0.z));
+        uint32_t bits = go ? 0u : 0x80000000u;
+        r0 = p0;
+        if (go && advance) {
+            r0 = advance[pixel];
+            bits |= __float_as_uint(r0.w) & 0x3fffffffu;
+        }
+        r0.w = __uint_as_float(bits);
+    }
+    start[2 * (size_t)i] = r0;
+    start[2 * (size_t)i + 1] = r1;
+}
+
+hipError_t launch_start_records(const DevScene &sc, const uint32_t *pixels, uint32_t slots, const float4 *primary,
+                                const float4 *advance, float4 *start, hipStream_t stream)
+{
+    hipLaunchKernelGGL(start_records_kernel, dim3((slots + 255u) / 256u), dim3(256), 0, stream, sc, pixels, slots, primary, advance, start);
+    return hipGetLastError();
+}
+
+template <int MODE, bool STATS, bool SPARSE, bool COST = true, bool FIXED8 = false, bool WIDE = false>
+__global__ __launch_bounds__(kMarchThreads) __attribute__((amdgpu_waves_per_eu(6))) void render_persistent_kernel(DevScene sc, BatchArgs ba)
 {
     __shared__ MieLdsFull lds;
     load_tables(sc, lds);
@@ -1216,18 +1276,44 @@
                 if (take) {
                     const uint32_t s = q >> 6, l = q & 63u;
                     const uint32_t g = job.g;
-                    const uint32_t pixel = ba.pixels[g * 64u + l];
-                    if (pixel != 0xffffffffu) {
+                    f3 p_start = mk3(0, 0, 0), p_dir = mk3(0, 0, 1);
+                    uint32_t seed_base = 0, bits = 0;
+                    bool valid, starts = false;
+                    const float4 *prefix = nullptr;
+                    if (ba.start) {
+                        const float4 *rec = ba.start + 2 * (size_t)(g * 64u + l);
+                        const float4 r0 = rec[0], r1 = rec[1];
+                        const uint32_t w = __float_as_uint(r0.w);
+                        valid = (w & 0x40000000u) == 0u;
+                        starts = (w & 0x80000000u) == 0u;
+                        bits = w & 0x3fffffffu;
+                        p_start = mk3(r0.x, r0.y, r0.z);
+                        p_dir = mk3(r1.x, r1.y, r1.z);
+                        seed_base = __float_as_uint(r1.w);
+                        out_idx = job.base + s * ba.frame_stride + l;
+                    } else {
+                        const uint32_t pixel = ba.pixels[g * 64u + l];
+                        valid = pixel != 0xffffffffu;
+                        if (valid) {
+                            const float4 p0 = ba.primary[2 * (size_t)pixel];
+                            const float4 p1 = ba.primary[2 * (size_t)pixel + 1];
+                            out_idx = ba.frame_stride ? job.base + s * ba.frame_stride + l : pixel;
+                            p_start = mk3(p0.x, p0.y, p0.z);
+                            starts = p0.w != 0.f && in_box(sc, p_start);
+                            p_dir = mk3(p1.x, p1.y, p1.z);
+                            seed_base = __float_as_uint(p1.w);
+                            if (MODE != 1 && ba.advance) {
+                                prefix = ba.advance + pixel;
+                            }
+                        }
+                    }
+                    if (valid) {
                         if (STATS) {
                             iv_dealt += 1;
                         }
-                        const float4 p0 = ba.primary[2 * (size_t)pixel];
-                        const float4 p1 = ba.primary[2 * (size_t)pixel + 1];
-                        out_idx = ba.frame_stride ? job.base + s * ba.frame_stride + l : pixel;
-                        pos = mk3(p0.x, p0.y, p0.z);
-                        const bool hit = p0.w != 0.f;
-                        dir = mk3(p1.x, p1.y, p1.z);
-                        seed = tea4(__float_as_uint(p1.w), job.first + s);
+                        pos = p_start;
+                        dir = p_dir;
+                        seed = tea4(seed_base, job.first + s);
                         rad = mk3(0, 0, 0);
                         depth = 0;
                         work = 0;
@@ -1235,7 +1321,7 @@
                         if (MODE == 1) {
                             dir = new_direction(lds.cdf, lds.guide, seed, dir);
                         }
-                        bool go = hit && in_box(sc, pos);
+                        bool go = starts;
                         if (MODE != 2 && go) {
                             depth = 1;
                             if (depth == sc.max_depth) {
@@ -1248,14 +1334,13 @@
                             T = 1;
                             stepv = scale3(dir, sc.sample_step);
                             inv_maxd = inv_max_advance(sc, stepv);
-                            dfree = 0;
-                            if (MODE != 1 && ba.advance) {
-                                const float4 a = ba.advance[pixel];
-                                const uint32_t bits = __float_as_uint(a.w);
+                            if (prefix) {
+                                const float4 a = *prefix;
                                 pos = mk3(a.x, a.y, a.z);
-                                dfree = bits >> 24;
-                                c_dl += bits & 0x00ffffffu;
+                                bits = __float_as_uint(a.w);
                             }
+                            dfree = bits >> 24;
+                            c_dl += bits & 0x00ffffffu;
                             state = ST_MARCH;
                         } else {
                             ba.frames[out_idx] = make_float4(0.f, 0.f, 0.f, 1.f);
@@ -1299,10 +1384,10 @@
                     NeeLoads nee;
                     if (CT_MARCH_NEE_SKIP == 1) {
                         if (!nee_zero) {
-                            nee = in_scattering_issue_lds<FIXED8>(sc, lds.chopped, pos, dir, chopped, nee_key, nee_cell, nee_reused);
+                            nee = in_scattering_issue_lds<FIXED8, WIDE>(sc, lds, pos, dir, chopped, nee_key, nee_cell, nee_reused);
                         }
                     } else {
-                        nee = in_scattering_issue_lds<FIXED8>(sc, lds.chopped, pos, dir, chopped, nee_key, nee_cell, nee_reused, nee_zero);
+                        nee = in_scattering_issue_lds<FIXED8, WIDE>(sc, lds, pos, dir, chopped, nee_key, nee_cell, nee_reused, nee_zero);
                     }
                     if (STATS) {
                         st_nee_zero += nee_zero ? 1u : 0u;
@@ -1385,7 +1470,7 @@
                 }
                 pos = add3(pos, stepv);
                 uint32_t meta;
-                const uint2 cell = fetch_cell_m<SPARSE>(sc, pos, meta);
+                const uint2 cell = fetch_cell_m<SPARSE, WIDE>(sc, pos, meta);
                 dfree = meta & 0x3fu;
                 c_dl += 1;
                 if (COST) {
@@ -2388,13 +2473,13 @@
 LaunchShape persistent_shape(int device, bool delta, int blocks_per_cu)
 {
     hipDeviceProp_t prop;
-    LaunchShape s{ 1024, delta ? kDeltaThreads : 512, false };
+    LaunchShape s{ 1024, delta ? kDeltaThreads : kMarchThreads, false };
     if (hipGetDeviceProperties(&prop, device) == hipSuccess && prop.multiProcessorCount > 0) {
         int per_cu = 0;
         const hipError_t e = delta ? hipOccupancyMaxActiveBlocksPerMultiprocessor(&per_cu, render_delta_kernel<0, false, 0>, kDeltaThreads, 0)
-                                   : hipOccupancyMaxActiveBlocksPerMultiprocessor(&per_cu, render_persistent_kernel<0, false, false>, 512, 0);
+                                   : hipOccupancyMaxActiveBlocksPerMultiprocessor(&per_cu, render_persistent_kernel<0, false, false>, kMarchThreads, 0);
         if (e != hipSuccess || per_cu < 1) {
-            per_cu = delta ? 2 : 3;
+            per_cu = delta ? 2 : kMarchBlocksPerCu;
         }
         s.blocks = prop.multiProcessorCount * std::min(per_cu, 8);
         if (blocks_per_cu >= 1 && blocks_per_cu <= 8) {
@@ -2404,10 +2489,10 @@
     return s;
 }
 
-template <bool STATS, bool SPARSE, bool FIXED8>
+template <bool STATS, bool SPARSE, bool FIXED8, bool WIDE>
 static void launch_render_persistent_mode(const DevScene &sc, const BatchArgs &ba, dim3 grid, dim3 block, hipStream_t stream)
 {
-    if (!STATS && !SPARSE && ba.cost == nullptr) {
+    if (!STATS && !SPARSE && !WIDE && ba.cost == nullptr) {
         switch (sc.mode) {
         case 0: hipLaunchKernelGGL((render_persistent_kernel<0, false, false, false, FIXED8>), grid, block, 0, stream, sc, ba); break;
         case 1: hipLaunchKernelGGL((render_persistent_kernel<1, false, false, false, FIXED8>), grid, block, 0, stream, sc, ba); break;
@@ -2416,37 +2501,47 @@
         return;
     }
     switch (sc.mode) {
-    case 0: hipLaunchKernelGGL((render_persistent_kernel<0, STATS, SPARSE, true, FIXED8>), grid, block, 0, stream, sc, ba); break;
-    case 1: hipLaunchKernelGGL((render_persistent_kernel<1, STATS, SPARSE, true, FIXED8>), grid, block, 0, stream, sc, ba); break;
-    default: hipLaunchKernelGGL((render_persistent_kernel<2, STATS, SPARSE, true, FIXED8>), grid, block, 0, stream, sc, ba); break;
-    }
-}
-
-template <bool FIXED8>
+    case 0: hipLaunchKernelGGL((render_persistent_kernel<0, STATS, SPARSE, true, FIXED8, WIDE>), grid, block, 0, stream, sc, ba); break;
+    case 1: hipLaunchKernelGGL((render_persistent_kernel<1, STATS, SPARSE, true, FIXED8, WIDE>), grid, block, 0, stream, sc, ba); break;
+    default: hipLaunchKernelGGL((render_persistent_kernel<2, STATS, SPARSE, true, FIXED8, WIDE>), grid, block, 0, stream, sc, ba); break;
+    }
+}
+
+template <bool FIXED8, bool WIDE>
 static void launch_render_persistent_stats(const DevScene &sc, const BatchArgs &ba, dim3 grid, dim3 block, hipStream_t stream,
                                             bool stats)
 {
     const bool sparse = sc.m_rows != nullptr;
     if (stats) {
         if (sparse) {
-            launch_render_persistent_mode<true, true, FIXED8>(sc, ba, grid, block, stream);
+            launch_render_persistent_mode<true, true, FIXED8, WIDE>(sc, ba, grid, block, stream);
         } else {
-            launch_render_persistent_mode<true, false, FIXED8>(sc, ba, grid, block, stream);
+            launch_render_persistent_mode<true, false, FIXED8, WIDE>(sc, ba, grid, block, stream);
         }
     } else if (sparse) {
-        launch_render_persistent_mode<false, true, FIXED8>(sc, ba, grid, block, stream);
+        launch_render_persistent_mode<false, true, FIXED8, WIDE>(sc, ba, grid, block, stream);
     } else {
-        launch_render_persistent_mode<false, false, FIXED8>(sc, ba, grid, block, stream);
+        launch_render_persistent_mode<false, false, FIXED8, WIDE>(sc, ba, grid, block, stream);
+    }
+}
+
+template <bool WIDE>
+static void launch_render_persistent_wide(const DevScene &sc, const BatchArgs &ba, dim3 grid, dim3 block, hipStream_t stream, bool stats)
+{
+    if (sc.tex_fixed8) {
+        launch_render_persistent_stats<true, WIDE>(sc, ba, grid, block, stream, stats);
+    } else {
+        launch_render_persistent_stats<false, WIDE>(sc, ba, grid, block, stream, stats);
     }
 }
 
 hipError_t launch_render_persistent(const DevScene &sc, const BatchArgs &ba, LaunchShape shape, hipStream_t stream)
 {
     const dim3 grid(shape.blocks), block(shape.threads);
-    if (sc.tex_fixed8) {
-        launch_render_persistent_stats<true>(sc, ba, grid, block, stream, shape.stats);
+    if (shape.wide) {
+        launch_render_persistent_wide<true>(sc, ba, grid, block, stream, shape.stats);
     } else {
-        launch_render_persistent_stats<false>(sc, ba, grid, block, stream, shape.stats);
+        launch_render_persistent_wide<false>(sc, ba, grid, block, stream, shape.stats);
     }
     return hipGetLastError();
 }
```
